# KAIST-AILab/SyncVSR

Measured on AMD Instinct MI355X. Metric: lip-clips/sec training (29x88x88), higher is better.
Workload: dtype bf16; 1 GPU; LRW training step (fwd+bwd+allreduce+clip+AdamW), ResNet18 + 6-layer 512-d encoder + vq audio-token CE head, random-init weights, N(0,1) clips 29x88x88, uniform tokens/labels; per_gpu_batch=32, global_batch=32, parallelism=dp1, hip_graph=False, enqueue=native step list

## Files before the change

### include/syncvsr_hip.h

```cpp
#ifndef SYNCVSR_HIP_H
#define SYNCVSR_HIP_H

#include <stdint.h>

#ifndef __HIP_PLATFORM_AMD__
typedef void* hipStream_t;
#else
#include <hip/hip_runtime_api.h>
#endif

#define SVSR_OK 0
#define SVSR_ERR_ARG 1001
#define SVSR_GRAD_ADD_DW 1
#define SVSR_GRAD_ADD_DB 2
#define SVSR_ERR_GROUP_OPEN 1003
#define SVSR_ERR_NO_GROUP 1004
#define SVSR_ERR_MASK_SIZE 1005

typedef struct svsr_wgrad_problem {
    const void* x; const void* dy; float* dw; float* dbias; const int* plan_dev; const int* meta;
    int Nimg; int in_pix; int Ci; int in_pitch; int Co; int out_pix; int out_pitch; int wt_taps;
} svsr_wgrad_problem;

typedef struct svsr_enc_layer {
    const void* wqkv; const void* wo; const void* w1; const void* w2;
    const float* bqkv; const float* bo; const float* b1; const float* b2; const float* g1; const float* be1; const float* g2; const float* be2;
    void* qkv; void* probs; void* ctx; void* ao; void* x1; void* z; void* hg; void* f; void* xout;
    float* m1; float* r1; float* m2; float* r2;
    unsigned site_probs; unsigned site_ao; unsigned site_fo; unsigned pad_;
} svsr_enc_layer;

typedef struct svsr_enc_bwd_layer {
    const void* w2t; const void* w1t; const void* wot; const void* wqkvt;
    const float* g1; const float* g2;
    const void* f; const void* x1; const void* ao; const void* xin; const void* z; const void* qkv; const void* probs;
    const float* m1; const float* r1; const float* m2; const float* r2;
    void* ds2; void* df; void* dz; void* dx1; void* ds1; void* dao; void* dqkv; void* dx;
    float* part1; float* part2;
    unsigned site_probs; unsigned site_ao; unsigned site_fo; unsigned pad_;
} svsr_enc_bwd_layer;

#ifdef __cplusplus
extern "C" {
#endif

int svsr_tune(const char* key, int value);
int svsr_tune_value(const char* key, int* value);
int svsr_colsum_rows(const float* ws, int nrows, int64_t ld, float* out0, int64_t n0, float* out1, int64_t n1, int accumulate, float scale, hipStream_t stream);
int svsr_colsum_rows_multi(const void* entries, int n, hipStream_t stream);

int svsr_conv_plan(int mode, int Nimg, int H, int W, int Co_out, int k, int stride, int pad, int* words, int cap_words, int* meta);
int svsr_rows_plan(int Nimg, int P, int src0, int dst0, int Co_out, int* words, int cap_words, int* meta);
int svsr_igemm_fwd_kgroups(const int* meta, int Ci, int Co, int bn_epilogue);
int svsr_igemm_fwd(const void* in, const void* wt, void* out, void* out_pre, const float* bias, const void* addend, float* stats, const int* plan_dev, const int* meta, int Nimg, int in_pix, int Ci, int in_pitch, int Co, int out_pix, int out_pitch, int wt_taps, int act, int out_f32, float alpha, const unsigned* drop_seed, unsigned drop_site, float drop_p, hipStream_t stream);

int svsr_wgrad_plan(int Nimg, int H, int W, int Ci, int Co, int k, int stride, int pad, int* words, int cap_words, int* meta, int64_t* part_floats);
int svsr_wgrad_rows_plan(int Nimg, int P, int src0, int dst0, int Ci, int Co, int has_bias, int* words, int cap_words, int* meta, int64_t* part_floats);
int svsr_igemm_wgrad(const void* x, const void* dyp, float* dw, float* dbias, const int* plan_dev, const int* meta, int Nimg, int in_pix, int Ci, int in_pitch, int Co, int out_pix, int out_pitch, int wt_taps, float* part, int64_t part_floats, hipStream_t stream);
int64_t svsr_igemm_wgrad_group_bytes(int n);
int svsr_igemm_wgrad_group(const svsr_wgrad_problem* problems, int n, void* table_dev, int64_t table_bytes, hipStream_t stream);
int svsr_igemm_wgrad_v2(const void* x, const void* dyp, float* dw, float* dbias, const int* plan_dev, const int* meta, int Nimg, int in_pix, int Ci, int in_pitch, int Co, int out_pix, int out_pitch, int wt_taps, float* part, int64_t part_floats, int mode, hipStream_t stream);
int svsr_igemm_wgrad_group_v2(const svsr_wgrad_problem* problems, const int* modes, int n, void* table_dev, int64_t table_bytes, hipStream_t stream);

int svsr_conv3x3_c64_stat_rows(int Nimg, int H, int W);
int64_t svsr_conv3x3_c64_pixtab(int Nimg, int H, int W, int* out, int64_t cap);
int svsr_conv3x3_c64(const void* in, const void* wt, void* out, const void* addend, float* stats, int Nimg, int H, int W, const int* dy, const int* dx, const int* tw, const int* pixtab, hipStream_t stream);

int svsr_igemm_dgrad_bn(const void* in, const void* wt, void* out, const void* addend, float* stats, const int* plan_dev, const int* meta, int Nimg, int in_pix, int Ci, int in_pitch, int Co, int out_pix, int out_pitch, int wt_taps, const void* y, const void* x, const float* mean, const float* rstd, const float* gamma, const float* beta, int act, hipStream_t stream);
int svsr_igemm_dgrad_relu(const void* in, const void* wt, void* out, float* stats, const int* plan_dev, const int* meta, int Nimg, int in_pix, int Ci, int in_pitch, int Co, int out_pix, int out_pitch, int wt_taps, const void* y, const float* zeros, const float* ones, float gscale, hipStream_t stream);
int svsr_conv3x3_c64_dgrad_bn(const void* in, const void* wt, void* out, const void* addend, float* stats, int Nimg, int H, int W, const int* dy, const int* dx, const int* tw, const void* y, const void* x, const float* mean, const float* rstd, const float* gamma, const float* beta, int act, const int* pixtab, hipStream_t stream);
int svsr_bn_bwd_from_stats(const void* g, const void* x, const float* mean, const float* rstd, const float* gamma, const float* stats, int nrows, float* coef, float* dgamma, float* dbeta, void* dx, int64_t npix, int C, hipStream_t stream);


int svsr_conv3x3_wgrad_plan(int Nimg, int H, int W, int Ci, int Co, int* splits, int64_t* part_floats);
int svsr_conv3x3_wgrad(const void* x, const void* dy, float* dw, int Nimg, int H, int W, int Ci, int Co, float* part, int64_t part_floats, hipStream_t stream);
int svsr_conv3x3_wgrad_v2(const void* x, const void* dy, float* dw, int Nimg, int H, int W, int Ci, int Co, float* part, int64_t part_floats, int mode, hipStream_t stream);

int svsr_stem_conv_fwd_stat_rows(int B, int T, int H, int W);
int64_t svsr_stem_conv_fwd_ws_bytes(int B, int T, int H, int W);
int svsr_stem_conv_fwd(const float* vid, const float* w, void* out, float* stats, int B, int T, int H, int W, void* ws, int64_t ws_bytes, hipStream_t stream);

int svsr_stem_conv_wgrad_plan(int B, int T, int H, int W, int* splits, int64_t* part_floats);
int svsr_stem_conv_wgrad(const float* vid, const void* dy, float* dw, int B, int T, int H, int W, int use_tr, float* part, int64_t part_floats, hipStream_t stream);

int svsr_stem_bwd_wgrad_ok(int B, int T, int H, int W);
int svsr_stem_bwd_wgrad(const float* vid, const void* gpool, const void* amax, const void* x, const float* mean, const float* rstd, const float* coef, float* dw, int B, int T, int H, int W, float* part, int64_t part_floats, hipStream_t stream);

int svsr_bn_finalize(const float* part, int nrows, int C, float count, float eps, float momentum, float* mean, float* rstd, float* running_mean, float* running_var, int64_t* num_batches_tracked, hipStream_t stream);

int svsr_bn_eval_prepare(const float* running_mean, const float* running_var, int C, float eps, float* mean, float* rstd, hipStream_t stream);

int svsr_bn_act_fwd(const void* x, const void* res, void* y, const float* mean, const float* rstd, const float* gamma, const float* beta, int64_t npix, int C, int act, hipStream_t stream);

int svsr_bn_act_bwd_rows(int64_t npix, int C);
int svsr_bn_act_bwd(const void* dy, const void* y, const void* x, const float* mean, const float* rstd, const float* gamma, float* slots, float* coef, float* dgamma, float* dbeta, void* dx, void* dres, int64_t npix, int C, int act, const float* beta, const void* res, hipStream_t stream);

int svsr_stem_bn_act_pool_fwd(const void* x, void* y, void* amax, const float* mean, const float* rstd, const float* gamma, const float* beta, int N, int Hc, int Wc, int Hp, int Wp, int C, int act, void* xwin, hipStream_t stream);

int svsr_stem_bn_act_pool_bwd_rows(int N, int Hc, int Wc, int C);
int svsr_stem_bn_act_pool_bwd(const void* dpool, const void* amax, const void* x, const float* mean, const float* rstd, const float* gamma, const float* beta, float* slots, float* coef, float* dgamma, float* dbeta, void* dx, int N, int Hc, int Wc, int Hp, int Wp, int C, int act, const void* xwin, void* gpool, hipStream_t stream);

int svsr_avgpool_fwd(const void* x, void* y, int64_t N, int HW, int C, hipStream_t stream);
int svsr_avgpool_bwd(const void* dy, void* dx, int64_t N, int HW, int C, hipStream_t stream);

int svsr_add_ln_fwd(const void* a, const void* r, const float* gamma, const float* beta, void* y, float* mean, float* rstd, int R, int D, float eps, hipStream_t stream);
int svsr_add_ln_bwd_rows(int R);
int svsr_add_ln_bwd(const void* dy, const void* a, const void* r, const float* gamma, const float* mean, const float* rstd, void* ds, float* dgamma, float* dbeta, int R, int D, const void* addend, float* part, hipStream_t stream);
int svsr_add_ln_bwd_partials(const void* dy, const void* a, const void* r, const float* gamma, const float* mean, const float* rstd, void* ds, int R, int D, const void* addend, float* part, hipStream_t stream);
int svsr_add_ln_bwd_branch(const void* dy, const void* a, const void* r, const float* gamma, const float* mean, const float* rstd, void* ds, int R, int D, const void* addend, float* part, void* ds2, float alpha2, const unsigned* drop_seed, unsigned drop_site, float drop_p, hipStream_t stream);
int svsr_bias_act_bwd_partials(const void* dy, const void* z, void* dz, float* db, int R, int N, int n_valid, int ld, int act, float gscale, float* part, hipStream_t stream);

int svsr_embed_ln_fwd(const void* feats, const float* cls, const float* pos, const float* type0, const float* gamma, const float* beta, void* sum_out, void* y, float* mean, float* rstd, int B, int S, int D, float eps, const unsigned* drop_seed, unsigned site_in, float p_in, unsigned site_out, float p_out, hipStream_t stream);
int svsr_embed_bwd_scatter(const void* ds, void* dfeats, float* dcls, float* dpos, float* dtype0, int B, int S, int D, float* part, const unsigned* drop_seed, unsigned site_in, float p_in, hipStream_t stream);

int svsr_rmsnorm_fwd(const void* x, const float* g, void* y, float* inv, int R, int D, int ld, float eps, hipStream_t stream);
int svsr_rmsnorm_bwd_rows(int R);
int svsr_rmsnorm_bwd(const void* dy, const void* x, const float* g, const float* inv, const void* addend, void* dx, float* dg, float* part, int R, int D, int ld, hipStream_t stream);

int svsr_rotary(void* qkv, const float* tab, int R, int S, int heads_total, int ld, int sign, hipStream_t stream);

int svsr_geglu_fwd(const void* u, void* y, int R, int I, int ldu, int ldy, const unsigned* drop_seed, unsigned drop_site, float drop_p, hipStream_t stream);
int svsr_geglu_bwd(const void* dy, const void* u, void* du, int R, int I, int ldu, int ldy, const unsigned* drop_seed, unsigned drop_site, float drop_p, hipStream_t stream);

int svsr_xt_embed_fwd(const void* feats, const float* wmask, const float* cls, void* x0, int B, int S, int F, int D, int ld, const unsigned* drop_seed, unsigned drop_site, float drop_p, hipStream_t stream);
int svsr_xt_embed_bwd(const void* dx0, void* dfeats, float* dcls, int B, int S, int F, int D, int ld, const unsigned* drop_seed, unsigned drop_site, float drop_p, hipStream_t stream);

int svsr_bias_act_bwd_rows(int R, int N);
int svsr_bias_act_bwd(const void* dy, const void* z, void* dz, float* db, int R, int N, int n_valid, int ld, int act, float gscale, float* part, hipStream_t stream);

int svsr_ce_fwd(const void* logits, int logits_f32, int ld, const int64_t* target_idx, const float* target_prob, int ldt, int R, int V, float smoothing, float* loss, float* lse, float* row_loss, hipStream_t stream);
int svsr_ce_bwd(const void* logits, int logits_f32, int ld, const int64_t* target_idx, const float* target_prob, int ldt, int R, int V, float smoothing, const float* lse, const float* gout, void* dlogits, int ldo, hipStream_t stream);

int svsr_linear_ce_ok(int R, int K, int G, int V);
int svsr_linear_ce_fwd(const void* h, const void* w, const float* bias, const int64_t* tok, int R, int K, int G, int V, int seq_S, int seq_s0, int seq_T, float* loss, float* lse, float* row_loss, hipStream_t stream);
int svsr_linear_ce_bwd(const void* h, const void* w, const float* bias, const int64_t* tok, int R, int K, int G, int V, int seq_S, int seq_s0, int seq_T, const float* lse, const float* gout, void* dlogits, hipStream_t stream);

int64_t svsr_w2v_stats_floats(int B, int F0);
int svsr_w2v_conv0(const float* wave, int B, int L_in, int pad, const float* w, const float* bias, const float* gamma, const float* beta, float eps, void* out, int out_rows, float* stats, int mode, hipStream_t stream);
int svsr_w2v_norm_gelu(void* x, int B, int F, int rows, const float* gamma, const float* beta, float eps, float* stats, int F0, int mode, hipStream_t stream);
int svsr_w2v_quantize(const void* feat, int R, int F, int keep, const float* gamma, const float* beta, float eps, const void* w, const float* bias, const unsigned* seed, unsigned site, int64_t* tok, float* logits_out, hipStream_t stream);

int svsr_topk_acc(const float* logits, const int64_t* labels, const float* soft_labels, int B, int C, float* out2, float* rows2, hipStream_t stream);

int svsr_grad_sumsq(const float* g, int64_t n, void* opt_state, hipStream_t stream);
int svsr_grad_sumsq_parts(const float* g, int64_t n, void* opt_state, int part0, int nparts, hipStream_t stream);
int svsr_adamw_step(float* p, const float* g, float* m, float* v, void* shadow, int64_t n, int64_t decay_end, float lr, float beta1, float beta2, float eps, float weight_decay, float max_norm, int warmup, int total_steps, void* opt_state, hipStream_t stream);
int svsr_adamw_range(float* p, const float* g, float* m, float* v, void* shadow, int64_t n, int64_t decay_end, float lr, float beta1, float beta2, float eps, float weight_decay, float max_norm, int warmup, int total_steps, void* opt_state, int advance, hipStream_t stream);

int svsr_cast_bf16(const float* src, void* dst, int64_t n, hipStream_t stream);
int svsr_transpose_cast_multi(const float* src, void* dst, const void* table, int n_entries, hipStream_t stream);
int svsr_transpose_bf16_multi(const void* src16, void* dst, const void* table, int n_entries, hipStream_t stream);
int svsr_fill_f32(float* p, int64_t n, float v, hipStream_t stream);
int svsr_fill_ranges(float* base, int64_t limit, const int64_t* ranges, int n, unsigned bits, hipStream_t stream);
int svsr_enc_gave_up(int reset);
int svsr_enc_gave_up_peek(void);
int svsr_debug_enc_spin_limit(unsigned limit);
int64_t svsr_enc_fwd_ws_bytes(int B);
int svsr_debug_enc_trace(int64_t* out, int n);
int svsr_enc_fwd(const void* x0, const svsr_enc_layer* layers, int n_layers, int B, int S, float ln_eps, const unsigned* drop_seed, float p_hidden, float p_attn, void* ws, int64_t ws_bytes, hipStream_t stream);

int64_t svsr_enc_bwd_ws_bytes(int B);
int svsr_enc_bwd(const void* dy, const svsr_enc_bwd_layer* layers, int n_layers, int B, int S, const unsigned* drop_seed, float p_hidden, float p_attn, void* ws, int64_t ws_bytes, hipStream_t stream);

int svsr_word_add(int* word, int delta, hipStream_t stream);
int svsr_lincomb2(const float* a, const float* b, float wb, float* out, hipStream_t stream);
int svsr_lincomb3_ratio(const float* a, float wa, const float* b, float wb, const float* c, float wc, float* out0, const float* num, const float* den, float* out1, hipStream_t stream);

int svsr_clip_prep(const void* src_u8, const int* params, float* dst, int B, int T, int Hs, int Ws, int H, int W, float mean, float std, hipStream_t stream);

int svsr_mha_fwd(const void* q, int q_pitch, const void* k, const void* v, int kv_pitch, const void* pe, int pe_pitch, const float* bias_u, const float* bias_v, const int* klen, int causal, int B, int H, int dh, int Lq, int Lk, int ldp, float scale, void* ctx, int ctx_pitch, void* probs, const unsigned* drop_seed, unsigned drop_site, float drop_p, hipStream_t stream);

int svsr_mha_bwd(const void* dctx, int dctx_pitch, const void* q, int q_pitch, const void* k, const void* v, int kv_pitch, const void* pe, int pe_pitch, const float* bias_u, const float* bias_v, const void* probs, void* ds, int B, int H, int dh, int Lq, int Lk, int ldp, float scale, void* dq, int dq_pitch, void* dq_ac, void* dq_bd, int aux_pitch, void* dk, void* dv, int dkv_pitch, void* dpe, int dpe_pitch, float* pe_part, const unsigned* drop_seed, unsigned drop_site, float drop_p, hipStream_t stream);

int64_t svsr_mha_flash_ws_bytes(int H, int Lq);
int svsr_mha_flash_fwd(const void* q, int q_pitch, const void* k, const void* v, int kv_pitch, const void* pe, int pe_pitch, const float* bias_u, const float* bias_v, const int* klen, int causal, int B, int H, int dh, int Lq, int Lk, int ldp, float scale, void* ctx, int ctx_pitch, float* lse, const unsigned* drop_seed, unsigned drop_site, float drop_p, hipStream_t stream);
int svsr_mha_flash_bwd(const void* dctx, int dctx_pitch, const void* ctx, int ctx_pitch, const float* lse, const void* q, int q_pitch, const void* k, const void* v, int kv_pitch, const void* pe, int pe_pitch, const float* bias_u, const float* bias_v, const int* klen, int causal, void* probs, void* ds, int B, int H, int dh, int Lq, int Lk, int ldp, float scale, void* dq, int dq_pitch, void* dq_ac, void* dq_bd, int aux_pitch, void* dk, void* dv, int dkv_pitch, void* dpe, int dpe_pitch, float* pe_part, void* ws, int64_t ws_bytes, const unsigned* drop_seed, unsigned drop_site, float drop_p, hipStream_t stream);
int svsr_mha_pe_transpose(const void* pe, int pe_pitch, int H, int Lq, void* ws, int64_t ws_bytes, hipStream_t stream);
int svsr_mha_flash_bwd_parts(const void* dctx, int dctx_pitch, const void* ctx, int ctx_pitch, const float* lse, const void* q, int q_pitch, const void* k, const void* v, int kv_pitch, const void* pe, int pe_pitch, const float* bias_u, const float* bias_v, const int* klen, int causal, void* probs, void* ds, int B, int H, int dh, int Lq, int Lk, int ldp, float scale, void* dq, int dq_pitch, void* dq_ac, void* dq_bd, int aux_pitch, void* dk, void* dv, int dkv_pitch, void* dpe, int dpe_pitch, float* pe_part, void* ws, int64_t ws_bytes, const unsigned* drop_seed, unsigned drop_site, float drop_p, int parts, hipStream_t stream);

int svsr_glu_dwconv_fwd_stat_rows(int B, int T);
int svsr_glu_dwconv_fwd(const void* u, const float* w, const float* bias, void* c, float* stats, int B, int T, int D, int K, hipStream_t stream);

int svsr_glu_dwconv_bwd(const void* dc, const void* u, const float* w, void* du, float* dw, float* dbias, float* part, int nsplit, int B, int T, int D, int K, hipStream_t stream);
int svsr_glu_dwconv_bwd_parts(const void* dc, const void* u, const float* w, void* du, float* dw, float* dbias, float* part, int nsplit, int B, int T, int D, int K, int parts, hipStream_t stream);

int svsr_ctc_fwd(const float* logits, int ld, const int64_t* labels, int Lmax, const int* ilen, int B, int T, int V, float* lse, float* ab, float* nll, float* loss, hipStream_t stream);

int svsr_ctc_grad(const float* logits, int ld, const int64_t* labels, int Lmax, const int* ilen, int B, int T, int V, const float* lse, const float* ab, const float* nll, const float* gout, void* dlogits, int ldo, hipStream_t stream);

int svsr_ctc_prefix_score(const float* logp, int ldp, const float* r_prev, const int64_t* last, const int64_t* ids, float* r_new, float* psi, int T, int V, int n, int S, int out_len, int blank, int eos, hipStream_t stream);

int svsr_lrs_targets(const int64_t* label, int B, int L, int odim, int64_t ignore_id, int64_t eos, int64_t* labels, int64_t* ys_in, int64_t* ys_out, hipStream_t stream);
int svsr_lrs_target_errors(int reset);
int svsr_embed_pos_fwd(const int64_t* tok, const float* emb, const float* pe, void* x, int R, int L, int D, float scale, hipStream_t stream);
int svsr_embed_pos_bwd(const int64_t* tok, const void* dx, float* demb, int R, int D, float scale, hipStream_t stream);

int svsr_ls_loss_fwd(const float* logits, int ld, const int64_t* target, int R, int V, float smoothing, float inv_denom, float* loss, float* lse, float* counts, float* rows3, hipStream_t stream);
int svsr_ls_loss_bwd(const float* logits, int ld, const int64_t* target, int R, int V, float smoothing, float inv_denom, const float* lse, const float* gout, void* dlogits, int ldo, hipStream_t stream);

int svsr_scale_bf16(const void* x, void* y, int64_t n, float alpha, const unsigned* drop_seed, unsigned drop_site, float drop_p, hipStream_t stream);

int svsr_mha_table_fwd(const void* pool, int pool_rows, int64_t pitch, const int* table, int table_pitch, int n, int Lq, int L, int H, float scale, void* ctx, int64_t ctx_pitch, hipStream_t stream);
int svsr_lm_embed_fwd(const void* x, int64_t x_pitch, const float* gamma, const float* beta, const float* pe, int pe_rows, const int* pos, int R, int D, float eps, float scale, void* out, hipStream_t stream);

int svsr_tconv_fwd(const void* x, int64_t x_pitch, int B, int T, int n_in, int d, int nb, const int64_t* branches, int co, int act, void* out, int64_t out_pitch, const void* res, int64_t res_pitch, int res_act, hipStream_t stream);
int svsr_tcn_se_fwd(const void* x, int64_t x_pitch, int B, int T, int n_in, int R, int nb, const void* w1, const void* w2, float* gate, hipStream_t stream);
int svsr_tcn_norm_pool_fwd(const void* x, int64_t x_pitch, int B, int T, int C, const float* scale, const float* shift, const float* mask, void* h, void* pooled, hipStream_t stream);

int svsr_beam_select_slices(int V, int beam, int max_rows);
int svsr_beam_select(const float* s0, const float* s1, const float* s2, const float* s3, float w0, float w1, float w2, float w3, int nplanes, int64_t ldv, const float* run, const int* clip_of, const int* row_lo, const int* out_off, int n, int C, int V, int beam, int max_rows, int out_rows, void* cand, int64_t* prev, int64_t* tok, float* total, float* vals, int* clip_out, int* count, hipStream_t stream);
int svsr_ctc_prefix_score_clips(const float* logp, int ldp, const float* r_prev, const int64_t* last, const int64_t* ids, const int* clip_of, const int* tlen, float* r_new, float* psi, int C, int Tmax, int V, int n, int S, int out_len, int blank, int eos, hipStream_t stream);
int svsr_mha_src_step_fwd(const void* q, int64_t q_pitch, const void* kv, int64_t kv_pitch, const int* clip_of, const int* tlen, int C, int Tmax, int n, int H, float scale, void* ctx, int64_t ctx_pitch, hipStream_t stream);

void* svsr_steplist_create(void);
int svsr_steplist_destroy(void* list);
int svsr_steplist_knows(const char* name);
int svsr_steplist_push_call(void* list, const char* name, const int64_t* slots, int nslots);
int svsr_steplist_push_wait(void* list, hipStream_t waiter, hipStream_t signaller);
int svsr_steplist_push_memset(void* list, void* ptr, int value, int64_t bytes, hipStream_t stream);
int svsr_steplist_push_break(void* list);
int svsr_steplist_segments(void* list);
int64_t svsr_steplist_size(void* list);
int svsr_steplist_run(void* list, int segment, int* failed);
int svsr_steplist_dry_run(void* list, int segment, int64_t* counts);
int svsr_steplist_push_group(void* list, int group);
int svsr_steplist_push_copy(void* list, void* dst, const void* src, int64_t bytes, hipStream_t stream, int when_skipped);
int svsr_steplist_set_skips(void* list, const uint8_t* mask, int ngroups);
int svsr_steplist_groups(void* list);
int64_t svsr_steplist_calls(void* list, int group);
int64_t svsr_steplist_last_issued(void* list);
int svsr_stream_wait(hipStream_t waiter, hipStream_t signaller);
int svsr_memset_async(void* ptr, int value, int64_t bytes, hipStream_t stream);
int svsr_memcpy_async(void* dst, const void* src, int64_t bytes, hipStream_t stream);

int svsr_device_cus(void);

int svsr_clock_probe(int64_t* out, int blocks, int iters, hipStream_t stream);

int svsr_debug_occupy_start(int workgroups, int lds_bytes, hipStream_t stream);
int svsr_debug_occupy_stop(void);

#ifdef __cplusplus
}
#endif
#endif
```

### syncvsr_amd/csrc/igemm_fwd.h

```cpp
#pragma once
#include "common.h"

struct IgemmFwdArgs {
    const bf16_t* in;
    const bf16_t* wt;
    void* out;
    bf16_t* out_pre;
    const float* bias;
    const bf16_t* addend;
    float* stats;
    const int* plan;
    int Nimg, in_pix, Ci, in_pitch;
    int Co, out_pix, out_pitch, wt_taps;
    int act, out_f32;
    float alpha;
    DropArgs drop;
    const bf16_t* bnb_y;
    const bf16_t* bnb_x;
    const float* bnb_mean;
    const float* bnb_rstd;
    const float* bnb_gamma;
    const float* bnb_beta;
    int bnb_act;
};


#define LDS_SWZ(row, chunk) ((row) * 64 + ((((chunk) ^ (((row) >> 1) & 7))) << 3))

#define P8_MAGIC 0x50380001
#define P8_HDR_WORDS 8
#define P8_DESC_WORDS 64
#define P8_BM 256
#define P8_BN 128
int igemm_p8_launch(const IgemmFwdArgs& a, const int* meta, hipStream_t stream);
```

### syncvsr_amd/csrc/igemm_fwd.hip

```cpp

#include <algorithm>
#include <map>
#include <vector>

#include "common.h"
#include "igemm_fwd.h"

#define PLAN_CLS_WORDS 24
#define PLAN_HDR_WORDS 2

__device__ unsigned g_zero_page[64];


template <int BM, int BN, int TM, int TN>
__device__ __forceinline__ void igemm_epilogue(const IgemmFwdArgs& p, f32x16 (&acc)[TM][TN], unsigned char* smem_raw, const long* sRow,
                                               int wm0, int wn0, int n0, int tid, bool active, int m_tile) {
    constexpr int WN = BN / 2;
    const int lane = tid & 63, wave = tid >> 6;
    float st_s[TN], st_q[TN];
    const bool bnb = p.bnb_x != nullptr;
    if (p.stats != nullptr && !bnb) {
#pragma unroll
        for (int j = 0; j < TN; ++j) {
            float s = 0.f, q = 0.f;
#pragma unroll
            for (int i = 0; i < TM; ++i)
#pragma unroll
                for (int r = 0; r < 16; ++r) { const float v = acc[i][j][r]; s += v; q += v * v; }
            st_s[j] = s + __shfl_xor(s, 32, 64);
            st_q[j] = q + __shfl_xor(q, 32, 64);
        }
    }
    float* sOut = reinterpret_cast<float*>(smem_raw);
    if (active) {
#pragma unroll
        for (int i = 0; i < TM; ++i)
#pragma unroll
            for (int j = 0; j < TN; ++j)
#pragma unroll
                for (int r = 0; r < 16; ++r) {
                    const int row = wm0 + i * 32 + (r & 3) + 8 * (r >> 2) + 4 * (lane >> 5);
                    sOut[row * BN + wn0 + j * 32 + (lane & 31)] = acc[i][j][r];
                }
    }
    __syncthreads();
    const bool vec_pitch = (p.out_pitch & 7) == 0;
    constexpr int CV = BN / 8;
    static_assert(256 % CV == 0, "a thread keeps its column group across the store loop");
    float bias8[8];
    {
        const int nb = n0 + (tid % CV) * 8;
#pragma unroll
        for (int k = 0; k < 8; ++k) bias8[k] = (p.bias != nullptr && nb + k < p.Co) ? p.bias[nb + k] : 0.f;
    }
    constexpr int ITERS = BM * CV / 256, RSTEP = 256 / CV;
    static_assert(BM * CV % 256 == 0, "whole rows per pass");
    const int c8 = tid % CV, rbase = tid / CV, n = n0 + c8 * 8;
    float bs1[8], bs2[8];
#pragma unroll
    for (int k = 0; k < 8; ++k) { bs1[k] = 0.f; bs2[k] = 0.f; }
    if (bnb) {
        float mu[8], rs[8];
        if (active) {
#pragma unroll
            for (int k = 0; k < 8; ++k) { mu[k] = p.bnb_mean[n + k]; rs[k] = p.bnb_rstd[n + k]; }
            const bool from_x = p.bnb_y == nullptr, swish_act = p.bnb_act == 2;
            float sc[8], sh[8];
            if (from_x || swish_act) {
#pragma unroll
                for (int k = 0; k < 8; ++k) { sc[k] = p.bnb_gamma[n + k] * rs[k]; sh[k] = __builtin_fmaf(-mu[k], sc[k], p.bnb_beta[n + k]); }
            }
            long offs[ITERS];
            u32x4 add8[ITERS], y8[ITERS], x8[ITERS];
#pragma unroll
            for (int i = 0; i < ITERS; ++i) offs[i] = sRow[rbase + RSTEP * i];
#pragma unroll
            for (int i = 0; i < ITERS; ++i) {
                const long o = (offs[i] >= 0 ? offs[i] : 0) + n;
                x8[i] = *reinterpret_cast<const u32x4*>(p.bnb_x + o);
                if (!from_x) y8[i] = *reinterpret_cast<const u32x4*>(p.bnb_y + o);
                if (p.addend != nullptr) add8[i] = *reinterpret_cast<const u32x4*>(p.addend + o);
            }
#pragma unroll
            for (int i = 0; i < ITERS; ++i) {
                if (offs[i] < 0) continue;
                const int r = rbase + RSTEP * i;
                const f32x4 lo = *reinterpret_cast<const f32x4*>(sOut + r * BN + c8 * 8);
                const f32x4 hi = *reinterpret_cast<const f32x4*>(sOut + r * BN + c8 * 8 + 4);
                float v[8] = {lo[0], lo[1], lo[2], lo[3], hi[0], hi[1], hi[2], hi[3]};
                float yv[8], xv[8];
                unpack8(x8[i], xv);
                if (from_x) {
#pragma unroll
                    for (int k = 0; k < 8; ++k) yv[k] = __builtin_fmaf(xv[k], sc[k], sh[k]);
                } else {
                    unpack8(y8[i], yv);
                }
                if (p.addend != nullptr) {
                    float a8[8];
                    unpack8(add8[i], a8);
#pragma unroll
                    for (int k = 0; k < 8; ++k) v[k] += a8[k];
                }
                if (swish_act) {
#pragma unroll
                    for (int k = 0; k < 8; ++k) {
                        const float z = __builtin_fmaf(xv[k], sc[k], sh[k]) + (from_x ? 0.f : yv[k]);
                        v[k] = bf2f(f2bf(bf2f(f2bf(v[k])) * swish_grad(z)));
                        bs1[k] += v[k];
                        bs2[k] += v[k] * (xv[k] - mu[k]) * rs[k];
                    }
                } else {
#pragma unroll
                    for (int k = 0; k < 8; ++k) {
                        v[k] = yv[k] > 0.f ? bf2f(f2bf(v[k])) : 0.f;
                        if (p.alpha != 1.f) v[k] = bf2f(f2bf(v[k] * p.alpha));
                        bs1[k] += v[k];
                        bs2[k] += v[k] * (xv[k] - mu[k]) * rs[k];
                    }
                }
                *reinterpret_cast<u32x4*>(reinterpret_cast<bf16_t*>(p.out) + offs[i] + n) = pack8(v);
            }
        }
    } else if (__builtin_expect(active && vec_pitch && n + 8 <= p.Co, 1)) {
        long offs[ITERS];
        f32x4 lo[ITERS], hi[ITERS];
        u32x4 add8[ITERS];
#pragma unroll
        for (int i = 0; i < ITERS; ++i) {
            const int r = rbase + RSTEP * i;
            offs[i] = sRow[r];
            lo[i] = *reinterpret_cast<const f32x4*>(sOut + r * BN + c8 * 8);
            hi[i] = *reinterpret_cast<const f32x4*>(sOut + r * BN + c8 * 8 + 4);
        }
        if (p.addend != nullptr) {
#pragma unroll
            for (int i = 0; i < ITERS; ++i)
                add8[i] = *reinterpret_cast<const u32x4*>(p.addend + (offs[i] >= 0 ? offs[i] : 0) + n);
        }
        const unsigned key = p.drop.seed != nullptr ? drop_key(p.drop) : 0u;
#pragma unroll
        for (int i = 0; i < ITERS; ++i) {
            const long off = offs[i];
            if (off < 0) continue;
            float v[8] = {lo[i][0], lo[i][1], lo[i][2], lo[i][3], hi[i][0], hi[i][1], hi[i][2], hi[i][3]};
#pragma unroll
            for (int k = 0; k < 8; ++k) v[k] += bias8[k];
            if (p.act == 1) {
                if (p.out_pre != nullptr) *reinterpret_cast<u32x4*>(p.out_pre + off + n) = pack8(v);
#pragma unroll
                for (int k = 0; k < 8; ++k) v[k] = gelu_erf(v[k]);
            } else if (p.act == 2) {
#pragma unroll
                for (int k = 0; k < 8; ++k) v[k] = fmaxf(v[k], 0.f);
            }
            if (p.drop.seed != nullptr) {
#pragma unroll
                for (int k = 0; k < 8; ++k) v[k] = drop_keep(key, p.drop.thresh, (unsigned)(off + n + k)) ? v[k] * p.drop.scale : 0.f;
            }
            if (p.alpha != 1.f) {
#pragma unroll
                for (int k = 0; k < 8; ++k) v[k] *= p.alpha;
            }
            if (p.addend != nullptr) {
                float a8[8];
                unpack8(add8[i], a8);
#pragma unroll
                for (int k = 0; k < 8; ++k) v[k] += a8[k];
            }
            if (p.out_f32) {
                float* o = reinterpret_cast<float*>(p.out) + off + n;
                *reinterpret_cast<f32x4*>(o) = f32x4{v[0], v[1], v[2], v[3]};
                *reinterpret_cast<f32x4*>(o + 4) = f32x4{v[4], v[5], v[6], v[7]};
            } else {
                *reinterpret_cast<u32x4*>(reinterpret_cast<bf16_t*>(p.out) + off + n) = pack8(v);
            }
        }
    } else
    for (int task = active ? tid : BM * CV; task < BM * CV; task += 256) {
        const int r = task / CV, c8 = task - r * CV;
        const long off = sRow[r];
        const int n = n0 + c8 * 8;
        if (off < 0 || n >= p.Co) continue;
        float v[8];
        const f32x4 lo = *reinterpret_cast<const f32x4*>(sOut + r * BN + c8 * 8);
        const f32x4 hi = *reinterpret_cast<const f32x4*>(sOut + r * BN + c8 * 8 + 4);
        v[0] = lo[0]; v[1] = lo[1]; v[2] = lo[2]; v[3] = lo[3]; v[4] = hi[0]; v[5] = hi[1]; v[6] = hi[2]; v[7] = hi[3];
        if (vec_pitch && n + 8 <= p.Co) {
#pragma unroll
            for (int k = 0; k < 8; ++k) v[k] += bias8[k];
            if (p.act == 1) {
                if (p.out_pre != nullptr) *reinterpret_cast<u32x4*>(p.out_pre + off + n) = pack8(v);
#pragma unroll
                for (int k = 0; k < 8; ++k) v[k] = gelu_erf(v[k]);
            } else if (p.act == 2) {
#pragma unroll
                for (int k = 0; k < 8; ++k) v[k] = fmaxf(v[k], 0.f);
            }
            if (p.drop.seed != nullptr) {
                const unsigned key = drop_key(p.drop);
#pragma unroll
                for (int k = 0; k < 8; ++k) v[k] = drop_keep(key, p.drop.thresh, (unsigned)(off + n + k)) ? v[k] * p.drop.scale : 0.f;
            }
            if (p.alpha != 1.f) {
#pragma unroll
                for (int k = 0; k < 8; ++k) v[k] *= p.alpha;
            }
            if (p.addend != nullptr) {
                float a8[8];
                unpack8(*reinterpret_cast<const u32x4*>(p.addend + off + n), a8);
#pragma unroll
                for (int k = 0; k < 8; ++k) v[k] += a8[k];
            }
            if (p.out_f32) {
                float* o = reinterpret_cast<float*>(p.out) + off + n;
                *reinterpret_cast<f32x4*>(o) = f32x4{v[0], v[1], v[2], v[3]};
                *reinterpret_cast<f32x4*>(o + 4) = f32x4{v[4], v[5], v[6], v[7]};
            } else {
                *reinterpret_cast<u32x4*>(reinterpret_cast<bf16_t*>(p.out) + off + n) = pack8(v);
            }
        } else {
#pragma unroll
            for (int k = 0; k < 8; ++k) {
                if (n + k >= p.Co) break;
                float x = v[k] + bias8[k];
                if (p.act == 1) {
                    if (p.out_pre != nullptr) p.out_pre[off + n + k] = f2bf(x);
                    x = gelu_erf(x);
                } else if (p.act == 2) {
                    x = fmaxf(x, 0.f);
                }
                if (p.drop.seed != nullptr) x = drop_keep(drop_key(p.drop), p.drop.thresh, (unsigned)(off + n + k)) ? x * p.drop.scale : 0.f;
                x *= p.alpha;
                if (p.addend != nullptr) x += bf2f(p.addend[off + n + k]);
                if (p.out_f32) reinterpret_cast<float*>(p.out)[off + n + k] = x;
                else reinterpret_cast<bf16_t*>(p.out)[off + n + k] = f2bf(x);
            }
        }
    }
    if (bnb) {
        __syncthreads();
        float* red = reinterpret_cast<float*>(smem_raw);
        if (active) {
#pragma unroll
            for (int k = 0; k < 8; ++k) { red[tid * 16 + k] = bs1[k]; red[tid * 16 + 8 + k] = bs2[k]; }
        }
        __syncthreads();
        for (int c = active ? tid : 2 * BN; c < 2 * BN; c += 256) {
            const int which = c / BN, cc = c - which * BN;
            float s = 0.f;
            for (int rb = 0; rb < RSTEP; ++rb) s += red[(rb * CV + (cc >> 3)) * 16 + which * 8 + (cc & 7)];
            if (n0 + cc < p.Co) p.stats[((long)m_tile * 2 + which) * p.Co + n0 + cc] = s;
        }
    } else if (p.stats != nullptr) {
        __syncthreads();
        float* red = reinterpret_cast<float*>(smem_raw);
#pragma unroll
        for (int j = 0; j < TN; ++j)
            if (active && lane < 32) {
                red[(wave * WN + j * 32 + lane) * 2 + 0] = st_s[j];
                red[(wave * WN + j * 32 + lane) * 2 + 1] = st_q[j];
            }
        __syncthreads();
        for (int c = active ? tid : BN; c < BN; c += 256) {
            const int wcol = c / WN, cc = c - wcol * WN;
            const float s = red[((0 * 2 + wcol) * WN + cc) * 2 + 0] + red[((1 * 2 + wcol) * WN + cc) * 2 + 0];
            const float q = red[((0 * 2 + wcol) * WN + cc) * 2 + 1] + red[((1 * 2 + wcol) * WN + cc) * 2 + 1];
            if (n0 + c < p.Co) {
                p.stats[((long)m_tile * 2 + 0) * p.Co + n0 + c] = s;
                p.stats[((long)m_tile * 2 + 1) * p.Co + n0 + c] = q;
            }
        }
    }
}

template <int BM, int BN, int TM, int TN>
__device__ __forceinline__ void igemm_mma_tile(const bf16_t* cA, const bf16_t* cB, f32x16 (&acc)[TM][TN], int wm0, int wn0, int lane) {
#pragma unroll
    for (int ks = 0; ks < 4; ++ks) {
        const int ch = ks * 2 + (lane >> 5);
        bf16x8 fa[TM], fb[TN];
#pragma unroll
        for (int i = 0; i < TM; ++i) {
            const int row = wm0 + i * 32 + (lane & 31);
            fa[i] = *reinterpret_cast<const bf16x8*>(cA + LDS_SWZ(row, ch));
        }
#pragma unroll
        for (int j = 0; j < TN; ++j) {
            const int row = wn0 + j * 32 + (lane & 31);
            fb[j] = *reinterpret_cast<const bf16x8*>(cB + LDS_SWZ(row, ch));
        }
#pragma unroll
        for (int i = 0; i < TM; ++i)
#pragma unroll
            for (int j = 0; j < TN; ++j)
                acc[i][j] = __builtin_amdgcn_mfma_f32_32x32x16_bf16(fa[i], fb[j], acc[i][j], 0, 0, 0);
    }
}

template <int LPT, int MAXL>
__device__ __forceinline__ void wait_tiles_barrier(int later) {
    if constexpr (MAXL > 0) {
        if (later == MAXL) { SVSR_WAIT_VM_BARRIER(LPT * MAXL); return; }
        wait_tiles_barrier<LPT, MAXL - 1>(later);
    } else {
        asm volatile("s_waitcnt vmcnt(0)\n\ts_barrier" ::: "memory");
    }
}

__device__ __forceinline__ void split_row(int m, int P, float inv_p, int& n, int& j) {
    n = (int)((float)m * inv_p);
    j = m - n * P;
    if (j < 0) { n--; j += P; } else if (j >= P) { n++; j -= P; }
}

template <int BM, int BN, int NS, int KG = 1>
__global__ __launch_bounds__(256 * KG) void k_igemm_fwd_glds(const IgemmFwdArgs p) {
    constexpr int BK = 64;
    static_assert(NS >= 2 && (BM / 32 + BN / 32) * (NS - 2) <= 63, "vmcnt immediate is 6 bits");
    constexpr int WM = BM / 2, WN = BN / 2, TM = WM / 32, TN = WN / 32;
    constexpr int A_ELEMS = BM * BK, B_ELEMS = BN * BK, S_ELEMS = A_ELEMS + B_ELEMS;
    constexpr int AR = BM / 32, BR = BN / 32, LPT = AR + BR;
    extern __shared__ __attribute__((aligned(16))) unsigned char smem_raw[];
    const int grp = KG == 1 ? 0 : __builtin_amdgcn_readfirstlane((int)threadIdx.x >> 8);
    bf16_t* sStage = reinterpret_cast<bf16_t*>(smem_raw) + grp * NS * S_ELEMS;
    long* sRow = reinterpret_cast<long*>(reinterpret_cast<bf16_t*>(smem_raw) + KG * NS * S_ELEMS);
    int* sTap = reinterpret_cast<int*>(sRow + BM);

    const int tid = threadIdx.x & 255, lane = tid & 63, wave = tid >> 6;
    const int wm0 = (wave >> 1) * WM, wn0 = (wave & 1) * WN;
    const int bx = blockIdx.x, by = blockIdx.y;
    const int n0 = by * BN;
    const int slot = tid & 7, r0 = tid >> 3;
    const int csw = slot ^ ((r0 >> 1) & 7);
    const int wrow = __builtin_amdgcn_readfirstlane(wave) * 8;

    const int hdr0 = p.plan[0];
    const int ncls = hdr0 & 0xffff;
    const bool identity = (hdr0 >> 16) != 0;
    int cls = 0;
    for (int c = 1; c < ncls; ++c)
        if (bx >= p.plan[PLAN_HDR_WORDS + c * PLAN_CLS_WORDS + 3]) cls = c;
    const int* cw = p.plan + PLAN_HDR_WORDS + cls * PLAN_CLS_WORDS;
    const int ntaps = cw[0], P = cw[1];
    const int* pos = p.plan + p.plan[1] + 2 * cw[2];
    const int m0 = (bx - cw[3]) * BM;
    const int Mc = p.Nimg * P;
    const float inv_p = 1.0f / (float)P;
    if (tid < 18) sTap[tid] = cw[4 + tid];

    const bf16_t* zero_src = reinterpret_cast<const bf16_t*>(g_zero_page) + slot * 8;
    const bf16_t* a_ptr[AR];
    unsigned a_ok = 0;
#pragma unroll
    for (int i = 0; i < AR; ++i) {
        const int m = m0 + r0 + 32 * i;
        const bool ok = m < Mc;
        if (identity) {
            a_ptr[i] = p.in + (long)(ok ? m : 0) * p.in_pix * p.in_pitch + csw * 8;
        } else {
            int n, j;
            split_row(ok ? m : 0, P, inv_p, n, j);
            a_ptr[i] = p.in + ((long)n * p.in_pix + pos[2 * j]) * p.in_pitch + csw * 8;
        }
        a_ok |= (ok ? 1u : 0u) << i;
    }
    const bf16_t* b_ptr[BR];
#pragma unroll
    for (int i = 0; i < BR; ++i) {
        const int n = n0 + r0 + 32 * i;
        b_ptr[i] = n < p.Co ? p.wt + (long)n * p.wt_taps * p.Ci + csw * 8 : nullptr;
    }
    for (int r = tid; r < BM; r += 256) {
        const int m = m0 + r;
        long off = -1;
        if (m < Mc) {
            if (identity) {
                off = (long)m * p.out_pix * p.out_pitch;
            } else {
                int n, j;
                split_row(m, P, inv_p, n, j);
                off = ((long)n * p.out_pix + pos[2 * j + 1]) * p.out_pitch;
            }
        }
        sRow[r] = off;
    }
    __syncthreads();

    const int KT_all = ntaps * (p.Ci / BK);
    const int KT_loop = (KT_all + KG - 1) / KG;
    const int k_begin = grp * KT_loop;
    const int KT = KT_all - k_begin < KT_loop ? (KT_all - k_begin > 0 ? KT_all - k_begin : 0) : KT_loop;
    const int spt = p.Ci / BK;
    int t_next = k_begin / spt, c_next = (k_begin - (k_begin / spt) * spt) * BK;
    auto stage = [&](int buf) {
        const int tw = sTap[9 + t_next];
        const int c0 = c_next;
        const long a_off = (long)sTap[t_next] * p.in_pitch + c0;
        bf16_t* dstA = sStage + buf * S_ELEMS + wrow * 64;
#pragma unroll
        for (int i = 0; i < AR; ++i) {
            const bf16_t* src = ((a_ok >> i) & 1u) ? a_ptr[i] + a_off : zero_src;
            __builtin_amdgcn_global_load_lds((const __attribute__((address_space(1))) void*)src,
                                             (__attribute__((address_space(3))) void*)(dstA + i * 32 * 64), 16, 0, 0);
        }
        bf16_t* dstB = sStage + buf * S_ELEMS + A_ELEMS + wrow * 64;
#pragma unroll
        for (int i = 0; i < BR; ++i) {
            const bf16_t* src = b_ptr[i] != nullptr ? b_ptr[i] + (long)tw * p.Ci + c0 : zero_src;
            __builtin_amdgcn_global_load_lds((const __attribute__((address_space(1))) void*)src,
                                             (__attribute__((address_space(3))) void*)(dstB + i * 32 * 64), 16, 0, 0);
        }
        c_next += BK;
        if (c_next >= p.Ci) { c_next = 0; ++t_next; }
    };

    f32x16 acc[TM][TN];
#pragma unroll
    for (int i = 0; i < TM; ++i)
#pragma unroll
        for (int j = 0; j < TN; ++j)
#pragma unroll
            for (int r = 0; r < 16; ++r) acc[i][j][r] = 0.f;

#pragma unroll
    for (int s = 0; s < NS - 1; ++s)
        if (s < KT) stage(s);
    int buf = 0;
    for (int it = 0; it < KT_loop; ++it) {
        int later = KT - 1 - it < NS - 2 ? KT - 1 - it : NS - 2;
        if (later < 0) later = 0;
        wait_tiles_barrier<LPT, NS - 2>(later);
        if (it + NS - 1 < KT) stage(buf >= 1 ? buf - 1 : NS - 1);
        if (KG == 1 || it < KT) {
            const bf16_t* cA = sStage + buf * S_ELEMS;
            igemm_mma_tile<BM, BN, TM, TN>(cA, cA + A_ELEMS, acc, wm0, wn0, lane);
        }
        buf = buf + 1 == NS ? 0 : buf + 1;
    }
    __syncthreads();
    if constexpr (KG == 2) {
        float* sX = reinterpret_cast<float*>(reinterpret_cast<bf16_t*>(smem_raw) + NS * S_ELEMS);
        static_assert((size_t)TM * TN * 16 * 256 * sizeof(float) <= (size_t)NS * S_ELEMS * sizeof(bf16_t), "exchange buffer fits the ring");
        if (grp == 1) {
#pragma unroll
            for (int i = 0; i < TM; ++i)
#pragma unroll
                for (int j = 0; j < TN; ++j)
#pragma unroll
                    for (int r = 0; r < 16; ++r) sX[((i * TN + j) * 16 + r) * 256 + tid] = acc[i][j][r];
        }
        __syncthreads();
        if (grp == 0) {
#pragma unroll
            for (int i = 0; i < TM; ++i)
#pragma unroll
                for (int j = 0; j < TN; ++j)
#pragma unroll
                    for (int r = 0; r < 16; ++r) acc[i][j][r] += sX[((i * TN + j) * 16 + r) * 256 + tid];
        }
        __syncthreads();
    }
    igemm_epilogue<BM, BN, TM, TN>(p, acc, smem_raw, sRow, wm0, wn0, n0, tid, grp == 0, bx);
}

template <int BM, int BN, int NS, int KG = 1>
static int launch_glds(const IgemmFwdArgs& a, int gx, int gy, hipStream_t stream) {
    const size_t lds = (size_t)KG * NS * (BM + BN) * 64 * sizeof(bf16_t) + (size_t)BM * sizeof(long) + 128;
    static size_t attr_set = 0;
    if (attr_set < lds) {
        (void)hipFuncSetAttribute(reinterpret_cast<const void*>(k_igemm_fwd_glds<BM, BN, NS, KG>), hipFuncAttributeMaxDynamicSharedMemorySize, (int)lds);
        attr_set = lds;
    }
    IgemmFwdArgs b = a;
    hipLaunchKernelGGL((k_igemm_fwd_glds<BM, BN, NS, KG>), dim3(gx, gy), dim3(256 * KG), lds, stream, b);
    return svsr_check_launch();
}

struct IgemmFwdPlan { int bm, bn, ns, gy; };

static IgemmFwdPlan igemm_fwd_plan(long M, int Co, int max_taps) {
    const int cus = svsr_stream_cus(nullptr);
    IgemmFwdPlan pl;
    const int forced = svsr_tune_get(SVSR_TUNE_IGEMM_TILE);
    const int thr = svsr_tune_get(SVSR_TUNE_IGEMM_M128);
    int bm;
    if (forced == 64 || forced == 128) bm = forced;
    else if (Co <= 64) bm = M >= 16384 ? 128 : 64;
    else {
        const long blocks128 = ((M + 127) / 128) * ((Co + 127) / 128);
        bm = (M >= thr || blocks128 >= 224) ? 128 : 64;
    }
    const int lin_rows = svsr_tune_get(SVSR_TUNE_IGEMM_LIN_BN64);
    if (bm == 64 && forced == 0 && Co > 64 && max_taps == 1 && lin_rows > 0 && M >= lin_rows) { pl.bm = 128; pl.bn = 64; pl.ns = 3; }
    else if (bm == 128 && Co > 64 && max_taps > 1 && ((M + 127) / 128) * ((Co + 127) / 128) < svsr_tune_get(SVSR_TUNE_IGEMM_BN64_BELOW)) { pl.bm = 128; pl.bn = 64; pl.ns = 2; }
    else if (bm == 128 && Co <= 64) { pl.bm = 128; pl.bn = 64; pl.ns = max_taps <= 4 ? 2 : 3; }
    else if (bm == 128) { pl.bm = 128; pl.bn = 128; pl.ns = 2; }
    else { pl.bm = 64; pl.bn = 64; pl.ns = 0; }
    pl.gy = (Co + pl.bn - 1) / pl.bn;
    if (pl.ns == 0) pl.ns = ((M + pl.bm - 1) / pl.bm) * pl.gy <= (long)cus * 5 / 2 ? 4 : 3;
    return pl;
}

struct PlanClass { int ntaps; int delta[9], tw[9]; std::vector<int> pos; };

static int plan_emit_p8(const std::vector<PlanClass>& cls, int Nimg, int Co, int in_pix, int out_pix, int* words, int cap_words, int* meta, long M, int max_taps, int bn) {
    long tiles_m = 0;
    for (const PlanClass& c : cls) tiles_m += ((long)Nimg * (long)(c.pos.size() / 2) + P8_BM - 1) / P8_BM;
    const int gy = Co / bn;
    const long nwords = P8_HDR_WORDS + tiles_m * (P8_DESC_WORDS + 2 * P8_BM);
    if (nwords > 0x7fffffffL || (long)Nimg * in_pix >= (1L << 31) || (long)Nimg * out_pix >= (1L << 31)) return -SVSR_ERR_ARG;
    if (words != nullptr) {
        if (cap_words < nwords) return -SVSR_ERR_ARG;
        const int off_desc = P8_HDR_WORDS, off_rows = P8_HDR_WORDS + (int)tiles_m * P8_DESC_WORDS;
        words[0] = P8_MAGIC; words[1] = (int)tiles_m; words[2] = gy; words[3] = off_desc; words[4] = off_rows;
        words[5] = (int)((tiles_m + 7) / 8 * 8 * gy); words[6] = 0; words[7] = 0;
        long t = 0;
        for (const PlanClass& c : cls) {
            const long P = (long)(c.pos.size() / 2), Mc = (long)Nimg * P;
            for (long m0 = 0; m0 < Mc; m0 += P8_BM, ++t) {
                int* d = words + off_desc + t * P8_DESC_WORDS;
                for (int k = 0; k < P8_DESC_WORDS; ++k) d[k] = 0;
                d[0] = c.ntaps; d[1] = (int)(Mc - m0 < P8_BM ? Mc - m0 : P8_BM);
                for (int k = 0; k < c.ntaps; ++k) { d[2 + k] = c.delta[k]; d[11 + k] = c.tw[k]; }
                int* rt = words + off_rows + t * 2 * P8_BM;
                for (int rr = 0; rr < P8_BM; ++rr) {
                    const long m = m0 + rr;
                    if (m < Mc) {
                        const long n = m / P, j = m - n * P;
                        rt[2 * rr] = (int)(n * in_pix + c.pos[2 * j]);
                        rt[2 * rr + 1] = (int)(n * out_pix + c.pos[2 * j + 1]);
                    } else { rt[2 * rr] = rt[0]; rt[2 * rr + 1] = -1; }
                }
            }
        }
    }
    if (meta != nullptr) {
        meta[0] = P8_BM; meta[1] = bn; meta[2] = 3; meta[3] = (int)tiles_m; meta[4] = gy; meta[5] = (int)cls.size(); meta[6] = max_taps;
        meta[7] = (int)(M & 0x7fffffff);
    }
    return (int)nwords;
}

static int plan_emit(std::vector<PlanClass>& cls, int Nimg, int Co, int* words, int cap_words, int* meta, const int* p8_pix = nullptr) {
    std::stable_sort(cls.begin(), cls.end(), [](const PlanClass& a, const PlanClass& b) { return a.ntaps > b.ntaps; });
    long M = 0;
    int max_taps = 0;
    for (const PlanClass& c : cls) { M += (long)Nimg * (long)(c.pos.size() / 2); if (c.ntaps > max_taps) max_taps = c.ntaps; }
    if (M >= (1L << 24) * 64 || cls.empty()) return -SVSR_ERR_ARG;
    if (p8_pix != nullptr && svsr_tune_get(SVSR_TUNE_P8) && Co % 64 == 0) {
        long tiles_m = 0;
        int min_taps = 9;
        for (const PlanClass& c : cls) { tiles_m += ((long)Nimg * (long)(c.pos.size() / 2) + P8_BM - 1) / P8_BM; if (c.ntaps < min_taps) min_taps = c.ntaps; }
        const int min_items = svsr_tune_get(SVSR_TUNE_P8_MIN_ITEMS);
        if (min_taps >= 4 && Co % P8_BN == 0 && tiles_m * (Co / P8_BN) >= min_items)
            return plan_emit_p8(cls, Nimg, Co, p8_pix[0], p8_pix[1], words, cap_words, meta, M, max_taps, P8_BN);
        if (min_taps >= 4 && Co >= 128 && tiles_m * (Co / 64) >= min_items)
            return plan_emit_p8(cls, Nimg, Co, p8_pix[0], p8_pix[1], words, cap_words, meta, M, max_taps, 64);
    }
    const IgemmFwdPlan pl = igemm_fwd_plan(M, Co, max_taps);
    const int ncls = (int)cls.size();
    int nwords = PLAN_HDR_WORDS + ncls * PLAN_CLS_WORDS;
    const int pos_word0 = nwords;
    for (const PlanClass& c : cls) nwords += (int)c.pos.size();
    long tiles = 0;
    if (words != nullptr) {
        if (cap_words < nwords) return -SVSR_ERR_ARG;
        words[0] = ncls; words[1] = pos_word0;
        int pos_off = 0;
        for (int i = 0; i < ncls; ++i) {
            const PlanClass& c = cls[i];
            int* w = words + PLAN_HDR_WORDS + i * PLAN_CLS_WORDS;
            const int P = (int)(c.pos.size() / 2);
            if ((long)Nimg * P >= (1L << 24)) return -SVSR_ERR_ARG;
            w[0] = c.ntaps; w[1] = P; w[2] = pos_off; w[3] = (int)tiles;
            for (int t = 0; t < 9; ++t) { w[4 + t] = t < c.ntaps ? c.delta[t] : 0; w[13 + t] = t < c.ntaps ? c.tw[t] : 0; }
            w[22] = 0; w[23] = 0;
            std::copy(c.pos.begin(), c.pos.end(), words + pos_word0 + 2 * pos_off);
            pos_off += P;
            tiles += ((long)Nimg * P + pl.bm - 1) / pl.bm;
        }
    } else {
        for (const PlanClass& c : cls) tiles += ((long)Nimg * (long)(c.pos.size() / 2) + pl.bm - 1) / pl.bm;
    }
    if (tiles > 0x7fffffffL) return -SVSR_ERR_ARG;
    if (meta != nullptr) {
        meta[0] = pl.bm; meta[1] = pl.bn; meta[2] = pl.ns; meta[3] = (int)tiles; meta[4] = pl.gy; meta[5] = ncls; meta[6] = max_taps;
        meta[7] = (int)(M & 0x7fffffff);
    }
    return nwords;
}

extern "C" int svsr_conv_plan(int mode, int Nimg, int H, int W, int Co_out, int k, int stride, int pad, int* words, int cap_words, int* meta) {
    if (Nimg < 1 || H < 1 || W < 1 || k < 1 || k > 3 || stride < 1 || pad < 0 || Co_out < 1 || mode < 0 || mode > 2) return -SVSR_ERR_ARG;
    const int Ho = (H + 2 * pad - k) / stride + 1, Wo = (W + 2 * pad - k) / stride + 1;
    if (Ho < 1 || Wo < 1) return -SVSR_ERR_ARG;
    std::vector<PlanClass> cls;
    std::map<std::vector<int>, int> index;
    auto add = [&](const std::vector<int>& key, int src, int dst) {
        auto it = index.find(key);
        if (it == index.end()) {
            PlanClass c;
            c.ntaps = (int)(key.size() / 2);
            for (int t = 0; t < c.ntaps; ++t) { c.delta[t] = key[2 * t]; c.tw[t] = key[2 * t + 1]; }
            cls.push_back(c);
            it = index.emplace(key, (int)cls.size() - 1).first;
        }
        cls[it->second].pos.push_back(src);
        cls[it->second].pos.push_back(dst);
    };
    std::vector<int> key;
    if (mode == 0) {
        for (int a = 0; a < Ho; ++a)
            for (int b = 0; b < Wo; ++b) {
                key.clear();
                for (int kh = 0; kh < k; ++kh)
                    for (int kw = 0; kw < k; ++kw) {
                        const int iy = a * stride + kh - pad, ix = b * stride + kw - pad;
                        if (iy < 0 || iy >= H || ix < 0 || ix >= W) continue;
                        key.push_back((kh - pad) * W + (kw - pad));
                        key.push_back(kh * k + kw);
                    }
                add(key, (a * stride) * W + b * stride, a * Wo + b);
            }
    } else {
        for (int y = 0; y < H; ++y)
            for (int x = 0; x < W; ++x) {
                key.clear();
                const int a = y / stride, b = x / stride, py = y % stride, px = x % stride;
                for (int kh = 0; kh < k; ++kh) {
                    if ((py + pad - kh) % stride) continue;
                    for (int kw = 0; kw < k; ++kw) {
                        if ((px + pad - kw) % stride) continue;
                        const int dq = (py + pad - kh) / stride, dp = (px + pad - kw) / stride;
                        const int oy = a + dq, ox = b + dp;
                        if (oy < 0 || oy >= Ho || ox < 0 || ox >= Wo) continue;
                        key.push_back(dq * Wo + dp);
                        key.push_back(kh * k + kw);
                    }
                }
                int ca = a < Ho ? a : Ho - 1, cb = b < Wo ? b : Wo - 1;
                if (ca != a || cb != b) {
                    const int shift = (a - ca) * Wo + (b - cb);
                    for (size_t t = 0; t < key.size(); t += 2) key[t] += shift;
                }
                if (mode == 2 && key.empty()) continue;
                add(key, ca * Wo + cb, y * W + x);
            }
    }
    const int p8_pix[2] = {mode == 0 ? H * W : Ho * Wo, mode == 0 ? Ho * Wo : H * W};
    const bool p8_ok = k == 3 && pad == 1 && H >= 2 && W >= 2 && (stride == 1 || (stride == 2 && mode == 0 && svsr_tune_get(SVSR_TUNE_P8) >= 1 && svsr_tune_get(SVSR_TUNE_P8) != 3));
    return plan_emit(cls, Nimg, Co_out, words, cap_words, meta, p8_ok ? p8_pix : nullptr);
}

extern "C" int svsr_rows_plan(int Nimg, int P, int src0, int dst0, int Co_out, int* words, int cap_words, int* meta) {
    if (Nimg < 1 || P < 1 || Co_out < 1) return -SVSR_ERR_ARG;
    std::vector<PlanClass> cls(1);
    cls[0].ntaps = 1; cls[0].delta[0] = 0; cls[0].tw[0] = 0;
    cls[0].pos.reserve(2 * (size_t)P);
    for (int j = 0; j < P; ++j) { cls[0].pos.push_back(src0 + j); cls[0].pos.push_back(dst0 + j); }
    const int n = plan_emit(cls, Nimg, Co_out, words, cap_words, meta);
    if (n > 0 && words != nullptr && P == 1 && src0 == 0 && dst0 == 0) words[0] |= 1 << 16;
    return n;
}

extern "C" int svsr_igemm_fwd_kgroups(const int* meta, int Ci, int Co, int bn_epilogue) {
    if (meta == nullptr || Ci < 64) return 1;
    const int bm = meta[0], bn = meta[1], gx = meta[3], gy = (Co + bn - 1) / bn;
    const int ks = svsr_tune_get(SVSR_TUNE_IGEMM_KSPLIT);
    if (!bn_epilogue && bm == 64 && bn == 64 && ks && (long)gx * gy <= ks && (long)meta[6] * (Ci / 64) >= 12) return 2;
    const int ks128 = svsr_tune_get(SVSR_TUNE_IGEMM_KSPLIT128);
    if (!bn_epilogue && bm == 128 && bn == 64 && meta[2] == 3 && meta[6] == 1 && ks128 > 0 && Ci / 64 >= ks128 && (long)gx * gy <= 288) return 2;
    return 1;
}

static int igemm_fwd_run(const void* in, const void* wt, void* out, void* out_pre, const float* bias, const void* addend,
                         float* stats, const int* plan_dev, const int* meta, int Nimg, int in_pix, int Ci, int in_pitch, int Co,
                         int out_pix, int out_pitch, int wt_taps, int act, int out_f32, float alpha, const unsigned* drop_seed,
                         unsigned drop_site, float drop_p, const void* bnb_y, const void* bnb_x, const float* bnb_mean,
                         const float* bnb_rstd, const float* bnb_gamma, const float* bnb_beta, int bnb_act, hipStream_t stream) {
    if (plan_dev == nullptr || meta == nullptr || Ci % 64 != 0 || Ci <= 0 || Co <= 0 || in_pitch % 8 != 0 || Nimg <= 0 || wt_taps < 1)
        return SVSR_ERR_ARG;
    if (act != 0 && (addend != nullptr || alpha != 1.f)) return SVSR_ERR_ARG;
    IgemmFwdArgs a;
    a.in = (const bf16_t*)in; a.wt = (const bf16_t*)wt; a.out = out; a.out_pre = (bf16_t*)out_pre;
    a.bias = bias; a.addend = (const bf16_t*)addend; a.stats = stats; a.plan = plan_dev;
    a.Nimg = Nimg; a.in_pix = in_pix; a.Ci = Ci; a.in_pitch = in_pitch; a.Co = Co; a.out_pix = out_pix; a.out_pitch = out_pitch;
    a.wt_taps = wt_taps; a.act = act; a.out_f32 = out_f32; a.alpha = alpha;
    a.drop = svsr_make_drop(drop_seed, drop_site, drop_p);
    a.bnb_y = (const bf16_t*)bnb_y; a.bnb_x = (const bf16_t*)bnb_x; a.bnb_mean = bnb_mean; a.bnb_rstd = bnb_rstd;
    a.bnb_gamma = bnb_gamma; a.bnb_beta = bnb_beta; a.bnb_act = bnb_act;
    const int bm = meta[0], bn = meta[1], ns = meta[2], gx = meta[3], gy = (Co + bn - 1) / bn;
    if (gx < 1) return SVSR_ERR_ARG;
    if (bm == P8_BM) return (bnb_x != nullptr && alpha != 1.f) ? SVSR_ERR_ARG : igemm_p8_launch(a, meta, stream);
    if (svsr_igemm_fwd_kgroups(meta, Ci, Co, bnb_x != nullptr) == 2) {
        if (bm == 128) return launch_glds<128, 64, 3, 2>(a, gx, gy, stream);
        return launch_glds<64, 64, 4, 2>(a, gx, gy, stream);
    }
#define SVSR_IGEMM_CASE(BM_, BN_, NS_) if (bm == BM_ && bn == BN_ && ns == NS_) return launch_glds<BM_, BN_, NS_>(a, gx, gy, stream)
    SVSR_IGEMM_CASE(128, 128, 2);
    SVSR_IGEMM_CASE(128, 64, 2);
    SVSR_IGEMM_CASE(128, 64, 3);
    SVSR_IGEMM_CASE(64, 64, 4);
    SVSR_IGEMM_CASE(64, 64, 3);
#undef SVSR_IGEMM_CASE
    return SVSR_ERR_ARG;
}

extern "C" int svsr_igemm_fwd(const void* in, const void* wt, void* out, void* out_pre, const float* bias, const void* addend,
                              float* stats, const int* plan_dev, const int* meta, int Nimg, int in_pix, int Ci, int in_pitch, int Co,
                              int out_pix, int out_pitch, int wt_taps, int act, int out_f32, float alpha, const unsigned* drop_seed,
                              unsigned drop_site, float drop_p, hipStream_t stream) {
    return igemm_fwd_run(in, wt, out, out_pre, bias, addend, stats, plan_dev, meta, Nimg, in_pix, Ci, in_pitch, Co, out_pix, out_pitch,
                         wt_taps, act, out_f32, alpha, drop_seed, drop_site, drop_p, nullptr, nullptr, nullptr, nullptr, nullptr, nullptr, 0, stream);
}

extern "C" int svsr_igemm_dgrad_relu(const void* in, const void* wt, void* out, float* stats, const int* plan_dev, const int* meta, int Nimg,
                                     int in_pix, int Ci, int in_pitch, int Co, int out_pix, int out_pitch, int wt_taps, const void* y,
                                     const float* zeros, const float* ones, float gscale, hipStream_t stream) {
    if (y == nullptr || zeros == nullptr || ones == nullptr || stats == nullptr || Co % 8 != 0 || out_pitch % 8 != 0 || !(gscale > 0.f)) return SVSR_ERR_ARG;
    return igemm_fwd_run(in, wt, out, nullptr, nullptr, nullptr, stats, plan_dev, meta, Nimg, in_pix, Ci, in_pitch, Co, out_pix, out_pitch,
                         wt_taps, 0, 0, gscale, nullptr, 0, 0.f, nullptr, y, zeros, ones, ones, zeros, 1, stream);
}

extern "C" int svsr_igemm_dgrad_bn(const void* in, const void* wt, void* out, const void* addend, float* stats, const int* plan_dev,
                                   const int* meta, int Nimg, int in_pix, int Ci, int in_pitch, int Co, int out_pix, int out_pitch,
                                   int wt_taps, const void* y, const void* x, const float* mean, const float* rstd, const float* gamma,
                                   const float* beta, int act, hipStream_t stream) {
    if (x == nullptr || mean == nullptr || rstd == nullptr || stats == nullptr || Co % 8 != 0 || out_pitch % 8 != 0) return SVSR_ERR_ARG;
    if (act != 1 && act != 2) return SVSR_ERR_ARG;
    if ((y == nullptr || act == 2) && (gamma == nullptr || beta == nullptr)) return SVSR_ERR_ARG;
    return igemm_fwd_run(in, wt, out, nullptr, nullptr, addend, stats, plan_dev, meta, Nimg, in_pix, Ci, in_pitch, Co, out_pix, out_pitch,
                         wt_taps, 0, 0, 1.0f, nullptr, 0, 0.f, y, x, mean, rstd, gamma, beta, act, stream);
}
```

### syncvsr_amd/csrc/steplist.hip

```cpp
#include <stdlib.h>
#include <string.h>

#include <string>
#include <unordered_map>
#include <utility>
#include <vector>

#include "common.h"
#include "../../include/syncvsr_hip.h"

namespace {

typedef int64_t Slot;

template <typename T> struct FromSlot;
template <> struct FromSlot<int> { static int get(Slot s) { return (int)s; } };
template <> struct FromSlot<unsigned> { static unsigned get(Slot s) { return (unsigned)s; } };
template <> struct FromSlot<int64_t> { static int64_t get(Slot s) { return s; } };
template <> struct FromSlot<float> { static float get(Slot s) { double d; memcpy(&d, &s, sizeof d); return (float)d; } };
template <typename P> struct FromSlot<P*> { static P* get(Slot s) { return reinterpret_cast<P*>((uintptr_t)s); } };

template <typename... A, size_t... I>
int invoke(int (*fn)(A...), const Slot* s, std::index_sequence<I...>) { return fn(FromSlot<A>::get(s[I])...); }

template <typename... A>
int thunk_n(int (*)(A...)) { return (int)sizeof...(A); }

typedef int (*Thunk)(const Slot*);
struct Entry { Thunk call; int nargs; };

template <typename F, F fn> struct Bind;
template <typename... A, int (*fn)(A...)>
struct Bind<int (*)(A...), fn> {
    static int call(const Slot* s) { return invoke(fn, s, std::index_sequence_for<A...>{}); }
    static constexpr int nargs = (int)sizeof...(A);
};

#define SVSR_REG(f) {#f, Entry{&Bind<decltype(&f), &f>::call, Bind<decltype(&f), &f>::nargs}}

const std::unordered_map<std::string, Entry>& registry() {
    static const std::unordered_map<std::string, Entry> r = {
        SVSR_REG(svsr_colsum_rows), SVSR_REG(svsr_colsum_rows_multi), SVSR_REG(svsr_igemm_fwd), SVSR_REG(svsr_igemm_wgrad), SVSR_REG(svsr_conv3x3_c64),
        SVSR_REG(svsr_igemm_dgrad_bn), SVSR_REG(svsr_igemm_dgrad_relu), SVSR_REG(svsr_conv3x3_c64_dgrad_bn), SVSR_REG(svsr_bn_bwd_from_stats),
        SVSR_REG(svsr_conv3x3_wgrad), SVSR_REG(svsr_stem_conv_fwd), SVSR_REG(svsr_stem_conv_wgrad), SVSR_REG(svsr_stem_bwd_wgrad), SVSR_REG(svsr_bn_finalize),
        SVSR_REG(svsr_bn_eval_prepare), SVSR_REG(svsr_bn_act_fwd), SVSR_REG(svsr_bn_act_bwd), SVSR_REG(svsr_stem_bn_act_pool_fwd),
        SVSR_REG(svsr_stem_bn_act_pool_bwd), SVSR_REG(svsr_avgpool_fwd), SVSR_REG(svsr_avgpool_bwd), SVSR_REG(svsr_add_ln_fwd),
        SVSR_REG(svsr_add_ln_bwd), SVSR_REG(svsr_embed_ln_fwd), SVSR_REG(svsr_embed_bwd_scatter), SVSR_REG(svsr_rmsnorm_fwd),
        SVSR_REG(svsr_rmsnorm_bwd), SVSR_REG(svsr_rotary), SVSR_REG(svsr_geglu_fwd), SVSR_REG(svsr_geglu_bwd), SVSR_REG(svsr_xt_embed_fwd),
        SVSR_REG(svsr_xt_embed_bwd), SVSR_REG(svsr_bias_act_bwd), SVSR_REG(svsr_ce_fwd), SVSR_REG(svsr_ce_bwd), SVSR_REG(svsr_linear_ce_fwd), SVSR_REG(svsr_linear_ce_bwd), SVSR_REG(svsr_topk_acc),
        SVSR_REG(svsr_grad_sumsq), SVSR_REG(svsr_grad_sumsq_parts), SVSR_REG(svsr_adamw_step), SVSR_REG(svsr_adamw_range), SVSR_REG(svsr_cast_bf16), SVSR_REG(svsr_transpose_cast_multi),
        SVSR_REG(svsr_transpose_bf16_multi), SVSR_REG(svsr_fill_f32), SVSR_REG(svsr_clip_prep), SVSR_REG(svsr_mha_fwd), SVSR_REG(svsr_mha_bwd), SVSR_REG(svsr_mha_flash_fwd), SVSR_REG(svsr_mha_flash_bwd), SVSR_REG(svsr_mha_flash_bwd_parts), SVSR_REG(svsr_mha_pe_transpose),
        SVSR_REG(svsr_glu_dwconv_fwd), SVSR_REG(svsr_glu_dwconv_bwd), SVSR_REG(svsr_glu_dwconv_bwd_parts), SVSR_REG(svsr_ctc_fwd), SVSR_REG(svsr_ctc_grad),
        SVSR_REG(svsr_ctc_prefix_score), SVSR_REG(svsr_lrs_targets), SVSR_REG(svsr_embed_pos_fwd), SVSR_REG(svsr_embed_pos_bwd), SVSR_REG(svsr_ls_loss_fwd),
        SVSR_REG(svsr_ls_loss_bwd), SVSR_REG(svsr_scale_bf16), SVSR_REG(svsr_word_add), SVSR_REG(svsr_lincomb2), SVSR_REG(svsr_igemm_wgrad_group), SVSR_REG(svsr_enc_fwd), SVSR_REG(svsr_enc_bwd), SVSR_REG(svsr_lincomb3_ratio), SVSR_REG(svsr_add_ln_bwd_partials), SVSR_REG(svsr_add_ln_bwd_branch), SVSR_REG(svsr_bias_act_bwd_partials),
        SVSR_REG(svsr_memcpy_async), SVSR_REG(svsr_w2v_conv0), SVSR_REG(svsr_w2v_norm_gelu), SVSR_REG(svsr_w2v_quantize),
        SVSR_REG(svsr_igemm_wgrad_v2), SVSR_REG(svsr_igemm_wgrad_group_v2), SVSR_REG(svsr_conv3x3_wgrad_v2), SVSR_REG(svsr_fill_ranges),
        SVSR_REG(svsr_mha_table_fwd), SVSR_REG(svsr_lm_embed_fwd),
        SVSR_REG(svsr_beam_select), SVSR_REG(svsr_ctc_prefix_score_clips), SVSR_REG(svsr_mha_src_step_fwd),
        SVSR_REG(svsr_tconv_fwd), SVSR_REG(svsr_tcn_se_fwd), SVSR_REG(svsr_tcn_norm_pool_fwd),
    };
    return r;
}

enum { OP_CALL = 0, OP_WAIT, OP_MEMSET, OP_BREAK, OP_COPY };
constexpr int MAX_ARGS = 48;

struct Op {
    int kind;
    Thunk call;
    int nargs;
    Slot args[MAX_ARGS];
    hipEvent_t ev;
    hipStream_t a, b;
    void* ptr; int value; size_t bytes;
    const void* src;
    int group;
};

struct StepList {
    std::vector<Op> ops;
    std::vector<size_t> seg_begin{0};
    std::vector<hipEvent_t> events;
    std::string last_error;
    int open_group = -1;
    std::vector<int64_t> group_calls;
    std::vector<uint8_t> skips;
    int64_t issued = 0;
};

bool skipped(const StepList* l, int group) { return group >= 0 && (size_t)group < l->skips.size() && l->skips[group] != 0; }

}

extern "C" {

int svsr_steplist_knows(const char* name) { return name != nullptr && registry().count(name) ? 1 : 0; }

void* svsr_steplist_create(void) { return new StepList(); }

int svsr_steplist_destroy(void* list) {
    StepList* l = static_cast<StepList*>(list);
    if (l == nullptr) return SVSR_ERR_ARG;
    for (hipEvent_t e : l->events) (void)hipEventDestroy(e);
    delete l;
    return SVSR_OK;
}

int svsr_steplist_push_call(void* list, const char* name, const int64_t* slots, int nslots) {
    StepList* l = static_cast<StepList*>(list);
    if (l == nullptr || name == nullptr || (slots == nullptr && nslots > 0)) return SVSR_ERR_ARG;
    auto it = registry().find(name);
    if (it == registry().end() || it->second.nargs != nslots || nslots > MAX_ARGS) return SVSR_ERR_ARG;
    Op op{};
    op.kind = OP_CALL; op.call = it->second.call; op.nargs = nslots; op.group = l->open_group;
    for (int i = 0; i < nslots; ++i) op.args[i] = slots[i];
    l->ops.push_back(op);
    if (l->open_group >= 0) ++l->group_calls[l->open_group];
    return SVSR_OK;
}

static unsigned wait_event_flags() {
    static const unsigned flags = [] {
        const char* v = getenv("SVSR_EVENT_SYSTEM_FENCE");
        return (unsigned)hipEventDisableTiming | ((v != nullptr && v[0] == '1') ? 0u : (unsigned)hipEventDisableSystemFence);
    }();
    return flags;
}

int svsr_steplist_push_wait(void* list, hipStream_t waiter, hipStream_t signaller) {
    StepList* l = static_cast<StepList*>(list);
    if (l == nullptr) return SVSR_ERR_ARG;
    Op op{};
    op.kind = OP_WAIT; op.a = waiter; op.b = signaller; op.group = -1;
    if (hipEventCreateWithFlags(&op.ev, wait_event_flags()) == hipSuccess) {
        l->events.push_back(op.ev);
    } else {
        op.ev = nullptr;
        (void)hipGetLastError();
    }
    l->ops.push_back(op);
    return SVSR_OK;
}

int svsr_steplist_push_memset(void* list, void* ptr, int value, int64_t bytes, hipStream_t stream) {
    StepList* l = static_cast<StepList*>(list);
    if (l == nullptr || ptr == nullptr || bytes < 0) return SVSR_ERR_ARG;
    Op op{};
    op.kind = OP_MEMSET; op.ptr = ptr; op.value = value; op.bytes = (size_t)bytes; op.a = stream; op.group = l->open_group;
    l->ops.push_back(op);
    return SVSR_OK;
}

int svsr_steplist_push_break(void* list) {
    StepList* l = static_cast<StepList*>(list);
    if (l == nullptr) return -SVSR_ERR_ARG;
    if (l->open_group >= 0) return -SVSR_ERR_GROUP_OPEN;
    l->seg_begin.push_back(l->ops.size());
    return (int)l->seg_begin.size() - 1;
}

int svsr_steplist_push_group(void* list, int group) {
    StepList* l = static_cast<StepList*>(list);
    if (l == nullptr || group < -1) return SVSR_ERR_ARG;
    if (group == -1) {
        if (l->open_group < 0) return SVSR_ERR_NO_GROUP;
        l->open_group = -1;
        return SVSR_OK;
    }
    if (l->open_group >= 0) return SVSR_ERR_GROUP_OPEN;
    if ((size_t)group >= l->group_calls.size()) l->group_calls.resize((size_t)group + 1, 0);
    l->open_group = group;
    return SVSR_OK;
}

int svsr_steplist_push_copy(void* list, void* dst, const void* src, int64_t bytes, hipStream_t stream, int when_skipped) {
    StepList* l = static_cast<StepList*>(list);
    if (l == nullptr || dst == nullptr || src == nullptr || bytes < 0) return SVSR_ERR_ARG;
    if (l->open_group >= 0) return SVSR_ERR_GROUP_OPEN;
    if (when_skipped < 0 || (size_t)when_skipped >= l->group_calls.size()) return SVSR_ERR_NO_GROUP;
    Op op{};
    op.kind = OP_COPY; op.ptr = dst; op.src = src; op.bytes = (size_t)bytes; op.a = stream; op.group = when_skipped;
    l->ops.push_back(op);
    return SVSR_OK;
}

int svsr_steplist_set_skips(void* list, const uint8_t* mask, int ngroups) {
    StepList* l = static_cast<StepList*>(list);
    if (l == nullptr || ngroups < 0 || (mask == nullptr && ngroups > 0)) return SVSR_ERR_ARG;
    if ((size_t)ngroups != l->group_calls.size()) return SVSR_ERR_MASK_SIZE;
    l->skips.assign(mask, mask + ngroups);
    return SVSR_OK;
}

int svsr_steplist_groups(void* list) {
    StepList* l = static_cast<StepList*>(list);
    return l == nullptr ? 0 : (int)l->group_calls.size();
}

int64_t svsr_steplist_calls(void* list, int group) {
    StepList* l = static_cast<StepList*>(list);
    if (l == nullptr) return -SVSR_ERR_ARG;
    if (group >= 0) return (size_t)group < l->group_calls.size() ? l->group_calls[group] : -SVSR_ERR_NO_GROUP;
    int64_t n = 0;
    for (const Op& op : l->ops) n += op.kind == OP_CALL;
    return n;
}

int64_t svsr_steplist_last_issued(void* list) {
    StepList* l = static_cast<StepList*>(list);
    return l == nullptr ? 0 : l->issued;
}

int svsr_steplist_segments(void* list) {
    StepList* l = static_cast<StepList*>(list);
    return l == nullptr ? 0 : (int)l->seg_begin.size();
}

int64_t svsr_steplist_size(void* list) {
    StepList* l = static_cast<StepList*>(list);
    return l == nullptr ? 0 : (int64_t)l->ops.size();
}

}

namespace {

template <bool ISSUE>
int walk(StepList* l, int segment, int* failed, int64_t* counts) {
    if (l == nullptr || segment >= (int)l->seg_begin.size()) return SVSR_ERR_ARG;
    const size_t lo = segment < 0 ? 0 : l->seg_begin[segment];
    const size_t hi = (segment < 0 || segment + 1 == (int)l->seg_begin.size()) ? l->ops.size() : l->seg_begin[segment + 1];
    if (ISSUE && segment <= 0) l->issued = 0;
    for (size_t i = lo; i < hi; ++i) {
        Op& op = l->ops[i];
        int rc = 0, kind = 0;
        switch (op.kind) {
            case OP_CALL:
                if (skipped(l, op.group)) continue;
                if (ISSUE) { rc = op.call(op.args); ++l->issued; }
                kind = 0;
                break;
            case OP_WAIT: {
                kind = 1;
                if (!ISSUE) break;
                hipError_t e = hipSuccess;
                if (op.ev == nullptr) {
                    e = hipEventCreateWithFlags(&op.ev, wait_event_flags());
                    if (e == hipSuccess) l->events.push_back(op.ev); else op.ev = nullptr;
                }
                if (e == hipSuccess) e = hipEventRecord(op.ev, op.b);
                if (e == hipSuccess) e = hipStreamWaitEvent(op.a, op.ev, 0);
                rc = (int)e;
                break;
            }
            case OP_MEMSET:
                if (skipped(l, op.group)) continue;
                if (ISSUE) rc = (int)hipMemsetAsync(op.ptr, op.value, op.bytes, op.a);
                kind = 2;
                break;
            case OP_COPY:
                if (!skipped(l, op.group)) continue;
                if (ISSUE) rc = (int)hipMemcpyAsync(op.ptr, op.src, op.bytes, hipMemcpyDeviceToDevice, op.a);
                kind = 3;
                break;
            default: continue;
        }
        if (rc != 0) {
            if (failed != nullptr) *failed = (int)i;
            return rc;
        }
        if (counts != nullptr) ++counts[kind];
    }
    return SVSR_OK;
}

}

extern "C" {

int svsr_steplist_run(void* list, int segment, int* failed) { return walk<true>(static_cast<StepList*>(list), segment, failed, nullptr); }

int svsr_steplist_dry_run(void* list, int segment, int64_t* counts) {
    if (counts == nullptr) return SVSR_ERR_ARG;
    counts[0] = counts[1] = counts[2] = counts[3] = 0;
    return walk<false>(static_cast<StepList*>(list), segment, nullptr, counts);
}

int svsr_stream_wait(hipStream_t waiter, hipStream_t signaller) {
    static hipEvent_t ring[64];
    static unsigned next = 0;
    static bool made = false;
    if (!made) {
        for (hipEvent_t& e : ring) {
            hipError_t rc = hipEventCreateWithFlags(&e, wait_event_flags());
            if (rc != hipSuccess) return (int)rc;
        }
        made = true;
    }
    hipEvent_t ev = ring[next++ & 63u];
    hipError_t e = hipEventRecord(ev, signaller);
    if (e == hipSuccess) e = hipStreamWaitEvent(waiter, ev, 0);
    return (int)e;
}

int svsr_memset_async(void* ptr, int value, int64_t bytes, hipStream_t stream) {
    if (ptr == nullptr || bytes < 0) return SVSR_ERR_ARG;
    return (int)hipMemsetAsync(ptr, value, (size_t)bytes, stream);
}

int svsr_memcpy_async(void* dst, const void* src, int64_t bytes, hipStream_t stream) {
    if (dst == nullptr || src == nullptr || bytes < 0) return SVSR_ERR_ARG;
    return (int)hipMemcpyAsync(dst, src, (size_t)bytes, hipMemcpyDeviceToDevice, stream);
}

}
```

### syncvsr_amd/model.py

```python
from __future__ import annotations

import math
from typing import Any, Optional

import torch
import torch.nn as nn

from . import ops
from .config import Config, audio_codec_dims
from .init import buffer_specs, hidden_dim, init_state_dict, pad64, param_specs, phys_shape, resnet_block_specs, xt_dims

BF16 = torch.bfloat16


class _SideStream:

    def __init__(self) -> None:
        self.stream: Optional[torch.cuda.Stream] = None
        self.keep: list = []
        self._issuing = False
        self.enabled = False
        self.enabled_small = False

    def run(self, fn, *keep, small: bool = False) -> None:
# ... 321 lines not shown
        return feats.float().view(videos.size(0), -1, 512)

    def forward(self, videos: torch.Tensor, audio_tokens: torch.Tensor, labels: torch.Tensor, word_mask: torch.Tensor) -> dict[str, torch.Tensor]:
        _require_device(videos)
        st = self.store()
        T = videos.size(2)
        A = self.audio_alignment
        audio_tokens = audio_tokens[:, : T * A].contiguous()
        if audio_tokens.size(1) != T * A:
            raise ValueError(f"audio_tokens has {audio_tokens.size(1)} steps, need >= {T * A}")
        wm = None
        if self.use_wb:
            if word_mask.shape != (videos.size(0), T):
                raise ValueError(f"word_mask must be [batch, frames] = {(videos.size(0), T)}, got {tuple(word_mask.shape)}")
            wm = word_mask.to(device=videos.device, dtype=torch.float32).contiguous()
        outs = _LrwFunction.apply(self.cls_token, self, st, videos.float().contiguous(), audio_tokens, labels.contiguous(),
                                   torch.is_grad_enabled(), wm)
        loss_category, loss_audio, acc = outs
        loss_total = loss_category + loss_audio * self.lambda_audio
        return {
            "loss_total": loss_total,
            "loss_category": loss_category,
            "loss_audio": loss_audio,
            "accuracy_top1": acc[0],
            "accuracy_top5": acc[1],
        }


    def prepare_batch(self, videos, audio_tokens, labels, word_mask):
        T = videos.size(2)
        A = self.audio_alignment
        if audio_tokens.size(1) < T * A:
            raise ValueError(f"audio_tokens has {audio_tokens.size(1)} steps, need >= {T * A}")
        hard = labels.dtype in (torch.int64, torch.int32)
        wm = word_mask
        if self.use_wb:
            if word_mask.shape != (videos.size(0), T):
                raise ValueError(f"word_mask must be [batch, frames] = {(videos.size(0), T)}, got {tuple(word_mask.shape)}")
            wm = word_mask.to(device=videos.device, dtype=torch.float32).contiguous()
        return (videos.float().contiguous(), audio_tokens[:, : T * A].contiguous(), (labels.long() if hard else labels.float()).contiguous(), wm)

    def _loss_weights(self) -> tuple[float, ...]:
        return (1.0, self.lambda_audio)

    def grad_store_spans(self, offsets: dict, phys: dict) -> list:
        if self.encoder_type != "huggingface":
            return []
        names = [(n, 1) for n, s, k in self._specs if k == "conv" and len(s) == 4]
        for i in range(self.layers):
            p = f"encoder.encoder.layer.{i}"
            names += [(f"{p}.attention.self.query.weight", 3), (f"{p}.attention.output.dense.weight", 1), (f"{p}.intermediate.dense.weight", 1),
                      (f"{p}.output.dense.weight", 1)]
        names += [("audio_projection.weight", 1), ("category_classifier.weight", 1)]
        spans = []
        for n, mult in names:
            o, numel, shape = offsets[n]
            if tuple(phys[n]) != tuple(shape):
                continue
            if mult == 3:
                kv = [offsets[n.replace("query", w)] for w in ("key", "value")]
                if [e[0] for e in kv] != [o + numel, o + 2 * numel] or any(tuple(phys[n.replace("query", w)]) != tuple(e[2]) for w, e in zip(("key", "value"), kv)):
                    continue
            spans.append((o, o + mult * numel))
        return spans

    def train_step_direct(self, videos, audio_tokens, labels, word_mask) -> dict[str, torch.Tensor]:
        _require_device(videos)
        st = self.store()
        self.direct_constants(videos.device)
        ctx = _NoAutogradCtx()
        self._metrics_on_side = True
        try:
            loss_category, loss_audio, acc = _LrwFunction.forward(ctx, self.cls_token, self, st, videos, audio_tokens, labels, True,
                                                                  word_mask if self.use_wb else None)
        finally:
            self._metrics_on_side = False
        if self._side.enabled:
            box: dict = {}
            self._side.run(lambda: box.__setitem__("t", ops.lincomb2(loss_category, loss_audio, self.lambda_audio)), loss_category, loss_audio)
            loss_total = box["t"]
        else:
            loss_total = ops.lincomb2(loss_category, loss_audio, self.lambda_audio)
        _LrwFunction.backward(ctx, *self._g_consts, None)
        return {"loss_total": loss_total, "loss_category": loss_category, "loss_audio": loss_audio, "accuracy_top1": acc[0],
                "accuracy_top5": acc[1]}


Model = TransformerLightningModule


class _ParamStore:

    def __init__(self, model, device: torch.device):
        self.device = device
        specs = model._specs
        fwd_rank = model._fwd_rank
        decay = sorted([(n, s) for n, s, k in specs if len(s) >= 2], key=lambda e: fwd_rank(e[0]))
        nodecay = [(n, s) for n, s, k in specs if len(s) < 2]
        self.offsets: dict[str, tuple[int, int, tuple[int, ...]]] = {}
        self._side = getattr(model, "_side", None)
        self._vc: dict = {}
        off = 0
        phys = getattr(model, "_phys", {})
        self.phys: dict[str, tuple[int, ...]] = {n: tuple(phys.get(n, s)) for n, s, _ in specs}
        for n, s in decay + nodecay:
            numel = math.prod(self.phys[n])
            off = (off + 3) // 4 * 4
            self.offsets[n] = (off, numel, tuple(s))
            off += numel
            if (n, s) == decay[-1]:
                off = (off + 3) // 4 * 4
                self.decay_end = off
        self.numel = (off + 3) // 4 * 4
        first = (decay + nodecay)[0][0]
        self.sumsq_head = self.offsets[first][1] if first == getattr(model, "stem_name", "?") + ".0.weight" and self.offsets[first][1] % 4 == 0 else 0
        later = [self.offsets[n][0] for n, s in decay if fwd_rank(n) >= 2]
        self.front_end = min(later) if later else self.decay_end
        self.flat = torch.zeros(self.numel, dtype=torch.float32, device=device)
        self.grad = torch.zeros(self.numel, dtype=torch.float32, device=device)
        self.w16 = torch.zeros(self.numel, dtype=BF16, device=device)
        self._params: dict[str, nn.Parameter] = {}
        for n, s, kind in specs:
            p = _get(model, n)
            o, numel, shape = self.offsets[n]
            view = self._view(self.flat, n)
            view.copy_(p.data.to(device))
            p.data = view
            p.grad = self._view(self.grad, n)
            self._params[n] = p
        self.buffers = {n: _get(model, n) for n, _, _ in model._bspecs}
        for n, b in self.buffers.items():
            if b.device != device:
                raise RuntimeError("move the module to the GPU before the first forward (model.to('cuda'))")
        fbufs = [(n, b) for n, b in self.buffers.items() if b.is_floating_point()]
        self.bufflat = torch.empty(sum(b.numel() for _, b in fbufs), dtype=torch.float32, device=device)
        o = 0
        for n, b in fbufs:
            view = self.bufflat[o : o + b.numel()].view(b.shape)
            view.copy_(b)
            b.data = view
            o += b.numel()
        entries = []
        toff = 0
        self.t_offsets: dict[str, tuple[int, tuple[int, int, int]]] = {}

        def add_t(key: str, src_off: int, A: int, T: int, Bd: int):
            nonlocal toff
            Apad = (A + 63) // 64 * 64
            self.t_offsets[key] = (toff, (Bd, T, Apad))
            entries.append((src_off, toff, A, T, Bd, Apad))
            toff += Bd * T * Apad

        for n, s, kind in specs:
            if kind == "conv" and len(s) == 4:
                add_t(n, self.offsets[n][0], s[0], s[2] * s[3], s[1])
        self.n_entries_front = sum(1 for e in entries if e[0] < self.front_end)
        assert all(e[0] < self.front_end for e in entries[: self.n_entries_front]) and all(e[0] >= self.front_end for e in entries[self.n_entries_front:])
        for key, src_off, A, Bd in model._transposed_entries(self.offsets):
            add_t(key, src_off, A, 1, Bd)
        self.w16t = torch.zeros(max(toff, 1), dtype=BF16, device=device)
        import numpy as np

        tab = np.zeros(len(entries), dtype=np.dtype([("src", "<i8"), ("dst", "<i8"), ("A", "<i4"), ("T", "<i4"), ("Bd", "<i4"), ("Apad", "<i4")]))
        for i, e in enumerate(entries):
            tab[i] = e
        self.table = torch.from_numpy(tab.view(np.uint8).copy()).to(device)
        self.n_entries = len(entries)
        self.bn: dict[str, dict[str, torch.Tensor]] = {}
        for n, s, kind in specs:
            if kind == "norm_w" and (n + "").replace(".weight", ".running_mean") in self.buffers:
                C = s[0]
                base = n[: -len(".weight")]
                self.bn[base] = dict(
                    coef=torch.empty(3 * C, dtype=torch.float32, device=device),
                    mean=torch.empty(C, dtype=torch.float32, device=device),
                    rstd=torch.empty(C, dtype=torch.float32, device=device),
                )
        self.shadow_fresh = False
        self.generation = 0

    def owns(self, model) -> bool:
        lo, hi = self.flat.data_ptr(), self.flat.data_ptr() + self.flat.numel() * 4
        anchor = model._specs[0][0]
        blo, bhi = self.bufflat.data_ptr(), self.bufflat.data_ptr() + self.bufflat.numel() * 4
        bufs_ok = all(blo <= b.data_ptr() < bhi for b in self.buffers.values() if b.is_floating_point() and b.numel())
        return bufs_ok and all(lo <= p.data_ptr() < hi for p in self._params.values()) and _get(model, anchor) is self._params[anchor]

    def _view(self, flat: torch.Tensor, name: str) -> torch.Tensor:
        o, numel, shape = self.offsets[name]
        seg = flat[o : o + numel]
        if len(shape) == 4:
            return seg.view(shape[0], shape[2], shape[3], shape[1]).permute(0, 3, 1, 2)
        ph = self.phys[name]
        if ph != shape:
            return seg.view(ph)[tuple(slice(0, d) for d in shape)]
        return seg.view(shape)

    def p32(self, name: str) -> torch.Tensor:
        v = self._vc.get(("p", name))
        if v is None:
            o, n, _ = self.offsets[name]
            v = self._vc[("p", name)] = self.flat[o : o + n]
        return v

    def g32(self, name: str) -> torch.Tensor:
        v = self._vc.get(("g", name))
        if v is None:
            o, n, _ = self.offsets[name]
            v = self._vc[("g", name)] = self.grad[o : o + n]
        return v

    def s16(self, name: str, numel: Optional[int] = None) -> torch.Tensor:
        v = self._vc.get(("s", name, numel))
        if v is None:
            o, n, _ = self.offsets[name]
            v = self._vc[("s", name, numel)] = self.w16[o : o + (numel or n)]
        return v

    def t16(self, key: str) -> torch.Tensor:
        v = self._vc.get(("t", key))
        if v is None:
            o, (Bd, T, Apad) = self.t_offsets[key]
            v = self._vc[("t", key)] = self.w16t[o : o + Bd * T * Apad].view(Bd, T, Apad)
        return v

    def span(self, name: str, numel: Optional[int] = None) -> tuple[int, int]:
        o, n, _ = self.offsets[name]
        return o, o + (numel or n)

    def refresh_shadows(self) -> None:
        if self._side is not None:
            self._side.join()
        self.generation += 1
        ops.cast_bf16(self.flat, self.w16)
        ops.transpose_shadows(self.flat, self.w16, self.w16t, self.table, self.n_entries)

    def zero_grad(self) -> None:
        if self.__dict__.get("grad_clean", False):
            self.grad_clean = False
            return
        ops.memset(self.grad, 0)

    def rebind_grads(self) -> None:
        for n, p in self._params.items():
            g = p.grad
            if g is None or g.data_ptr() != self.grad.data_ptr() + self.offsets[n][0] * 4:
                p.grad = self._view(self.grad, n)


def _bn_stats(st: _ParamStore, base: str, training: bool, count: int, stats):
    ws = st.bn[base]
    if training:
        ops.bn_finalize(stats, ws["mean"].numel(), count, ws["mean"], ws["rstd"], st.buffers[f"{base}.running_mean"],
                        st.buffers[f"{base}.running_var"], st.buffers[f"{base}.num_batches_tracked"])
    else:
        ops.bn_eval_prepare(st.buffers[f"{base}.running_mean"], st.buffers[f"{base}.running_var"], ws["mean"], ws["rstd"])
    return ws["mean"], ws["rstd"]


def _conv_bn(st: _ParamStore, tape: dict, x: torch.Tensor, conv: str, bn: str, k: int, stride: int, pad: int, training: bool,
             res: Optional[torch.Tensor], act: int) -> torch.Tensor:
    o, n, shape = st.offsets[f"{conv}.weight"]
    w16 = st.w16[o : o + n].view(shape[0], k, k, shape[1])
    c, stats = ops.conv2d_fwd(x, w16, k, stride, pad, want_stats=training)
    mean, rstd = _bn_stats(st, bn, training, c.numel() // c.shape[-1], stats)
    y = ops.bn_act_fwd(c, res, mean, rstd, st.p32(f"{bn}.weight"), st.p32(f"{bn}.bias"), act)
    tape[conv] = dict(x=x, c=c, y=y, mean=mean, rstd=rstd, k=k, stride=stride, pad=pad, act=act, bn=bn, res=res)
    return y


def _trunk_blocks(model):
    for prefix, inp, planes, stride, down in resnet_block_specs():
        yield model.trunk_name + prefix[len("resnet"):], inp, planes, stride, down


def _frontend_forward(model, st: "_ParamStore", tape: dict, videos: torch.Tensor, training: bool) -> torch.Tensor:
    B, _, T, H, W = videos.shape
    N = B * T
    sc, sb, act = model.stem_name + ".0", model.stem_name + ".1", model.trunk_act
    c, stats = ops.stem_conv_fwd(videos, st.p32(f"{sc}.weight"), want_stats=training)
    mean, rstd = _bn_stats(st, sb, training, c.numel() // 64, stats)
    if training:
        x, amax, xwin = ops.stem_bn_gelu_pool_fwd(c, mean, rstd, st.p32(f"{sb}.weight"), st.p32(f"{sb}.bias"), model.stem_act, want_win=True)
    else:
        (x, amax), xwin = ops.stem_bn_gelu_pool_fwd(c, mean, rstd, st.p32(f"{sb}.weight"), st.p32(f"{sb}.bias"), model.stem_act), None
    tape["stem"] = dict(videos=videos, c=c, amax=amax, xwin=xwin, mean=mean, rstd=rstd, pooled_shape=tuple(x.shape))
    for prefix, inp, planes, stride, down in _trunk_blocks(model):
        xin = x
        if down and training and model._side.enabled:
            box: dict = {}
            model._side.run(lambda xin=xin, prefix=prefix, stride=stride: box.__setitem__(
                "idt", _conv_bn(st, tape, xin, f"{prefix}.downsample.0", f"{prefix}.downsample.1", 1, stride, 0, training, None, 0)), xin)
            o1 = _conv_bn(st, tape, xin, f"{prefix}.conv1", f"{prefix}.bn1", 3, stride, 1, training, None, act)
            model._side.join()
            idt = box["idt"]
        else:
            o1 = _conv_bn(st, tape, xin, f"{prefix}.conv1", f"{prefix}.bn1", 3, stride, 1, training, None, act)
            idt = _conv_bn(st, tape, xin, f"{prefix}.downsample.0", f"{prefix}.downsample.1", 1, stride, 0, training, None, 0) if down else xin
        x = _conv_bn(st, tape, o1, f"{prefix}.conv2", f"{prefix}.bn2", 3, 1, 1, training, idt, act)
    tape["trunk_out_shape"] = tuple(x.shape)
    return ops.avgpool_fwd(x)


def _frontend_backward(model, st: "_ParamStore", tape: dict, dfeats: torch.Tensor) -> None:
    use_tr = model.use_tr
    act = model.trunk_act
    dx = ops.avgpool_bwd(dfeats, tape["trunk_out_shape"])
    fused = act in (1, 2) and ops.BN_BWD_FUSED
    dx_stats = None
    blocks = list(_trunk_blocks(model))
    rec = tape.get("_record_grads")
    for bi in range(len(blocks) - 1, -1, -1):
        prefix, inp, planes, stride, down = blocks[bi]
        if rec is not None:
            rec[prefix] = (dx.clone(), dx_stats is not None)
        t2 = tape[f"{prefix}.conv2"]
        ws2 = st.bn[t2["bn"]]
        if dx_stats is not None:
            dres = dx
            dc2 = ops.bn_bwd_from_stats(dx, t2["c"], t2["mean"], t2["rstd"], st.p32(f"{t2['bn']}.weight"), dx_stats, ws2["coef"],
                                        st.g32(f"{t2['bn']}.weight"), st.g32(f"{t2['bn']}.bias"))
        else:
            dc2, dres = ops.bn_act_bwd(dx, t2["y"], t2["c"], t2["mean"], t2["rstd"], st.p32(f"{t2['bn']}.weight"), ws2["coef"],
                                       st.g32(f"{t2['bn']}.weight"), st.g32(f"{t2['bn']}.bias"), act, True,
                                       beta=st.p32(f"{t2['bn']}.bias"), res=t2["res"])
        _conv_wgrad(model, st, f"{prefix}.conv2", t2, dc2, use_tr)
        t1 = tape[f"{prefix}.conv1"]
        ws1 = st.bn[t1["bn"]]
        w2t = st.t16(f"{prefix}.conv2.weight").view(planes, 3, 3, planes)
        if fused:
            g1, st1 = ops.conv2d_dgrad_bn(dc2, w2t, 3, 1, 1, t2["x"].shape[1:3], None, None, t1["c"], t1["mean"], t1["rstd"],
                                          st.p32(f"{t1['bn']}.weight"), st.p32(f"{t1['bn']}.bias"), act)
            dc1 = ops.bn_bwd_from_stats(g1, t1["c"], t1["mean"], t1["rstd"], st.p32(f"{t1['bn']}.weight"), st1, ws1["coef"],
                                        st.g32(f"{t1['bn']}.weight"), st.g32(f"{t1['bn']}.bias"))
        else:
            do1 = ops.conv2d_dgrad(dc2, w2t, 3, 1, 1, t2["x"].shape[1:3])
            dc1, _ = ops.bn_act_bwd(do1, t1["y"], t1["c"], t1["mean"], t1["rstd"], st.p32(f"{t1['bn']}.weight"), ws1["coef"],
                                    st.g32(f"{t1['bn']}.weight"), st.g32(f"{t1['bn']}.bias"), act, False, beta=st.p32(f"{t1['bn']}.bias"))
        _conv_wgrad(model, st, f"{prefix}.conv1", t1, dc1, use_tr)
        in_hw = t1["x"].shape[1:3]
        w1t = st.t16(f"{prefix}.conv1.weight").view(inp, 3, 3, planes)
        tp = tape[f"{blocks[bi - 1][0]}.conv2"] if fused and bi > 0 else None
        if tp is not None:
            tp_aux = tp["y"] if act == 1 else tp["res"]
            tp_gb = (st.p32(f"{tp['bn']}.weight"), st.p32(f"{tp['bn']}.bias"), act)
        if down:
            td = tape[f"{prefix}.downsample.0"]
            wsd = st.bn[td["bn"]]
            dcd, _ = ops.bn_act_bwd(dres, None, td["c"], td["mean"], td["rstd"], st.p32(f"{td['bn']}.weight"), wsd["coef"],
                                    st.g32(f"{td['bn']}.weight"), st.g32(f"{td['bn']}.bias"), 0, False)
            _conv_wgrad(model, st, f"{prefix}.downsample.0", td, dcd, use_tr)
            wdt = st.t16(f"{prefix}.downsample.0.weight").view(inp, 1, 1, planes)
            dxd = ops.conv2d_dgrad(dcd, wdt, 1, stride, 0, in_hw)
            if tp is not None:
                dx, dx_stats = ops.conv2d_dgrad_bn(dc1, w1t, 3, stride, 1, in_hw, dxd, tp_aux, tp["c"], tp["mean"], tp["rstd"], *tp_gb)
            else:
                dx, dx_stats = ops.conv2d_dgrad(dc1, w1t, 3, stride, 1, in_hw, addend=dxd), None
        elif tp is not None:
            dx, dx_stats = ops.conv2d_dgrad_bn(dc1, w1t, 3, stride, 1, in_hw, dres, tp_aux, tp["c"], tp["mean"], tp["rstd"], *tp_gb)
        else:
            dx, dx_stats = ops.conv2d_dgrad(dc1, w1t, 3, stride, 1, in_hw, addend=dres), None
        _ready(model, st, f"{prefix}.conv1.weight")
    ts = tape["stem"]
    if rec is not None:
        rec["stem"] = (dx.clone(), False)
    sc, sb = model.stem_name + ".0", model.stem_name + ".1"
    ws = st.bn[sb]
    fused = ts.get("xwin") is not None and use_tr and ops.stem_bwd_wgrad_ok(ts["videos"])
    dconv = ops.stem_bn_gelu_pool_bwd(dx, ts["amax"], ts["c"], ts["mean"], ts["rstd"], st.p32(f"{sb}.weight"), st.p32(f"{sb}.bias"),
                                      ws["coef"], st.g32(f"{sb}.weight"), st.g32(f"{sb}.bias"), model.stem_act, xwin=ts.get("xwin"),
                                      want_dx=not fused)
    if fused:
        _flush_deferred(model)
        model._side.join()
        early = getattr(model, "_early_sumsq", None)
        if early is not None and st.sumsq_head:
            with ops.window_group("tail"):
                model._side.run(lambda: ops.grad_sumsq_parts(st.grad, st.sumsq_head, st.numel - st.sumsq_head, early, 0, ops.SUMSQ_PARTS - 1))
            st.sumsq_tail_done = True
        ops.stem_bwd_wgrad(ts["videos"], dconv, ts["amax"], ts["c"], ts["mean"], ts["rstd"], ws["coef"], st.g32(f"{sc}.weight"))
    else:
        ops.stem_conv_wgrad(ts["videos"], dconv, st.g32(f"{sc}.weight"), use_tr)
    _flush_deferred(model)
    model._side.join()
    _ready(model, st, None)


_ABLATE: frozenset = frozenset()


def _conv_wgrad(model, st: "_ParamStore", conv: str, t: dict, dc: torch.Tensor, use_tr: bool) -> None:
    if "conv_wgrad" in _ABLATE:
        return
    model._side.run(lambda: ops.conv2d_wgrad(t["x"], dc, st.g32(f"{conv}.weight"), t["k"], t["stride"], t["pad"], use_tr), dc)


def _lin_wgrad(model, x, dy, gw, gb, rows: int, K: int, N: int, x_pitch: int, dy_pitch: int) -> None:
    if "lin_wgrad" in _ABLATE:
        return
    group = getattr(model, "_wg_group", None)
    if group is not None:
        group.append(dict(x=x, dy=dy, dw=gw, db=gb, rows=rows, K=K, N=N, x_pitch=x_pitch, dy_pitch=dy_pitch))
        return
    model._side.run(lambda: ops.linear_wgrad(x, dy, gw, rows=rows, K=K, N=N, x_pitch=x_pitch, dy_pitch=dy_pitch, db=gb), x, dy, small=True)


def _flush_lin_wgrads(model) -> None:
    group, model._wg_group = model._wg_group, None
    if not group:
        return
    keep = [t for q in group for t in (q["x"], q["dy"])]
    if model._side.enabled:
        model._side.run(lambda: ops.linear_wgrad_group(group), *keep)
    else:
        ops.linear_wgrad_group(group)


def _defer_list(model) -> Optional[list]:
    if not (model._side.enabled or model._side.enabled_small):
        return None
    d = model.__dict__.get("_deferred")
    if d is None:
        d = model.__dict__["_deferred"] = []
    return d


def _flush_deferred(model) -> None:
    d = model.__dict__.get("_deferred")
    if d:
        fns, keep = [f for f, _ in d], [k for _, k in d]
        d.clear()
        model._side.run(lambda: ops.run_deferred(fns), *keep, small=True)


def _ready(model, st: "_ParamStore", name: Optional[str]) -> None:
    _flush_deferred(model)
    if model.grad_ready_hook is not None:
        hook, lo = model.grad_ready_hook, (0 if name is None else st.offsets[name][0])
        ops.host_callback(lambda: hook(lo))


def _encoder_forward(model: TransformerLightningModule, st: _ParamStore, tape: dict, feats: torch.Tensor, B: int, T: int) -> torch.Tensor:
    D, S, H = model.dim, T + 1, model.heads
    R = B * S
    pos = st.p32("encoder.embeddings.position_embeddings.weight")
    type0 = st.p32("encoder.embeddings.token_type_embeddings.weight")
    d_in, d_out = model._d("emb.in", "emb"), model._d("emb.out")
    s0, x, mean0, rstd0 = ops.embed_ln_fwd(feats, st.p32("cls_token"), pos, type0, st.p32("encoder.embeddings.LayerNorm.weight"),
                                           st.p32("encoder.embeddings.LayerNorm.bias"), B, S, D, model.ln_eps, drop_in=d_in, drop_out=d_out)
    tape["emb"] = dict(sum=s0, mean=mean0, rstd=rstd0, d_in=d_in, d_out=d_out)
    if ops.enc_fused_ok(D, H, model.inter, S):
        return _encoder_forward_fused(model, st, tape, x, B, S)
    for i in range(model.layers):
        p = f"encoder.encoder.layer.{i}"
        wqkv = st.s16(f"{p}.attention.self.query.weight", 3 * D * D)
        bqkv = st.flat[st.offsets[f"{p}.attention.self.query.bias"][0] :][: 3 * D]
        qkv, _ = ops.linear_fwd(x, wqkv, bqkv, rows=R, K=D, N=3 * D, x_pitch=D)
        dpr, dao, dfo = model._d(f"enc.{i}.attn.probs", "attn"), model._d(f"enc.{i}.attn.out"), model._d(f"enc.{i}.ff.out")
        ctx, probs = ops.mha_fwd(qkv, 3 * D, qkv[:, D:], qkv[:, 2 * D:], 3 * D, B=B, H=H, Lq=S, Lk=S, drop=dpr)
        ao, _ = ops.linear_fwd(ctx, st.s16(f"{p}.attention.output.dense.weight"), st.p32(f"{p}.attention.output.dense.bias"),
                               rows=R, K=D, N=D, x_pitch=D, drop=dao)
        x1, m1, r1 = ops.add_ln_fwd(ao, x, st.p32(f"{p}.attention.output.LayerNorm.weight"), st.p32(f"{p}.attention.output.LayerNorm.bias"), model.ln_eps)
        hg, z = ops.linear_fwd(x1, st.s16(f"{p}.intermediate.dense.weight"), st.p32(f"{p}.intermediate.dense.bias"),
                               rows=R, K=D, N=model.inter, x_pitch=D, gelu=True)
        f, _ = ops.linear_fwd(hg, st.s16(f"{p}.output.dense.weight"), st.p32(f"{p}.output.dense.bias"), rows=R, K=model.inter, N=D,
                              x_pitch=model.inter, drop=dfo)
        x2, m2, r2 = ops.add_ln_fwd(f, x1, st.p32(f"{p}.output.LayerNorm.weight"), st.p32(f"{p}.output.LayerNorm.bias"), model.ln_eps)
        tape[p] = dict(x=x, qkv=qkv, ctx=ctx, probs=probs, ao=ao, x1=x1, m1=m1, r1=r1, z=z, hg=hg, f=f, m2=m2, r2=r2, dpr=dpr, dao=dao, dfo=dfo)
        x = x2
    return x


def _encoder_forward_fused(model: TransformerLightningModule, st: _ParamStore, tape: dict, x: torch.Tensor, B: int, S: int) -> torch.Tensor:
    D, H, I, Lc = model.dim, model.heads, model.inter, model.layers
    R = B * S
    dev = x.device
    ldp = ops.probs_pitch(S)
    qkv = torch.empty((Lc, R, 3 * D), dtype=BF16, device=dev)
    probs = torch.empty((Lc, B * H, S, ldp), dtype=BF16, device=dev)
    act = torch.empty((5, Lc, R, D), dtype=BF16, device=dev)
    zz = torch.empty((2, Lc, R, I), dtype=BF16, device=dev)
    stat = torch.empty((4, Lc, R), dtype=torch.float32, device=dev)
    training = model.training
    recs = []
    xin = x
    for i in range(Lc):
        p = f"encoder.encoder.layer.{i}"
        dpr, dao, dfo = model._d(f"enc.{i}.attn.probs", "attn"), model._d(f"enc.{i}.attn.out"), model._d(f"enc.{i}.ff.out")
        rec = dict(
            wqkv=st.s16(f"{p}.attention.self.query.weight", 3 * D * D), wo=st.s16(f"{p}.attention.output.dense.weight"),
            w1=st.s16(f"{p}.intermediate.dense.weight"), w2=st.s16(f"{p}.output.dense.weight"),
            bqkv=st.flat[st.offsets[f"{p}.attention.self.query.bias"][0]:][: 3 * D], bo=st.p32(f"{p}.attention.output.dense.bias"),
            b1=st.p32(f"{p}.intermediate.dense.bias"), b2=st.p32(f"{p}.output.dense.bias"),
            g1=st.p32(f"{p}.attention.output.LayerNorm.weight"), be1=st.p32(f"{p}.attention.output.LayerNorm.bias"),
            g2=st.p32(f"{p}.output.LayerNorm.weight"), be2=st.p32(f"{p}.output.LayerNorm.bias"),
            qkv=qkv[i], probs=probs[i], ctx=act[0, i], ao=act[1, i], x1=act[2, i], z=zz[0, i], hg=zz[1, i], f=act[3, i], xout=act[4, i],
            m1=stat[0, i], r1=stat[1, i], m2=stat[2, i], r2=stat[3, i],
            site_probs=model._sites[f"enc.{i}.attn.probs"], site_ao=model._sites[f"enc.{i}.attn.out"], site_fo=model._sites[f"enc.{i}.ff.out"])
        recs.append(rec)
        tape[p] = dict(x=xin, qkv=rec["qkv"], ctx=rec["ctx"], probs=rec["probs"], ao=rec["ao"], x1=rec["x1"], m1=rec["m1"], r1=rec["r1"], z=rec["z"],
                       hg=rec["hg"], f=rec["f"], m2=rec["m2"], r2=rec["r2"], dpr=dpr, dao=dao, dfo=dfo)
        xin = rec["xout"]
    on = training and (model.drop_p > 0.0 or model.attn_drop_p > 0.0)
    ops.enc_fwd(x, recs, B, S, model.ln_eps, model._drop_word if on else None, model.drop_p if training else 0.0,
                model.attn_drop_p if training else 0.0)
    return xin


def _encoder_layers_backward_fused(model: TransformerLightningModule, st: _ParamStore, tape: dict, dh: torch.Tensor, B: int, S: int,
                                   defer: Optional[list]) -> torch.Tensor:
    D, H, I, Lc = model.dim, model.heads, model.inter, model.layers
    R = B * S
    dev = dh.device
    t0 = tape["encoder.encoder.layer.0"]
    hidden_drop = t0["dfo"] is not None or t0["dao"] is not None
    act = torch.empty((6 if hidden_drop else 4, Lc, R, D), dtype=BF16, device=dev)
    dz = torch.empty((Lc, R, I), dtype=BF16, device=dev)
    dqkv = torch.empty((Lc, R, 3 * D), dtype=BF16, device=dev)
    part = torch.empty((Lc, 2, B, 2 * D), dtype=torch.float32, device=dev)
    recs = []
    for i in range(Lc):
        p = f"encoder.encoder.layer.{i}"
        t = tape[p]
        recs.append(dict(
            w2t=st.t16(f"{p}.output.dense.weight"), w1t=st.t16(f"{p}.intermediate.dense.weight"),
            wot=st.t16(f"{p}.attention.output.dense.weight"), wqkvt=st.t16(f"{p}.qkv"),
            g1=st.p32(f"{p}.attention.output.LayerNorm.weight"), g2=st.p32(f"{p}.output.LayerNorm.weight"),
            f=t["f"], x1=t["x1"], ao=t["ao"], xin=t["x"], z=t["z"], qkv=t["qkv"], probs=t["probs"], m1=t["m1"], r1=t["r1"], m2=t["m2"], r2=t["r2"],
            ds2=act[0, i], dx1=act[1, i], ds1=act[2, i], dx=act[3, i], df=act[4, i] if hidden_drop else act[0, i],
            dao=act[5, i] if hidden_drop else act[2, i], dz=dz[i], dqkv=dqkv[i], part1=part[i, 0], part2=part[i, 1],
            site_probs=model._sites[f"enc.{i}.attn.probs"], site_ao=model._sites[f"enc.{i}.attn.out"], site_fo=model._sites[f"enc.{i}.ff.out"]))
    on = hidden_drop or t0["dpr"] is not None
    ops.enc_bwd(dh, recs, B, S, model._drop_word if on else None, model.drop_p if hidden_drop else 0.0,
                model.attn_drop_p if t0["dpr"] is not None else 0.0)

    def ln_grads(rows, name):
        gw, gb = st.g32(f"{name}.weight"), st.g32(f"{name}.bias")
        if defer is None:
            ops.colsum_rows(rows, B, 2 * D, gw, D, gb, D)
        else:
            defer.append((lambda: ops.colsum_rows(rows, B, 2 * D, gw, D, gb, D), rows))

    for i in reversed(range(Lc)):
        p = f"encoder.encoder.layer.{i}"
        t, q = tape[p], recs[i]
        ln_grads(q["part2"], f"{p}.output.LayerNorm")
        _lin_wgrad(model, t["hg"], q["df"], st.g32(f"{p}.output.dense.weight"), st.g32(f"{p}.output.dense.bias"), R, I, D, I, D)
        _lin_wgrad(model, t["x1"], q["dz"], st.g32(f"{p}.intermediate.dense.weight"), st.g32(f"{p}.intermediate.dense.bias"), R, D, I, D, I)
        ln_grads(q["part1"], f"{p}.attention.output.LayerNorm")
        _lin_wgrad(model, t["ctx"], q["dao"], st.g32(f"{p}.attention.output.dense.weight"), st.g32(f"{p}.attention.output.dense.bias"), R, D, D, D, D)
        gq = st.grad[st.offsets[f"{p}.attention.self.query.weight"][0]:][: 3 * D * D]
        gqb = st.grad[st.offsets[f"{p}.attention.self.query.bias"][0]:][: 3 * D]
        _lin_wgrad(model, t["x"], q["dqkv"], gq, gqb, R, D, 3 * D, D, 3 * D)
        _flush_deferred(model)
        if getattr(model, "_wg_group", None) is None:
            _ready(model, st, f"{p}.attention.self.query.weight")
        elif i > 0:
            _flush_lin_wgrads(model)
            model._wg_group = []
            _ready(model, st, f"{p}.attention.self.query.weight")
    return recs[0]["dx"]


def _encoder_backward(model: TransformerLightningModule, st: _ParamStore, tape: dict, dh: torch.Tensor, B: int, T: int) -> torch.Tensor:
    D, S, H, I = model.dim, T + 1, model.heads, model.inter
    R = B * S
    use_tr = model.use_tr
    dx = dh
    defer = _defer_list(model)

    fused = ops.ENC_BWD_FUSED and ops.enc_fused_ok(D, H, I, S) and model.layers <= 8
    if fused:
        dx = _encoder_layers_backward_fused(model, st, tape, dh, B, S, defer)
    for i in reversed(range(0 if fused else model.layers)):
        p = f"encoder.encoder.layer.{i}"
        t = tape[p]
        ds2 = ops.add_ln_bwd(dx, t["f"], t["x1"], st.p32(f"{p}.output.LayerNorm.weight"), t["m2"], t["r2"],
                             st.g32(f"{p}.output.LayerNorm.weight"), st.g32(f"{p}.output.LayerNorm.bias"), defer=defer)
        df = ds2 if t["dfo"] is None else ops.scale_bf16(ds2, 1.0, drop=t["dfo"])
        _lin_wgrad(model, t["hg"], df, st.g32(f"{p}.output.dense.weight"), st.g32(f"{p}.output.dense.bias"), R, I, D, I, D)
        dhg = ops.linear_dgrad(df, st.t16(f"{p}.output.dense.weight"), rows=R, N=D, K=I, dy_pitch=D)
        dz = ops.bias_act_bwd(dhg, t["z"], st.g32(f"{p}.intermediate.dense.bias"), R=R, N=I, n_valid=I, ld=I, defer=defer)
        _lin_wgrad(model, t["x1"], dz, st.g32(f"{p}.intermediate.dense.weight"), None, R, D, I, D, I)
        dx1 = ops.linear_dgrad(dz, st.t16(f"{p}.intermediate.dense.weight"), rows=R, N=I, K=D, dy_pitch=I, addend=ds2)
        ds1 = ops.add_ln_bwd(dx1, t["ao"], t["x"], st.p32(f"{p}.attention.output.LayerNorm.weight"), t["m1"], t["r1"],
                             st.g32(f"{p}.attention.output.LayerNorm.weight"), st.g32(f"{p}.attention.output.LayerNorm.bias"), defer=defer)
        dao_ = ds1 if t["dao"] is None else ops.scale_bf16(ds1, 1.0, drop=t["dao"])
        _lin_wgrad(model, t["ctx"], dao_, st.g32(f"{p}.attention.output.dense.weight"), st.g32(f"{p}.attention.output.dense.bias"), R, D, D, D, D)
        dctx = ops.linear_dgrad(dao_, st.t16(f"{p}.attention.output.dense.weight"), rows=R, N=D, K=D, dy_pitch=D)
        qkv = t["qkv"]
        dqkv = torch.empty_like(qkv)
        ops.mha_bwd(dctx, qkv, 3 * D, qkv[:, D:], qkv[:, 2 * D:], 3 * D, t["probs"], B=B, H=H, Lq=S, Lk=S, dq=dqkv, dq_pitch=3 * D,
                    dk=dqkv[:, D:], dv=dqkv[:, 2 * D:], dkv_pitch=3 * D, drop=t["dpr"])
        gq = st.grad[st.offsets[f"{p}.attention.self.query.weight"][0] :][: 3 * D * D]
        gqb = st.grad[st.offsets[f"{p}.attention.self.query.bias"][0] :][: 3 * D]
        _lin_wgrad(model, t["x"], dqkv, gq, gqb, R, D, 3 * D, D, 3 * D)
        dx = ops.linear_dgrad(dqkv, st.t16(f"{p}.qkv"), rows=R, N=3 * D, K=D, dy_pitch=3 * D, addend=ds1)
        _flush_deferred(model)
        if getattr(model, "_wg_group", None) is None:
            _ready(model, st, f"{p}.attention.self.query.weight")
        elif i > 0:
            _flush_lin_wgrads(model)
            model._wg_group = []
            _ready(model, st, f"{p}.attention.self.query.weight")
    if getattr(model, "_wg_group", None) is not None:
        _flush_lin_wgrads(model)
        _ready(model, st, "encoder.encoder.layer.0.attention.self.query.weight")
    te = tape["emb"]
    if te["d_out"] is not None:
        dx = ops.scale_bf16(dx, 1.0, drop=te["d_out"])
    ds0 = ops.add_ln_bwd(dx, te["sum"], None, st.p32("encoder.embeddings.LayerNorm.weight"), te["mean"], te["rstd"],
                         st.g32("encoder.embeddings.LayerNorm.weight"), st.g32("encoder.embeddings.LayerNorm.bias"), defer=defer)
    dfeats = ops.embed_bwd_scatter(ds0, st.g32("cls_token"), st.g32("encoder.embeddings.position_embeddings.weight"),
                                   st.g32("encoder.embeddings.token_type_embeddings.weight"), B, S, D, drop_in=te["d_in"])
    _ready(model, st, "cls_token")
    return dfeats


def _xt_skips(model) -> set:
    if not model.training or model.layer_drop_p <= 0.0:
        return set()
    if model.layer_skip_override is not None:
        return set(model.layer_skip_override)
    return {n for n in range(2 * model.layers) if model._layer_rng.random() < model.layer_drop_p}


def _xt_block_fwd(model, st: _ParamStore, tape: dict, x: torch.Tensor, n: int, B: int, S: int, tab: torch.Tensor, nrot: int) -> torch.Tensor:
    D, Dp, H, E = model.dim, model.dim_p, model.heads, model.attn_inner
    I, Ip, Up = model.inter, model.inter_p, model.glu_p
    R, i, b = B * S, n // 2, f"encoder.layers.{n}"
    h, inv = ops.rmsnorm_fwd(x, st.p32(f"{b}.0.0.g"), D, model.rms_eps)
    if n % 2 == 0:
        qkv, _ = ops.linear_fwd(h, st.s16(f"{b}.1.to_q.weight", 3 * E * Dp), None, rows=R, K=Dp, N=3 * E, x_pitch=Dp)
        ops.rotary_(qkv, tab, S, nrot, 1)
        dpr = model._d(f"enc.{i}.attn.probs", "attn")
        ctx, probs = ops.mha_fwd(qkv, 3 * E, qkv[:, E:], qkv[:, 2 * E:], 3 * E, B=B, H=H, Lq=S, Lk=S, drop=dpr)
        x1, _ = ops.linear_fwd(ctx, st.s16(f"{b}.1.to_out.weight"), None, rows=R, K=E, N=Dp, x_pitch=E, addend=x)
        tape[b] = dict(x=x, h=h, inv=inv, qkv=qkv, ctx=ctx, probs=probs, dpr=dpr)
    else:
        u, _ = ops.linear_fwd(h, st.s16(f"{b}.1.ff.0.proj.weight"), st.p32(f"{b}.1.ff.0.proj.bias"), rows=R, K=Dp, N=Up, x_pitch=Dp)
        dff = model._d(f"enc.{i}.ff.hidden")
        y = ops.geglu_fwd(u, I, Ip, drop=dff)
        x1, _ = ops.linear_fwd(y, st.s16(f"{b}.1.ff.3.weight"), st.p32(f"{b}.1.ff.3.bias"), rows=R, K=Ip, N=Dp, x_pitch=Ip, addend=x)
        tape[b] = dict(x=x, h=h, inv=inv, u=u, y=y, dff=dff)
    return x1


def _xt_block_bwd(model, st: _ParamStore, tape: dict, dx: torch.Tensor, n: int, B: int, S: int) -> torch.Tensor:
    D, Dp, H, E = model.dim, model.dim_p, model.heads, model.attn_inner
    I, Ip, Up = model.inter, model.inter_p, model.glu_p
    R, b, t, tx = B * S, f"encoder.layers.{n}", tape[f"encoder.layers.{n}"], tape["xt"]
    if n % 2 == 1:
        _lin_wgrad(model, t["y"], dx, st.g32(f"{b}.1.ff.3.weight"), st.g32(f"{b}.1.ff.3.bias"), R, Ip, Dp, Ip, Dp)
        dy = ops.linear_dgrad(dx, st.t16(f"{b}.1.ff.3.weight"), rows=R, N=Dp, K=Ip, dy_pitch=Dp)
        du = ops.geglu_bwd(dy, t["u"], I, drop=t["dff"])
        _lin_wgrad(model, t["h"], du, st.g32(f"{b}.1.ff.0.proj.weight"), st.g32(f"{b}.1.ff.0.proj.bias"), R, Dp, Up, Dp, Up)
        dhn = ops.linear_dgrad(du, st.t16(f"{b}.1.ff.0.proj.weight"), rows=R, N=Up, K=Dp, dy_pitch=Up)
    else:
        _lin_wgrad(model, t["ctx"], dx, st.g32(f"{b}.1.to_out.weight"), None, R, E, Dp, E, Dp)
        dctx = ops.linear_dgrad(dx, st.t16(f"{b}.1.to_out.weight"), rows=R, N=Dp, K=E, dy_pitch=Dp)
# ... 192 lines not shown
```

### syncvsr_amd/ops.py

```python
from __future__ import annotations

import bisect
import ctypes
import os
import struct
from contextlib import contextmanager, nullcontext
from typing import Callable, Optional, Sequence

import torch

from . import _lib

BF16 = torch.bfloat16
BN_EPS = 1e-5
BN_MOMENTUM = 0.1
HALO_WGRAD = True


_DEV_INDEX: Optional[int] = None
STREAM_OVERRIDE: Optional[int] = None


def _stream() -> int:
    global _DEV_INDEX
# ... 209 lines not shown
        n = self.groups
        mask = (ctypes.c_uint8 * max(n, 1))()
        for g in skips:
            if not 0 <= g < n:
                raise ValueError(f"op group {g} is not in this step list ({n} groups)")
            mask[g] = 1
        _lib.check(self.lib.svsr_steplist_set_skips(self.handle, mask, n), "svsr_steplist_set_skips")

    def window_skips(self, zero: bool, tail: bool) -> set:
        if self.window is None:
            return set()
        return {g for g, run in zip(self.window, (zero, tail)) if not run}

    def would_issue(self, segment: int = -1) -> dict:
        counts = (ctypes.c_int64 * 4)()
        _lib.check(self.lib.svsr_steplist_dry_run(self.handle, int(segment), counts), "svsr_steplist_dry_run")
        return dict(zip(("calls", "waits", "memsets", "copies"), (int(c) for c in counts)))

    @property
    def last_issued(self) -> int:
        return int(self.lib.svsr_steplist_last_issued(self.handle))

    def add_callback(self, fn: Callable[[], None]) -> None:
        seg = self.lib.svsr_steplist_push_break(self.handle)
        if seg < 1:
            _lib.check(-seg if seg < 0 else 1001, "svsr_steplist_push_break")
        self.callbacks.setdefault(seg - 1, []).append(fn)

    @property
    def segments(self) -> int:
        return int(self.lib.svsr_steplist_segments(self.handle))

    @property
    def size(self) -> int:
        return int(self.lib.svsr_steplist_size(self.handle))

    def kept_bytes(self) -> int:
        seen: dict[int, int] = {}
        for t in self.keep:
            if torch.is_tensor(t) and t.is_cuda:
                s = t.untyped_storage()
                seen[s.data_ptr()] = s.nbytes()
        return sum(seen.values())

    def run(self) -> None:
        failed = ctypes.c_int(-1)
        run, h, cbs = self.lib.svsr_steplist_run, self.handle, self.callbacks
        if len(cbs) == 0:
            rc = run(h, -1, ctypes.byref(failed))
            if rc != 0:
                _lib.check(rc, f"svsr_steplist_run (op {failed.value})")
            return
        for k in range(self.segments):
            rc = run(h, k, ctypes.byref(failed))
            if rc != 0:
                _lib.check(rc, f"svsr_steplist_run (op {failed.value})")
            for fn in cbs.get(k, ()):
                fn()


_REC: Optional[StepRecorder] = None
_ALLOC_KEEP = ("empty", "empty_like")
_ALLOC_FORBID = ("zeros", "zeros_like", "ones", "ones_like", "full", "full_like")


@contextmanager
def recording(rec: StepRecorder):
    global _REC, PLAN_CACHE_PINNED
    if _REC is not None or _TIMING is not None:
        raise RuntimeError("nested recording / recording while per-launch event timing is on")
    saved = {n: getattr(torch, n) for n in _ALLOC_KEEP + _ALLOC_FORBID}

    def keeper(fn):
        def w(*a, **k):
            t = fn(*a, **k)
            rec.keep.append(t)
            return t
        return w

    def forbid(name):
        def w(*a, **k):
            raise RuntimeError(f"torch.{name} inside a recorded step launches a kernel the native step list does not hold (use ops.zeros)")
        return w

    for n in _ALLOC_KEEP:
        setattr(torch, n, keeper(saved[n]))
    for n in _ALLOC_FORBID:
        setattr(torch, n, forbid(n))
    _REC = rec
    rec.main_stream = _stream()
    PLAN_CACHE_PINNED = True
    try:
        yield rec
    finally:
        _REC = None
        for n, f in saved.items():
            setattr(torch, n, f)
        rec.closed = True


def active_recorder() -> Optional[StepRecorder]:
    return _REC


def layer_groups() -> Optional[StepRecorder]:
    return _REC if _REC is not None and _REC.layer_groups else None


def window_group(which: str):
    rec = _REC
    if rec is None or rec.window is None:
        return nullcontext()
    return rec.group(rec.window[("zero", "tail").index(which)])


def host_callback(fn: Callable[[], None]) -> None:
    fn()
    if _REC is not None:
        _REC.add_callback(fn)


def stream_wait(waiter: torch.cuda.Stream, signaller: torch.cuda.Stream) -> None:
    if _REC is None:
        waiter.wait_stream(signaller)
        return
    w, s = waiter.cuda_stream, signaller.cuda_stream
    _lib.check(_lib.load().svsr_stream_wait(w, s), "svsr_stream_wait")
    _REC.wait(w, s)


def device_cus() -> int:
    return int(_lib.load().svsr_device_cus())


def shader_clock_mhz(blocks: int = 256, iters: int = 20000) -> float:
    out = torch.zeros(blocks * 2 + 1, dtype=torch.int64, device="cuda")
    _lib.check(_lib.load().svsr_clock_probe(_p(out), blocks, iters, _stream()), "svsr_clock_probe")
    torch.cuda.current_stream().synchronize()
    h = out[: blocks * 2].view(blocks, 2).sum(0).tolist()
    return 100.0 * h[0] / max(1, h[1])


def memset(t: torch.Tensor, value: int = 0) -> None:
    nbytes, stream = t.numel() * t.element_size(), _stream()
    if _REC is not None and _REC.append_only:
        _REC.memset(t.data_ptr(), value, nbytes, stream)
        return
    _lib.check(_lib.load().svsr_memset_async(t.data_ptr(), value, nbytes, stream), "svsr_memset_async")
    if _REC is not None:
        _REC.memset(t.data_ptr(), value, nbytes, stream)


GRAD_STORE = True
GRAD_FILL_NAN = False


class GradCoverage:

    def __init__(self, grad: torch.Tensor, spans):
        self.grad, self.base, self.numel = grad, grad.data_ptr(), grad.numel()
        self.spans, self.holes = self.plan(spans, self.numel)
        self._planned = set(self.spans)
        self._los = [lo for lo, _ in self.spans]
        self._ranges = (ctypes.c_int64 * (2 * max(1, len(self.holes))))(*[v for h in self.holes for v in h])
        self._touched: set = set()

    @staticmethod
    def plan(spans, numel: int) -> tuple:
        spans = sorted({(int(lo), int(hi)) for lo, hi in spans})
        holes, at = [], 0
        for lo, hi in spans:
            if lo % 4 or lo < at or hi <= lo or hi > numel:
                raise ValueError(f"gradient span [{lo}, {hi}) is misaligned, empty, overlaps its neighbour or leaves the buffer")
            if lo > at:
                holes.append((at // 4 * 4, lo))
            at = hi
        if numel % 4:
            raise ValueError("the flat gradient buffer is a multiple of 4 elements")
        if at < numel:
            holes.append((at // 4 * 4, numel))
        return spans, holes

    def hole_elems(self) -> int:
        return sum(hi - lo for lo, hi in self.holes)

    def fill(self) -> None:
        if GRAD_FILL_NAN:
            _call("svsr_fill_f32", self.base, self.numel, float("nan"), _stream())
        if self.holes:
            _call("svsr_fill_ranges", self.base, self.numel, self._ranges, len(self.holes), 0, _stream())

    def begin(self) -> None:
        global _COVER
        self._touched = set()
        _COVER = self

    def touch(self, ptr: int, n: int) -> int:
        lo = (ptr - self.base) // 4
        key = (lo, lo + n)
        if key not in self._planned:
            i = bisect.bisect_left(self._los, lo)
            run, at = [], lo
            while i + len(run) < len(self.spans) and self.spans[i + len(run)][0] == at and self.spans[i + len(run)][1] <= lo + n:
                at = self.spans[i + len(run)][1]
                run.append(self.spans[i + len(run)])
            if len(run) > 1 and at == lo + n:
                done = [s in self._touched for s in run]
                if all(done):
                    return 1
                if any(done):
                    raise RuntimeError(f"a weight-gradient launch writes elements [{lo}, {lo + n}) of the gradient buffer: some of the first-touch spans "
                                       f"it covers were written earlier in this step, others not — it can neither add nor store")
                self._touched.update(run)
                return 0
            i = bisect.bisect_right(self._los, lo)
            for s in self.spans[max(0, i - 1) : i + 1]:
                if s[0] < lo + n and lo < s[1]:
                    raise RuntimeError(f"a weight-gradient launch writes elements [{lo}, {lo + n}) of the gradient buffer, part of the first-touch span "
                                       f"[{s[0]}, {s[1]}) but not all of it: the span is not zero-filled, so the launch can neither add nor store")
            return 1
        if key in self._touched:
            return 1
        self._touched.add(key)
        return 0

    def end(self) -> list:
        global _COVER
        if _COVER is self:
            _COVER = None
        return sorted(self._planned - self._touched)


_COVER: Optional[GradCoverage] = None


def _grad_add(dw: torch.Tensor, n: int) -> int:
    return 1 if _COVER is None else _COVER.touch(dw.data_ptr(), n)


def end_grad_coverage() -> list:
    return [] if _COVER is None else _COVER.end()


def zeros(shape, dtype, device) -> torch.Tensor:
    t = torch.empty(shape, dtype=dtype, device=device)
    memset(t, 0)
    return t


def word_add(word: torch.Tensor, delta: int) -> None:
    _call("svsr_word_add", _p(word), int(delta), _stream())


def lincomb2(a: torch.Tensor, b: torch.Tensor, wb: float) -> torch.Tensor:
    out = torch.empty((), dtype=torch.float32, device=a.device)
    _call("svsr_lincomb2", _p(a), _p(b), float(wb), _p(out), _stream())
    return out


def lincomb3_ratio(a, wa: float, b, wb: float, c, wc: float, num=None, den=None):
    out0 = torch.empty((), dtype=torch.float32, device=a.device)
    out1 = torch.empty((), dtype=torch.float32, device=a.device) if num is not None else None
    _call("svsr_lincomb3_ratio", _p(a), float(wa), _p(b), float(wb), _p(c), float(wc), _p(out0), _p(num), _p(den), _p(out1), _stream())
    return out0, out1


def _call(name: str, *args, label: Optional[str] = None, flops: float = 0.0, nbytes: float = 0.0) -> None:
    if _REC is not None and _REC.append_only:
        _REC.call(name, args)
        return
    timing = _TIMING
    if timing is not None:
        s, e = torch.cuda.Event(enable_timing=True), torch.cuda.Event(enable_timing=True)
        s.record()
    rc = getattr(_lib.load(), name)(*args)
    if timing is not None:
        e.record()
        timing.setdefault(label or name, []).append((s, e, flops, nbytes))
    if rc != 0:
        _lib.check(rc, name)
    if _REC is not None:
        _REC.call(name, args)


class Plan:
    __slots__ = ("words", "meta", "bm", "bn", "ns", "tiles", "label")

    def __init__(self, builder: str, *args):
        fn = getattr(_lib.load(), builder)
        meta = (ctypes.c_int * 8)()
        n = fn(*args, None, 0, meta)
        if n <= 0:
            _lib.check(-n if n < 0 else 1001, builder)
        host = torch.empty(n, dtype=torch.int32)
        n2 = fn(*args, host.data_ptr(), n, meta)
        if n2 != n:
            _lib.check(1001, builder)
        self.words = host.to("cuda")
        self.meta = meta
        self.bm, self.bn, self.ns, self.tiles = int(meta[0]), int(meta[1]), int(meta[2]), int(meta[3])
        self.label = f"k_igemm_p8<{self.bm},{self.bn},{self.ns}>" if self.bm == 256 else f"k_igemm_fwd_glds<{self.bm},{self.bn},{self.ns}>"


def conv_plan(mode: int, N: int, H: int, W: int, Co_out: int, k: int, stride: int, pad: int) -> Plan:
    key = ("conv", mode, N, H, W, Co_out, k, stride, pad)
    pl = _PLAN_CACHE.get(key)
    if pl is None:
        pl = _PLAN_CACHE[key] = Plan("svsr_conv_plan", mode, N, H, W, Co_out, k, stride, pad)
    return pl


def rows_plan(Nimg: int, P: int, src0: int, dst0: int, Co_out: int, Ci: Optional[int] = None) -> Plan:
    key = ("rows", Nimg, P, src0, dst0, Co_out)
    pl = _PLAN_CACHE.get(key)
    if pl is None:
        pl = _PLAN_CACHE[key] = Plan("svsr_rows_plan", Nimg, P, src0, dst0, Co_out)
    return pl


class WPlan:
    __slots__ = ("words", "meta", "bc", "splits", "part_floats", "label")

    def __init__(self, builder: str, *args):
        fn = getattr(_lib.load(), builder)
        meta = (ctypes.c_int * 8)()
        nfl = ctypes.c_int64(0)
        n = fn(*args, None, 0, meta, ctypes.byref(nfl))
        if n <= 0:
            _lib.check(-n if n < 0 else 1001, builder)
        host = torch.empty(n, dtype=torch.int32)
        if fn(*args, host.data_ptr(), n, meta, ctypes.byref(nfl)) != n:
            _lib.check(1001, builder)
        self.words = host.to("cuda")
        self.meta = meta
        self.bc, self.splits, self.part_floats = int(meta[0]), int(meta[2]), int(nfl.value)
        self.label = f"k_igemm_wgrad<{self.bc},{int(meta[1])}>"


def wgrad_conv_plan(N: int, H: int, W: int, Ci: int, Co: int, k: int, stride: int, pad: int) -> WPlan:
    key = ("wconv", N, H, W, Ci, Co, k, stride, pad)
    pl = _PLAN_CACHE.get(key)
    if pl is None:
        pl = _PLAN_CACHE[key] = WPlan("svsr_wgrad_plan", N, H, W, Ci, Co, k, stride, pad)
    return pl


def wgrad_rows_plan(Nimg: int, P: int, src0: int, dst0: int, Ci: int, Co: int, has_bias: bool) -> WPlan:
    key = ("wrows", Nimg, P, src0, dst0, Ci, Co, bool(has_bias))
    pl = _PLAN_CACHE.get(key)
    if pl is None:
        pl = _PLAN_CACHE[key] = WPlan("svsr_wgrad_rows_plan", Nimg, P, src0, dst0, Ci, Co, int(has_bias))
    return pl


def igemm_fwd(plan: Plan, inp: torch.Tensor, wt: torch.Tensor, out: torch.Tensor, *, Nimg: int, in_pix: int, Ci: int, in_pitch: int,
              Co: int, out_pix: int, out_pitch: int, wt_taps: int = 1, bias: Optional[torch.Tensor] = None,
              addend: Optional[torch.Tensor] = None, want_stats: bool = False, gelu: bool = False,
              out_pre: Optional[torch.Tensor] = None, out_f32: bool = False, relu: bool = False, alpha: float = 1.0, drop=None,
              flops: float = 0.0):
    stats = st = None
    if want_stats:
        stats = scratch(plan.tiles * 2 * Co)
        st = (stats, plan.tiles)
    label = plan.label
    if _TIMING is not None and plan.bm == 64 and int(_lib.load().svsr_igemm_fwd_kgroups(plan.meta, Ci, Co, 0)) == 2:
        label = label[:-1] + ",2>"
    _call("svsr_igemm_fwd", _p(inp), _p(wt), _p(out), _p(out_pre), _p(bias), _p(addend), _p(stats), plan.words.data_ptr(), plan.meta,
          Nimg, in_pix, Ci, in_pitch, Co, out_pix, out_pitch, wt_taps, 1 if gelu else (2 if relu else 0), int(out_f32), float(alpha),
          *_drop(drop), _stream(), label=label, flops=flops)
    return st


def igemm_wgrad(plan: WPlan, x: torch.Tensor, dyp: torch.Tensor, dw: torch.Tensor, *, Nimg: int, in_pix: int, Ci: int, in_pitch: int,
                Co: int, out_pix: int, out_pitch: int, wt_taps: int = 1, db: Optional[torch.Tensor] = None, flops: float = 0.0,
                mode: Optional[int] = None) -> None:
    part = scratch(plan.part_floats) if plan.part_floats else None
    if mode is None:
        mode = _grad_add(dw, Co * wt_taps * Ci) | 2
    _call("svsr_igemm_wgrad_v2", _p(x), _p(dyp), _p(dw), _p(db), plan.words.data_ptr(), plan.meta, Nimg, in_pix, Ci, in_pitch, Co, out_pix,
          out_pitch, wt_taps, _p(part), plan.part_floats, mode, _stream(), label=plan.label, flops=flops)


class _WgradProblem(ctypes.Structure):
    _fields_ = [("x", ctypes.c_void_p), ("dy", ctypes.c_void_p), ("dw", ctypes.c_void_p), ("dbias", ctypes.c_void_p), ("plan_dev", ctypes.c_void_p),
                ("meta", ctypes.c_void_p), ("Nimg", ctypes.c_int), ("in_pix", ctypes.c_int), ("Ci", ctypes.c_int), ("in_pitch", ctypes.c_int),
                ("Co", ctypes.c_int), ("out_pix", ctypes.c_int), ("out_pitch", ctypes.c_int), ("wt_taps", ctypes.c_int)]


_WG_TABLES: dict = {}


def _group_table(nbytes: int, device) -> torch.Tensor:
    key = (str(device), _stream())
    t = _WG_TABLES.get(key)
    if t is None or t.numel() < nbytes:
        if t is not None:
            _SCRATCH_KEEP.append(t)
        t = _WG_TABLES[key] = torch.empty(max(nbytes, 1 << 16), dtype=torch.uint8, device=device)
    return t


def linear_wgrad_group(problems: Sequence[dict]) -> None:
    grouped, keep, modes = [], [], []
    for q in problems:
        rows, K, N, seq, db = q["rows"], q["K"], q["N"], q.get("seq"), q.get("db")
        if seq is None:
            plan, geo = wgrad_rows_plan(rows, 1, 0, 0, K, N, db is not None), (rows, 1, 1)
        else:
            S, s0, n = seq
            plan, geo = wgrad_rows_plan(rows // n, n, s0, 0, K, N, db is not None), (rows // n, S, n)
        if not (plan.bc == 64 and int(plan.meta[1]) == 3 and plan.splits == 1):
            linear_wgrad(q["x"], q["dy"], q["dw"], rows=rows, K=K, N=N, x_pitch=q["x_pitch"], dy_pitch=q["dy_pitch"], seq=seq, db=db)
            continue
        grouped.append(_WgradProblem(_p(q["x"]), _p(q["dy"]), _p(q["dw"]), _p(db), plan.words.data_ptr(), ctypes.addressof(plan.meta),
                                     geo[0], geo[1], K, q["x_pitch"], N, geo[2], q["dy_pitch"], 1))
        keep.append(plan)
        modes.append(_grad_add(q["dw"], N * K) | 2)
    if not grouped:
        return
    arr = (_WgradProblem * len(grouped))(*grouped)
    nbytes = int(_lib.load().svsr_igemm_wgrad_group_bytes(len(grouped)))
    table = _group_table(nbytes, problems[0]["x"].device)
    flops = sum(2.0 * q["rows"] * q["K"] * q["N"] for q in problems)
    _call("svsr_igemm_wgrad_group_v2", arr, (ctypes.c_int * len(modes))(*modes), len(grouped), _p(table), nbytes, _stream(),
          label="k_igemm_wgrad_group<64,3>", flops=flops)


def conv_out_size(n: int, k: int, stride: int, pad: int) -> int:
    return (n + 2 * pad - k) // stride + 1


def conv2d_fwd(x: torch.Tensor, w16: torch.Tensor, k: int, stride: int, pad: int, want_stats: bool = False):
    N, H, W, Ci = x.shape
    Co = w16.shape[0]
    Ho, Wo = conv_out_size(H, k, stride, pad), conv_out_size(W, k, stride, pad)
    out = torch.empty((N, Ho, Wo, Co), dtype=BF16, device=x.device)
    if _c64_ok(Ci, Co, k, stride, pad, W):
        return out, conv3x3_c64(x, w16, out, None, want_stats, _conv_taps(k, pad))
    st = igemm_fwd(conv_plan(0, N, H, W, Co, k, stride, pad), x, w16, out, Nimg=N, in_pix=H * W, Ci=Ci, in_pitch=Ci, Co=Co,
                   out_pix=Ho * Wo, out_pitch=Co, wt_taps=k * k, want_stats=want_stats, flops=2.0 * N * Ho * Wo * Co * Ci * k * k)
    return out, st


_TAPS: dict = {}


def _conv_taps(k: int, pad: int) -> tuple:
    t = _TAPS.get((k, pad))
    if t is None:
        t = _TAPS[(k, pad)] = tuple((kh - pad, kw - pad, kh * k + kw) for kh in range(k) for kw in range(k))
    return t


C64_CONV = True


_C64_TABS: dict = {}


def c64_pixtab(N: int, H: int, W: int, device) -> torch.Tensor:
    key = (N, H, W, str(device))
    t = _C64_TABS.get(key)
    if t is None:
        lib = _lib.load()
        n = int(lib.svsr_conv3x3_c64_pixtab(N, H, W, None, 0))
        if n <= 0:
            raise _lib.SvsrError(f"svsr_conv3x3_c64_pixtab({N}, {H}, {W}) failed ({n})")
        host = torch.empty(n, dtype=torch.int32)
        got = int(lib.svsr_conv3x3_c64_pixtab(N, H, W, host.data_ptr(), n))
        if got != n:
            raise _lib.SvsrError(f"svsr_conv3x3_c64_pixtab wrote {got} of {n} entries")
        t = _C64_TABS[key] = host.to(device)
    return t


def _c64_ok(Ci: int, Co: int, k: int, stride: int, pad: int, W: int) -> bool:
    return C64_CONV and Ci == 64 and Co == 64 and k == 3 and stride == 1 and pad == 1 and W <= 29


def conv3x3_c64(x: torch.Tensor, wt: torch.Tensor, out: torch.Tensor, addend: Optional[torch.Tensor], want_stats: bool,
                taps: Sequence[tuple[int, int, int]]):
    N, H, W, _ = x.shape
    dy, dx, tw = zip(*taps)
    stats = st = None
    if want_stats:
        rows = _query("svsr_conv3x3_c64_stat_rows", N, H, W)[0]
        stats = scratch(rows * 2 * 64)
        st = (stats, rows)
    _call("svsr_conv3x3_c64", _p(x), _p(wt), _p(out), _p(addend), _p(stats), N, H, W, _ints(dy), _ints(dx), _ints(tw), _p(c64_pixtab(N, H, W, x.device)), _stream(),
          label="k_conv3x3_c64", flops=2.0 * N * H * W * 64 * 64 * 9)
    return st


def conv2d_dgrad(dy: torch.Tensor, w16t: torch.Tensor, k: int, stride: int, pad: int, in_hw: tuple[int, int],
                 addend: Optional[torch.Tensor] = None) -> torch.Tensor:
    N, Ho, Wo, Co = dy.shape
    Ci = w16t.shape[0]
    H, W = in_hw
    dx = torch.empty((N, H, W, Ci), dtype=BF16, device=dy.device) if addend is None else addend
    if stride == 1 and _c64_ok(Ci, Co, k, stride, pad, W):
        taps = tuple((pad - kh, pad - kw, kh * k + kw) for kh in range(k) for kw in range(k))
        conv3x3_c64(dy, w16t, dx, addend, False, taps)
        return dx
    igemm_fwd(conv_plan(1 if addend is None else 2, N, H, W, Ci, k, stride, pad), dy, w16t, dx, Nimg=N, in_pix=Ho * Wo, Ci=Co, in_pitch=Co, Co=Ci, out_pix=H * W,
              out_pitch=Ci, wt_taps=k * k, addend=addend, flops=2.0 * N * Ho * Wo * Co * Ci * k * k)
    return dx


BN_BWD_FUSED = True


def conv2d_dgrad_bn(dy: torch.Tensor, w16t: torch.Tensor, k: int, stride: int, pad: int, in_hw: tuple[int, int],
                    addend: Optional[torch.Tensor], y: Optional[torch.Tensor], x: torch.Tensor, mean: torch.Tensor, rstd: torch.Tensor,
                    gamma: Optional[torch.Tensor] = None, beta: Optional[torch.Tensor] = None, act: int = 1):
    N, Ho, Wo, Co = dy.shape
    Ci = w16t.shape[0]
    H, W = in_hw
    if x.shape != (N, H, W, Ci) or not x.is_contiguous() or (y is not None and (y.shape != x.shape or not y.is_contiguous())):
        raise ValueError("conv2d_dgrad_bn: y / x must be contiguous tensors with the geometry of the result")
    if (y is None or act == 2) and (gamma is None or beta is None):
        raise ValueError("conv2d_dgrad_bn: y=None / act=2 need gamma and beta")
    g = torch.empty((N, H, W, Ci), dtype=BF16, device=dy.device) if addend is None else addend
    if stride == 1 and _c64_ok(Ci, Co, k, stride, pad, W):
        taps = tuple((pad - kh, pad - kw, kh * k + kw) for kh in range(k) for kw in range(k))
        tdy, tdx, tw = zip(*taps)
        rows = _query("svsr_conv3x3_c64_stat_rows", N, H, W)[0]
        stats = scratch(rows * 2 * 64)
        _call("svsr_conv3x3_c64_dgrad_bn", _p(dy), _p(w16t), _p(g), _p(addend), _p(stats), N, H, W, _ints(tdy), _ints(tdx), _ints(tw),
              _p(y), _p(x), _p(mean), _p(rstd), _p(gamma), _p(beta), act, _p(c64_pixtab(N, H, W, dy.device)), _stream(), label="k_conv3x3_c64+bn", flops=2.0 * N * H * W * 64 * 64 * 9)
        return g, (stats, rows)
    plan = conv_plan(1, N, H, W, Ci, k, stride, pad)
    stats = scratch(plan.tiles * 2 * Ci)
    _call("svsr_igemm_dgrad_bn", _p(dy), _p(w16t), _p(g), _p(addend), _p(stats), plan.words.data_ptr(), plan.meta, N, Ho * Wo, Co, Co, Ci,
          H * W, Ci, k * k, _p(y), _p(x), _p(mean), _p(rstd), _p(gamma), _p(beta), act, _stream(), label=plan.label + "+bn", flops=2.0 * N * Ho * Wo * Co * Ci * k * k)
    return g, (stats, plan.tiles)


def bn_bwd_from_stats(g, x, mean, rstd, gamma, stats, coef, dgamma, dbeta) -> torch.Tensor:
    part, rows = stats
    C = x.shape[-1]
    dx = torch.empty_like(x)
    _call("svsr_bn_bwd_from_stats", _p(g), _p(x), _p(mean), _p(rstd), _p(gamma), _p(part), rows, _p(coef), _p(dgamma), _p(dbeta), _p(dx),
          x.numel() // C, C, _stream())
    return dx


def conv2d_wgrad(x: torch.Tensor, dy: torch.Tensor, dw: torch.Tensor, k: int, stride: int, pad: int, use_tr: bool = True, mode: Optional[int] = None) -> None:
    N, H, W, Ci = x.shape
    _, Ho, Wo, Co = dy.shape
    if HALO_WGRAD and use_tr and k == 3 and stride == 1 and pad == 1 and W <= 29 and H * W >= 100 and Ci % 64 == 0 and Co % 64 == 0:
        _, nfl = _query("svsr_conv3x3_wgrad_plan", N, H, W, Ci, Co)
        part = scratch(nfl) if nfl else None
        _call("svsr_conv3x3_wgrad_v2", _p(x), _p(dy), _p(dw), N, H, W, Ci, Co, _p(part), nfl, _grad_add(dw, Co * 9 * Ci) if mode is None else mode & 1, _stream(),
              label="k_wgrad3x3_halo", flops=2.0 * N * H * W * Co * Ci * 9)
        return
    igemm_wgrad(wgrad_conv_plan(N, H, W, Ci, Co, k, stride, pad), x, dy, dw, Nimg=N, in_pix=H * W, Ci=Ci, in_pitch=Ci, Co=Co,
                out_pix=Ho * Wo, out_pitch=Co, wt_taps=k * k, flops=2.0 * N * Ho * Wo * Co * Ci * k * k, mode=mode)


def halo_wgrad_ok(x: torch.Tensor, dy: torch.Tensor, k: int, stride: int, pad: int) -> bool:
    N, H, W, Ci = x.shape
    Co = dy.shape[-1]
    return HALO_WGRAD and k == 3 and stride == 1 and pad == 1 and W <= 29 and H * W >= 100 and Ci % 64 == 0 and Co % 64 == 0


def linear_fwd(x: torch.Tensor, w16: torch.Tensor, bias: Optional[torch.Tensor], *, rows: int, K: int, N: int, x_pitch: int,
               out: Optional[torch.Tensor] = None, out_pitch: Optional[int] = None, gelu: bool = False,
               out_f32: bool = False, addend: Optional[torch.Tensor] = None,
               seq: Optional[tuple[int, int, int]] = None, relu: bool = False, alpha: float = 1.0,
               drop=None) -> tuple[torch.Tensor, Optional[torch.Tensor]]:
    out_pitch = out_pitch or N
    if out is None:
        out = torch.empty((rows, out_pitch), dtype=torch.float32 if out_f32 else BF16, device=x.device)
    pre = torch.empty_like(out) if gelu else None
    if seq is None:
        plan, geo = rows_plan(rows, 1, 0, 0, N, None if (gelu or out_f32 or out_pitch % 8) else K), dict(Nimg=rows, in_pix=1, out_pix=1)
    else:
        S, s0, n = seq
        plan, geo = rows_plan(rows // n, n, s0, 0, N), dict(Nimg=rows // n, in_pix=S, out_pix=n)
    igemm_fwd(plan, x, w16, out, Ci=K, in_pitch=x_pitch, Co=N, out_pitch=out_pitch, bias=bias, addend=addend, gelu=gelu, out_pre=pre,
              out_f32=out_f32, relu=relu, alpha=alpha, drop=drop, flops=2.0 * rows * N * K, **geo)
    return out, pre


def linear_dgrad(dy: torch.Tensor, w16t: torch.Tensor, *, rows: int, N: int, K: int, dy_pitch: int, out: Optional[torch.Tensor] = None,
                 addend: Optional[torch.Tensor] = None, seq: Optional[tuple[int, int, int]] = None, alpha: float = 1.0,
                 drop=None) -> torch.Tensor:
    Np = w16t.shape[-1]
    if seq is None:
        if out is None:
            out = torch.empty((rows, K), dtype=BF16, device=dy.device)
        plan, geo = rows_plan(rows, 1, 0, 0, K, Np), dict(Nimg=rows, in_pix=1, out_pix=1)
    else:
        S, s0, n = seq
        assert out is not None
        plan, geo = rows_plan(rows // n, n, 0, s0, K), dict(Nimg=rows // n, in_pix=n, out_pix=S)
    igemm_fwd(plan, dy, w16t, out, Ci=Np, in_pitch=dy_pitch, Co=K, out_pitch=K, addend=addend, alpha=alpha, drop=drop,
              flops=2.0 * rows * N * K, **geo)
    return out


def linear_dgrad_bn(dy: torch.Tensor, w16t: torch.Tensor, *, rows: int, N: int, K: int, dy_pitch: int, x: torch.Tensor, mean: torch.Tensor,
                    rstd: torch.Tensor, gamma: torch.Tensor, beta: torch.Tensor, act: int):
    Np = w16t.shape[-1]
    if x.shape != (rows, K) or not x.is_contiguous():
        raise ValueError("linear_dgrad_bn: x must be a contiguous [rows, K] tensor")
    g = torch.empty((rows, K), dtype=BF16, device=dy.device)
    plan = rows_plan(rows, 1, 0, 0, K)
    stats = scratch(plan.tiles * 2 * K)
    _call("svsr_igemm_dgrad_bn", _p(dy), _p(w16t), _p(g), None, _p(stats), plan.words.data_ptr(), plan.meta, rows, 1, Np, dy_pitch, K,
          1, K, 1, None, _p(x), _p(mean), _p(rstd), _p(gamma), _p(beta), act, _stream(), label=plan.label + "+bn", flops=2.0 * rows * N * K)
    return g, (stats, plan.tiles)


_CONST_VECS: dict = {}


def linear_dgrad_relu(dy: torch.Tensor, w16t: torch.Tensor, *, rows: int, N: int, K: int, dy_pitch: int, y: torch.Tensor, gscale: float = 1.0):
    Np = w16t.shape[-1]
    if y.shape != (rows, K) or not y.is_contiguous():
        raise ValueError("linear_dgrad_relu: y must be a contiguous [rows, K] tensor")
    key = (str(dy.device), K)
    cv = _CONST_VECS.get(key)
    if cv is None:
        import numpy as np

        cv = _CONST_VECS[key] = tuple(torch.from_numpy(np.full(K, v, dtype=np.float32)).to(dy.device) for v in (0.0, 1.0))
    dz = torch.empty((rows, K), dtype=BF16, device=dy.device)
    plan = rows_plan(rows, 1, 0, 0, K)
    stats = torch.empty(plan.tiles * 2 * K, dtype=torch.float32, device=dy.device)
    _call("svsr_igemm_dgrad_relu", _p(dy), _p(w16t), _p(dz), _p(stats), plan.words.data_ptr(), plan.meta, rows, 1, Np, dy_pitch, K, 1, K, 1,
          _p(y), _p(cv[0]), _p(cv[1]), float(gscale), _stream(), label=plan.label + "+relu", flops=2.0 * rows * N * K)
    return dz, (stats, plan.tiles)


def linear_wgrad(x: torch.Tensor, dy: torch.Tensor, dw: torch.Tensor, *, rows: int, K: int, N: int, x_pitch: int, dy_pitch: int,
                 seq: Optional[tuple[int, int, int]] = None, use_tr: bool = True, db: Optional[torch.Tensor] = None, mode: Optional[int] = None) -> None:
    if seq is None:
        plan, geo = wgrad_rows_plan(rows, 1, 0, 0, K, N, db is not None), dict(Nimg=rows, in_pix=1, out_pix=1)
    else:
        S, s0, n = seq
        plan, geo = wgrad_rows_plan(rows // n, n, s0, 0, K, N, db is not None), dict(Nimg=rows // n, in_pix=S, out_pix=n)
    igemm_wgrad(plan, x, dy, dw, Ci=K, in_pitch=x_pitch, Co=N, out_pitch=dy_pitch, db=db, flops=2.0 * rows * N * K, mode=mode, **geo)


_STEM_WS: dict = {}


def stem_conv_fwd(videos: torch.Tensor, w: torch.Tensor, want_stats: bool = False):
    B, C, T, H, W = videos.shape
    assert C == 1 and videos.dtype == torch.float32 and videos.is_contiguous()
    out = torch.empty((B * T, H // 2, W // 2, 64), dtype=BF16, device=videos.device)
    stats = st = None
    if want_stats:
        rows = _query("svsr_stem_conv_fwd_stat_rows", B, T, H, W)[0]
        stats = scratch(rows * 2 * 64)
        st = (stats, rows)
    nws = _query("svsr_stem_conv_fwd_ws_bytes", B, T, H, W)[0]
    ws = None
    if nws:
        key = (videos.device, _stream())
        ws = _STEM_WS.get(key)
        if ws is None or ws.numel() < nws:
            if ws is not None:
                _SCRATCH_KEEP.append(ws)
            ws = _STEM_WS[key] = torch.empty(nws, dtype=torch.uint8, device=videos.device)
    _call("svsr_stem_conv_fwd", _p(videos), _p(w), _p(out), _p(stats), B, T, H, W, _p(ws), nws, _stream(),
          label="k_stem_conv_fwd", flops=2.0 * B * T * (H // 2) * (W // 2) * 64 * 245)
    return out, st


def stem_conv_wgrad(videos: torch.Tensor, dy: torch.Tensor, dw: torch.Tensor, use_tr: bool = True) -> None:
    B, _, T, H, W = videos.shape
    _, nfl = _query("svsr_stem_conv_wgrad_plan", B, T, H, W)
    _call("svsr_stem_conv_wgrad", _p(videos), _p(dy), _p(dw), B, T, H, W, int(use_tr), _p(scratch(nfl)), nfl, _stream(),
          label=f"k_stem_conv_wgrad<{'true' if use_tr else 'false'}>", flops=2.0 * B * T * (H // 2) * (W // 2) * 64 * 245)


ACT_NONE, ACT_RELU, ACT_GELU, ACT_SWISH = 0, 1, 1, 2


def stem_bn_gelu_pool_fwd(x: torch.Tensor, mean, rstd, gamma, beta, act: int = ACT_GELU, want_win: bool = False):
    N, Hc, Wc, C = x.shape
    Hp, Wp = (Hc - 1) // 2 + 1, (Wc - 1) // 2 + 1
    y = torch.empty((N, Hp, Wp, C), dtype=BF16, device=x.device)
    amax = torch.empty((N, Hp, Wp, C), dtype=torch.uint8, device=x.device)
    xwin = torch.empty((N, Hp, Wp, C), dtype=BF16, device=x.device) if want_win else None
    _call("svsr_stem_bn_act_pool_fwd", _p(x), _p(y), _p(amax), _p(mean), _p(rstd), _p(gamma), _p(beta), N, Hc, Wc, Hp, Wp, C, act, _p(xwin), _stream())
    return (y, amax, xwin) if want_win else (y, amax)


def stem_bn_gelu_pool_bwd(dpool, amax, x, mean, rstd, gamma, beta, coef, dgamma, dbeta, act: int = ACT_GELU, xwin=None, want_dx: bool = True):
    N, Hc, Wc, C = x.shape
    _, Hp, Wp, _ = dpool.shape
    assert want_dx or xwin is not None
    dx = torch.empty_like(x) if want_dx else None
    slots = scratch(_query("svsr_stem_bn_act_pool_bwd_rows", N, Hc, Wc, C)[0] * 2 * C)
    gpool = torch.empty_like(dpool) if xwin is not None else None
    _call("svsr_stem_bn_act_pool_bwd", _p(dpool), _p(amax), _p(x), _p(mean), _p(rstd), _p(gamma), _p(beta), _p(slots), _p(coef),
          _p(dgamma), _p(dbeta), _p(dx), N, Hc, Wc, Hp, Wp, C, act, _p(xwin), _p(gpool), _stream())
    return dx if want_dx else gpool


def stem_bwd_wgrad_ok(videos: torch.Tensor) -> bool:
    B, _, T, H, W = videos.shape
    return bool(_lib.load().svsr_stem_bwd_wgrad_ok(B, T, H, W))


def stem_bwd_wgrad(videos: torch.Tensor, gpool, amax, x, mean, rstd, coef, dw: torch.Tensor) -> None:
    B, _, T, H, W = videos.shape
    _, nfl = _query("svsr_stem_conv_wgrad_plan", B, T, H, W)
    _call("svsr_stem_bwd_wgrad", _p(videos), _p(gpool), _p(amax), _p(x), _p(mean), _p(rstd), _p(coef), _p(dw), B, T, H, W, _p(scratch(nfl)), nfl,
          _stream(), label="k_stem_bwd_wgrad", flops=2.0 * B * T * (H // 2) * (W // 2) * 64 * 245)


def bn_finalize(stats, C: int, count: int, mean, rstd, running_mean=None, running_var=None, nbt=None) -> None:
    part, rows = stats
    _call("svsr_bn_finalize", _p(part), rows, C, float(count), BN_EPS, BN_MOMENTUM, _p(mean), _p(rstd), _p(running_mean), _p(running_var),
          _p(nbt), _stream())


def bn_eval_prepare(running_mean, running_var, mean, rstd) -> None:
    _call("svsr_bn_eval_prepare", _p(running_mean), _p(running_var), running_mean.numel(), BN_EPS, _p(mean), _p(rstd), _stream())


def bn_act_fwd(x, res, mean, rstd, gamma, beta, act: int) -> torch.Tensor:
    C = x.shape[-1]
    y = torch.empty_like(x)
    _call("svsr_bn_act_fwd", _p(x), _p(res), _p(y), _p(mean), _p(rstd), _p(gamma), _p(beta), x.numel() // C, C, act, _stream())
    return y


def bn_act_bwd(dy, y, x, mean, rstd, gamma, coef, dgamma, dbeta, act: int, want_dres: bool, beta=None, res=None):
    C = x.shape[-1]
    dx = torch.empty_like(x)
    dres = torch.empty_like(x) if want_dres else None
    slots = scratch(_query("svsr_bn_act_bwd_rows", x.numel() // C, C)[0] * 2 * C)
    _call("svsr_bn_act_bwd", _p(dy), _p(y), _p(x), _p(mean), _p(rstd), _p(gamma), _p(slots), _p(coef), _p(dgamma), _p(dbeta), _p(dx),
          _p(dres), x.numel() // C, C, act, _p(beta), _p(res), _stream())
    return dx, dres


def avgpool_fwd(x: torch.Tensor) -> torch.Tensor:
    N, H, W, C = x.shape
    y = torch.empty((N, C), dtype=BF16, device=x.device)
    _call("svsr_avgpool_fwd", _p(x), _p(y), N, H * W, C, _stream())
    return y


def avgpool_bwd(dy: torch.Tensor, shape) -> torch.Tensor:
    N, H, W, C = shape
    dx = torch.empty(shape, dtype=BF16, device=dy.device)
    _call("svsr_avgpool_bwd", _p(dy), _p(dx), N, H * W, C, _stream())
    return dx


def add_ln_fwd(a, r, gamma, beta, eps: float):
    R, D = a.shape
    y = torch.empty_like(a)
    mean = torch.empty(R, dtype=torch.float32, device=a.device)
    rstd = torch.empty(R, dtype=torch.float32, device=a.device)
    _call("svsr_add_ln_fwd", _p(a), _p(r), _p(gamma), _p(beta), _p(y), _p(mean), _p(rstd), R, D, eps, _stream())
    return y, mean, rstd


def colsum_rows(part, rows: int, ld: int, out0, n0: int, out1=None, n1: int = 0) -> None:
    _call("svsr_colsum_rows", _p(part), rows, ld, _p(out0), n0, _p(out1), n1, 1, 1.0, _stream())


class _ColsumEntry(ctypes.Structure):
    _fields_ = [("ws", ctypes.c_void_p), ("out0", ctypes.c_void_p), ("out1", ctypes.c_void_p), ("ld", ctypes.c_int64), ("n0", ctypes.c_int64),
                ("n1", ctypes.c_int64), ("nrows", ctypes.c_int32), ("accumulate", ctypes.c_int32), ("scale", ctypes.c_float), ("reserved", ctypes.c_int32)]


COLSUM_MULTI = True


def _deferred_colsum(part, rows: int, ld: int, out0, n0: int, out1=None, n1: int = 0):
    f = lambda: colsum_rows(part, rows, ld, out0, n0, out1, n1)
    f.colsum = (part, rows, ld, out0, n0, out1, n1)
    return f


def run_deferred(fns) -> None:
    batch: list = []

    def flush():
        if len(batch) == 1:
            colsum_rows(*batch[0])
        elif batch:
            arr = (_ColsumEntry * len(batch))()
            for e, (part, rows, ld, out0, n0, out1, n1) in zip(arr, batch):
                e.ws, e.out0, e.out1, e.ld, e.n0, e.n1, e.nrows, e.accumulate, e.scale = _p(part), _p(out0), _p(out1), ld, n0, n1, rows, 1, 1.0
            _call("svsr_colsum_rows_multi", arr, len(batch), _stream())
        batch.clear()

    for f in fns:
        a = getattr(f, "colsum", None)
        if a is None or not COLSUM_MULTI:
            flush()
            f()
            continue
        outs = {_p(a[3]), _p(a[5])} - {None}
        if any(({_p(b[3]), _p(b[5])} - {None}) & outs for b in batch):
            flush()
        batch.append(a)
    flush()


def add_ln_bwd(dy, a, r, gamma, mean, rstd, dgamma, dbeta, addend=None, out=None, defer: Optional[list] = None, branch=None):
    R, D = a.shape
    ds = torch.empty_like(a) if out is None else out
    if defer is not None:
        rows = _query("svsr_add_ln_bwd_rows", R)[0]
        part = torch.empty(rows * 2 * D, dtype=torch.float32, device=a.device)
        if branch is not None:
            alpha, drop = branch
            ds2 = torch.empty_like(a)
            _call("svsr_add_ln_bwd_branch", _p(dy), _p(a), _p(r), _p(gamma), _p(mean), _p(rstd), _p(ds), R, D, _p(addend), _p(part), _p(ds2), float(alpha),
                  *_drop(drop), _stream())
            defer.append((_deferred_colsum(part, rows, 2 * D, dgamma, D, dbeta, D), part))
            return ds, ds2
        _call("svsr_add_ln_bwd_partials", _p(dy), _p(a), _p(r), _p(gamma), _p(mean), _p(rstd), _p(ds), R, D, _p(addend), _p(part), _stream())
        defer.append((_deferred_colsum(part, rows, 2 * D, dgamma, D, dbeta, D), part))
# ... 651 lines not shown
```

Measured before the change: 6543 clips/s.

## Fuse strided 1x1 downsample dgrad scatter into 3x3 dgrad epilogue via compact addend

Result: no change. 6584 clips/s, median of 6 (+0.6%).

```diff
diff --git a/include/syncvsr_hip.h b/include/syncvsr_hip.h
--- a/include/syncvsr_hip.h
+++ b/include/syncvsr_hip.h
@@ -51,6 +51,7 @@
 
 int svsr_conv_plan(int mode, int Nimg, int H, int W, int Co_out, int k, int stride, int pad, int* words, int cap_words, int* meta);
 int svsr_rows_plan(int Nimg, int P, int src0, int dst0, int Co_out, int* words, int cap_words, int* meta);
+int svsr_conv_plan_v2(int mode, int Nimg, int H, int W, int Co_out, int k, int stride, int pad, int addend_stride, int* words, int cap_words, int* meta);
 int svsr_igemm_fwd_kgroups(const int* meta, int Ci, int Co, int bn_epilogue);
 int svsr_igemm_fwd(const void* in, const void* wt, void* out, void* out_pre, const float* bias, const void* addend, float* stats, const int* plan_dev, const int* meta, int Nimg, int in_pix, int Ci, int in_pitch, int Co, int out_pix, int out_pitch, int wt_taps, int act, int out_f32, float alpha, const unsigned* drop_seed, unsigned drop_site, float drop_p, hipStream_t stream);
 
@@ -67,6 +68,8 @@
 int svsr_conv3x3_c64(const void* in, const void* wt, void* out, const void* addend, float* stats, int Nimg, int H, int W, const int* dy, const int* dx, const int* tw, const int* pixtab, hipStream_t stream);
 
 int svsr_igemm_dgrad_bn(const void* in, const void* wt, void* out, const void* addend, float* stats, const int* plan_dev, const int* meta, int Nimg, int in_pix, int Ci, int in_pitch, int Co, int out_pix, int out_pitch, int wt_taps, const void* y, const void* x, const float* mean, const float* rstd, const float* gamma, const float* beta, int act, hipStream_t stream);
+int svsr_igemm_dgrad_v2(const void* in, const void* wt, void* out, const void* addend, const int* plan_dev, const int* meta, int Nimg, int in_pix, int Ci, int in_pitch, int Co, int out_pix, int out_pitch, int wt_taps, int addend_stride, hipStream_t stream);
+int svsr_igemm_dgrad_bn_v2(const void* in, const void* wt, void* out, const void* addend, float* stats, const int* plan_dev, const int* meta, int Nimg, int in_pix, int Ci, int in_pitch, int Co, int out_pix, int out_pitch, int wt_taps, const void* y, const void* x, const float* mean, const float* rstd, const float* gamma, const float* beta, int act, int addend_stride, hipStream_t stream);
 int svsr_igemm_dgrad_relu(const void* in, const void* wt, void* out, float* stats, const int* plan_dev, const int* meta, int Nimg, int in_pix, int Ci, int in_pitch, int Co, int out_pix, int out_pitch, int wt_taps, const void* y, const float* zeros, const float* ones, float gscale, hipStream_t stream);
 int svsr_conv3x3_c64_dgrad_bn(const void* in, const void* wt, void* out, const void* addend, float* stats, int Nimg, int H, int W, const int* dy, const int* dx, const int* tw, const void* y, const void* x, const float* mean, const float* rstd, const float* gamma, const float* beta, int act, const int* pixtab, hipStream_t stream);
 int svsr_bn_bwd_from_stats(const void* g, const void* x, const float* mean, const float* rstd, const float* gamma, const float* stats, int nrows, float* coef, float* dgamma, float* dbeta, void* dx, int64_t npix, int C, hipStream_t stream);
diff --git a/syncvsr_amd/csrc/igemm_fwd.h b/syncvsr_amd/csrc/igemm_fwd.h
--- a/syncvsr_amd/csrc/igemm_fwd.h
+++ b/syncvsr_amd/csrc/igemm_fwd.h
@@ -22,6 +22,7 @@
     const float* bnb_gamma;
     const float* bnb_beta;
     int bnb_act;
+    int add_strided;
 };
 
 
diff --git a/syncvsr_amd/csrc/igemm_fwd.hip b/syncvsr_amd/csrc/igemm_fwd.hip
--- a/syncvsr_amd/csrc/igemm_fwd.hip
+++ b/syncvsr_amd/csrc/igemm_fwd.hip
@@ -12,9 +12,9 @@
 __device__ unsigned g_zero_page[64];
 
 
-template <int BM, int BN, int TM, int TN>
+template <int BM, int BN, int TM, int TN, bool SADD>
 __device__ __forceinline__ void igemm_epilogue(const IgemmFwdArgs& p, f32x16 (&acc)[TM][TN], unsigned char* smem_raw, const long* sRow,
-                                               int wm0, int wn0, int n0, int tid, bool active, int m_tile) {
+                                               const int* sAdd, int wm0, int wn0, int n0, int tid, bool active, int m_tile) {
     constexpr int WN = BN / 2;
     const int lane = tid & 63, wave = tid >> 6;
     float st_s[TN], st_q[TN];
@@ -79,7 +79,11 @@
                 const long o = (offs[i] >= 0 ? offs[i] : 0) + n;
                 x8[i] = *reinterpret_cast<const u32x4*>(p.bnb_x + o);
                 if (!from_x) y8[i] = *reinterpret_cast<const u32x4*>(p.bnb_y + o);
-                if (p.addend != nullptr) add8[i] = *reinterpret_cast<const u32x4*>(p.addend + o);
+                if (p.addend != nullptr) {
+                    if constexpr (!SADD) add8[i] = *reinterpret_cast<const u32x4*>(p.addend + o);
+                    else if (sAdd != nullptr) add8[i] = *reinterpret_cast<const u32x4*>(p.addend + (long)sAdd[rbase + RSTEP * i] * p.out_pitch + n);
+                    else add8[i] = u32x4{0u, 0u, 0u, 0u};
+                }
             }
 #pragma unroll
             for (int i = 0; i < ITERS; ++i) {
@@ -134,9 +138,18 @@
             hi[i] = *reinterpret_cast<const f32x4*>(sOut + r * BN + c8 * 8 + 4);
         }
         if (p.addend != nullptr) {
-#pragma unroll
-            for (int i = 0; i < ITERS; ++i)
-                add8[i] = *reinterpret_cast<const u32x4*>(p.addend + (offs[i] >= 0 ? offs[i] : 0) + n);
+            if constexpr (!SADD) {
+#pragma unroll
+                for (int i = 0; i < ITERS; ++i)
+                    add8[i] = *reinterpret_cast<const u32x4*>(p.addend + (offs[i] >= 0 ? offs[i] : 0) + n);
+            } else if (sAdd != nullptr) {
+#pragma unroll
+                for (int i = 0; i < ITERS; ++i)
+                    add8[i] = *reinterpret_cast<const u32x4*>(p.addend + (long)sAdd[rbase + RSTEP * i] * p.out_pitch + n);
+            } else {
+#pragma unroll
+                for (int i = 0; i < ITERS; ++i) add8[i] = u32x4{0u, 0u, 0u, 0u};
+            }
         }
         const unsigned key = p.drop.seed != nullptr ? drop_key(p.drop) : 0u;
 #pragma unroll
@@ -314,7 +327,7 @@
     if (j < 0) { n--; j += P; } else if (j >= P) { n++; j -= P; }
 }
 
-template <int BM, int BN, int NS, int KG = 1>
+template <int BM, int BN, int NS, int KG = 1, bool SADD = false>
 __global__ __launch_bounds__(256 * KG) void k_igemm_fwd_glds(const IgemmFwdArgs p) {
     constexpr int BK = 64;
     static_assert(NS >= 2 && (BM / 32 + BN / 32) * (NS - 2) <= 63, "vmcnt immediate is 6 bits");
@@ -326,6 +339,7 @@
     bf16_t* sStage = reinterpret_cast<bf16_t*>(smem_raw) + grp * NS * S_ELEMS;
     long* sRow = reinterpret_cast<long*>(reinterpret_cast<bf16_t*>(smem_raw) + KG * NS * S_ELEMS);
     int* sTap = reinterpret_cast<int*>(sRow + BM);
+    int* sAdd = sTap + 32;
 
     const int tid = threadIdx.x & 255, lane = tid & 63, wave = tid >> 6;
     const int wm0 = (wave >> 1) * WM, wn0 = (wave & 1) * WN;
@@ -347,7 +361,8 @@
     const int m0 = (bx - cw[3]) * BM;
     const int Mc = p.Nimg * P;
     const float inv_p = 1.0f / (float)P;
-    if (tid < 18) sTap[tid] = cw[4 + tid];
+    if (tid < (SADD ? 19 : 18)) sTap[tid] = cw[4 + tid];
+    const int add_tab = SADD ? cw[22] : 0, add_pix = SADD ? cw[23] : 0;
 
     const bf16_t* zero_src = reinterpret_cast<const bf16_t*>(g_zero_page) + slot * 8;
     const bf16_t* a_ptr[AR];
@@ -374,6 +389,7 @@
     for (int r = tid; r < BM; r += 256) {
         const int m = m0 + r;
         long off = -1;
+        int apix = 0;
         if (m < Mc) {
             if (identity) {
                 off = (long)m * p.out_pix * p.out_pitch;
@@ -381,9 +397,11 @@
                 int n, j;
                 split_row(m, P, inv_p, n, j);
                 off = ((long)n * p.out_pix + pos[2 * j + 1]) * p.out_pitch;
+                if (add_tab != 0) apix = n * add_pix + p.plan[add_tab + j];
             }
         }
         sRow[r] = off;
+        if (add_tab != 0) sAdd[r] = apix;
     }
     __syncthreads();
 
@@ -461,20 +479,29 @@
         }
         __syncthreads();
     }
-    igemm_epilogue<BM, BN, TM, TN>(p, acc, smem_raw, sRow, wm0, wn0, n0, tid, grp == 0, bx);
+    const int* sAddE = nullptr;
+    if constexpr (SADD) {
+        if (__builtin_amdgcn_readfirstlane(sTap[18]) != 0) sAddE = sAdd;
+    }
+    igemm_epilogue<BM, BN, TM, TN, SADD>(p, acc, smem_raw, sRow, sAddE, wm0, wn0, n0, tid, grp == 0, bx);
+}
+
+template <int BM, int BN, int NS, int KG, bool SADD>
+static int launch_glds_as(const IgemmFwdArgs& a, int gx, int gy, hipStream_t stream) {
+    const size_t lds = (size_t)KG * NS * (BM + BN) * 64 * sizeof(bf16_t) + (size_t)BM * sizeof(long) + 128 + (SADD ? (size_t)BM * sizeof(int) : 0);
+    static size_t attr_set = 0;
+    if (attr_set < lds) {
+        (void)hipFuncSetAttribute(reinterpret_cast<const void*>(k_igemm_fwd_glds<BM, BN, NS, KG, SADD>), hipFuncAttributeMaxDynamicSharedMemorySize, (int)lds);
+        attr_set = lds;
+    }
+    IgemmFwdArgs b = a;
+    hipLaunchKernelGGL((k_igemm_fwd_glds<BM, BN, NS, KG, SADD>), dim3(gx, gy), dim3(256 * KG), lds, stream, b);
+    return svsr_check_launch();
 }
 
 template <int BM, int BN, int NS, int KG = 1>
 static int launch_glds(const IgemmFwdArgs& a, int gx, int gy, hipStream_t stream) {
-    const size_t lds = (size_t)KG * NS * (BM + BN) * 64 * sizeof(bf16_t) + (size_t)BM * sizeof(long) + 128;
-    static size_t attr_set = 0;
-    if (attr_set < lds) {
-        (void)hipFuncSetAttribute(reinterpret_cast<const void*>(k_igemm_fwd_glds<BM, BN, NS, KG>), hipFuncAttributeMaxDynamicSharedMemorySize, (int)lds);
-        attr_set = lds;
-    }
-    IgemmFwdArgs b = a;
-    hipLaunchKernelGGL((k_igemm_fwd_glds<BM, BN, NS, KG>), dim3(gx, gy), dim3(256 * KG), lds, stream, b);
-    return svsr_check_launch();
+    return a.add_strided ? launch_glds_as<BM, BN, NS, KG, true>(a, gx, gy, stream) : launch_glds_as<BM, BN, NS, KG, false>(a, gx, gy, stream);
 }
 
 struct IgemmFwdPlan { int bm, bn, ns, gy; };
@@ -502,7 +529,7 @@
     return pl;
 }
 
-struct PlanClass { int ntaps; int delta[9], tw[9]; std::vector<int> pos; };
+struct PlanClass { int ntaps; int delta[9], tw[9]; std::vector<int> pos; std::vector<int> cidx; };
 
 static int plan_emit_p8(const std::vector<PlanClass>& cls, int Nimg, int Co, int in_pix, int out_pix, int* words, int cap_words, int* meta, long M, int max_taps, int bn) {
     long tiles_m = 0;
@@ -542,7 +569,8 @@
     return (int)nwords;
 }
 
-static int plan_emit(std::vector<PlanClass>& cls, int Nimg, int Co, int* words, int cap_words, int* meta, const int* p8_pix = nullptr) {
+static int plan_emit(std::vector<PlanClass>& cls, int Nimg, int Co, int* words, int cap_words, int* meta, const int* p8_pix = nullptr,
+                     int add_stride = 1, int add_pix = 0) {
     std::stable_sort(cls.begin(), cls.end(), [](const PlanClass& a, const PlanClass& b) { return a.ntaps > b.ntaps; });
     long M = 0;
     int max_taps = 0;
@@ -563,6 +591,9 @@
     int nwords = PLAN_HDR_WORDS + ncls * PLAN_CLS_WORDS;
     const int pos_word0 = nwords;
     for (const PlanClass& c : cls) nwords += (int)c.pos.size();
+    int add_word = nwords;
+    for (const PlanClass& c : cls) nwords += (int)c.cidx.size();
+    if (add_stride > 1 && (long)Nimg * add_pix >= (1L << 31)) return -SVSR_ERR_ARG;
     long tiles = 0;
     if (words != nullptr) {
         if (cap_words < nwords) return -SVSR_ERR_ARG;
@@ -575,7 +606,9 @@
             if ((long)Nimg * P >= (1L << 24)) return -SVSR_ERR_ARG;
             w[0] = c.ntaps; w[1] = P; w[2] = pos_off; w[3] = (int)tiles;
             for (int t = 0; t < 9; ++t) { w[4 + t] = t < c.ntaps ? c.delta[t] : 0; w[13 + t] = t < c.ntaps ? c.tw[t] : 0; }
-            w[22] = 0; w[23] = 0;
+            w[22] = c.cidx.empty() ? 0 : add_word; w[23] = c.cidx.empty() ? 0 : add_pix;
+            std::copy(c.cidx.begin(), c.cidx.end(), words + add_word);
+            add_word += (int)c.cidx.size();
             std::copy(c.pos.begin(), c.pos.end(), words + pos_word0 + 2 * pos_off);
             pos_off += P;
             tiles += ((long)Nimg * P + pl.bm - 1) / pl.bm;
@@ -585,29 +618,33 @@
     }
     if (tiles > 0x7fffffffL) return -SVSR_ERR_ARG;
     if (meta != nullptr) {
-        meta[0] = pl.bm; meta[1] = pl.bn; meta[2] = pl.ns; meta[3] = (int)tiles; meta[4] = pl.gy; meta[5] = ncls; meta[6] = max_taps;
+        meta[0] = pl.bm; meta[1] = pl.bn; meta[2] = pl.ns; meta[3] = (int)tiles; meta[4] = pl.gy; meta[5] = ncls | (add_stride > 1 ? add_stride << 16 : 0); meta[6] = max_taps;
         meta[7] = (int)(M & 0x7fffffff);
     }
     return nwords;
 }
 
-extern "C" int svsr_conv_plan(int mode, int Nimg, int H, int W, int Co_out, int k, int stride, int pad, int* words, int cap_words, int* meta) {
+static int conv_plan(int mode, int Nimg, int H, int W, int Co_out, int k, int stride, int pad, int add_stride, int* words, int cap_words, int* meta) {
     if (Nimg < 1 || H < 1 || W < 1 || k < 1 || k > 3 || stride < 1 || pad < 0 || Co_out < 1 || mode < 0 || mode > 2) return -SVSR_ERR_ARG;
+    if (add_stride < 1 || add_stride > 0x7fff || (add_stride > 1 && mode != 1)) return -SVSR_ERR_ARG;
+    const int Wc = (W + add_stride - 1) / add_stride, Hc = (H + add_stride - 1) / add_stride;
     const int Ho = (H + 2 * pad - k) / stride + 1, Wo = (W + 2 * pad - k) / stride + 1;
     if (Ho < 1 || Wo < 1) return -SVSR_ERR_ARG;
     std::vector<PlanClass> cls;
-    std::map<std::vector<int>, int> index;
-    auto add = [&](const std::vector<int>& key, int src, int dst) {
+    std::map<std::pair<std::vector<int>, bool>, int> index;
+    auto add = [&](const std::vector<int>& taps, int src, int dst, int cpix = -1) {
+        const std::pair<std::vector<int>, bool> key(taps, cpix >= 0);
         auto it = index.find(key);
         if (it == index.end()) {
             PlanClass c;
-            c.ntaps = (int)(key.size() / 2);
-            for (int t = 0; t < c.ntaps; ++t) { c.delta[t] = key[2 * t]; c.tw[t] = key[2 * t + 1]; }
+            c.ntaps = (int)(taps.size() / 2);
+            for (int t = 0; t < c.ntaps; ++t) { c.delta[t] = taps[2 * t]; c.tw[t] = taps[2 * t + 1]; }
             cls.push_back(c);
             it = index.emplace(key, (int)cls.size() - 1).first;
         }
         cls[it->second].pos.push_back(src);
         cls[it->second].pos.push_back(dst);
+        if (cpix >= 0) cls[it->second].cidx.push_back(cpix);
     };
     std::vector<int> key;
     if (mode == 0) {
@@ -645,12 +682,20 @@
                     for (size_t t = 0; t < key.size(); t += 2) key[t] += shift;
                 }
                 if (mode == 2 && key.empty()) continue;
-                add(key, ca * Wo + cb, y * W + x);
+                add(key, ca * Wo + cb, y * W + x, add_stride > 1 && y % add_stride == 0 && x % add_stride == 0 ? (y / add_stride) * Wc + x / add_stride : -1);
             }
     }
     const int p8_pix[2] = {mode == 0 ? H * W : Ho * Wo, mode == 0 ? Ho * Wo : H * W};
     const bool p8_ok = k == 3 && pad == 1 && H >= 2 && W >= 2 && (stride == 1 || (stride == 2 && mode == 0 && svsr_tune_get(SVSR_TUNE_P8) >= 1 && svsr_tune_get(SVSR_TUNE_P8) != 3));
-    return plan_emit(cls, Nimg, Co_out, words, cap_words, meta, p8_ok ? p8_pix : nullptr);
+    return plan_emit(cls, Nimg, Co_out, words, cap_words, meta, p8_ok && add_stride == 1 ? p8_pix : nullptr, add_stride, Hc * Wc);
+}
+
+extern "C" int svsr_conv_plan(int mode, int Nimg, int H, int W, int Co_out, int k, int stride, int pad, int* words, int cap_words, int* meta) {
+    return conv_plan(mode, Nimg, H, W, Co_out, k, stride, pad, 1, words, cap_words, meta);
+}
+
+extern "C" int svsr_conv_plan_v2(int mode, int Nimg, int H, int W, int Co_out, int k, int stride, int pad, int addend_stride, int* words, int cap_words, int* meta) {
+    return conv_plan(mode, Nimg, H, W, Co_out, k, stride, pad, addend_stride, words, cap_words, meta);
 }
 
 extern "C" int svsr_rows_plan(int Nimg, int P, int src0, int dst0, int Co_out, int* words, int cap_words, int* meta) {
@@ -678,7 +723,7 @@
                          float* stats, const int* plan_dev, const int* meta, int Nimg, int in_pix, int Ci, int in_pitch, int Co,
                          int out_pix, int out_pitch, int wt_taps, int act, int out_f32, float alpha, const unsigned* drop_seed,
                          unsigned drop_site, float drop_p, const void* bnb_y, const void* bnb_x, const float* bnb_mean,
-                         const float* bnb_rstd, const float* bnb_gamma, const float* bnb_beta, int bnb_act, hipStream_t stream) {
+                         const float* bnb_rstd, const float* bnb_gamma, const float* bnb_beta, int bnb_act, hipStream_t stream, int addend_stride = 1) {
     if (plan_dev == nullptr || meta == nullptr || Ci % 64 != 0 || Ci <= 0 || Co <= 0 || in_pitch % 8 != 0 || Nimg <= 0 || wt_taps < 1)
         return SVSR_ERR_ARG;
     if (act != 0 && (addend != nullptr || alpha != 1.f)) return SVSR_ERR_ARG;
@@ -690,6 +735,9 @@
     a.drop = svsr_make_drop(drop_seed, drop_site, drop_p);
     a.bnb_y = (const bf16_t*)bnb_y; a.bnb_x = (const bf16_t*)bnb_x; a.bnb_mean = bnb_mean; a.bnb_rstd = bnb_rstd;
     a.bnb_gamma = bnb_gamma; a.bnb_beta = bnb_beta; a.bnb_act = bnb_act;
+    if (addend_stride < 1 || (meta[5] >> 16) != (addend_stride > 1 ? addend_stride : 0)) return SVSR_ERR_ARG;
+    a.add_strided = addend_stride > 1;
+    if (a.add_strided && (addend == nullptr || addend == out || Co % 8 != 0 || out_pitch % 8 != 0 || out_f32 || meta[0] == P8_BM)) return SVSR_ERR_ARG;
     const int bm = meta[0], bn = meta[1], ns = meta[2], gx = meta[3], gy = (Co + bn - 1) / bn;
     if (gx < 1) return SVSR_ERR_ARG;
     if (bm == P8_BM) return (bnb_x != nullptr && alpha != 1.f) ? SVSR_ERR_ARG : igemm_p8_launch(a, meta, stream);
@@ -733,3 +781,21 @@
     return igemm_fwd_run(in, wt, out, nullptr, nullptr, addend, stats, plan_dev, meta, Nimg, in_pix, Ci, in_pitch, Co, out_pix, out_pitch,
                          wt_taps, 0, 0, 1.0f, nullptr, 0, 0.f, y, x, mean, rstd, gamma, beta, act, stream);
 }
+
+extern "C" int svsr_igemm_dgrad_bn_v2(const void* in, const void* wt, void* out, const void* addend, float* stats, const int* plan_dev,
+                                      const int* meta, int Nimg, int in_pix, int Ci, int in_pitch, int Co, int out_pix, int out_pitch,
+                                      int wt_taps, const void* y, const void* x, const float* mean, const float* rstd, const float* gamma,
+                                      const float* beta, int act, int addend_stride, hipStream_t stream) {
+    if (x == nullptr || mean == nullptr || rstd == nullptr || stats == nullptr || Co % 8 != 0 || out_pitch % 8 != 0) return SVSR_ERR_ARG;
+    if (act != 1 && act != 2) return SVSR_ERR_ARG;
+    if ((y == nullptr || act == 2) && (gamma == nullptr || beta == nullptr)) return SVSR_ERR_ARG;
+    return igemm_fwd_run(in, wt, out, nullptr, nullptr, addend, stats, plan_dev, meta, Nimg, in_pix, Ci, in_pitch, Co, out_pix, out_pitch,
+                         wt_taps, 0, 0, 1.0f, nullptr, 0, 0.f, y, x, mean, rstd, gamma, beta, act, stream, addend_stride);
+}
+
+extern "C" int svsr_igemm_dgrad_v2(const void* in, const void* wt, void* out, const void* addend, const int* plan_dev, const int* meta, int Nimg,
+                                   int in_pix, int Ci, int in_pitch, int Co, int out_pix, int out_pitch, int wt_taps, int addend_stride,
+                                   hipStream_t stream) {
+    return igemm_fwd_run(in, wt, out, nullptr, nullptr, addend, nullptr, plan_dev, meta, Nimg, in_pix, Ci, in_pitch, Co, out_pix, out_pitch,
+                         wt_taps, 0, 0, 1.0f, nullptr, 0, 0.f, nullptr, nullptr, nullptr, nullptr, nullptr, nullptr, 0, stream, addend_stride);
+}
diff --git a/syncvsr_amd/csrc/steplist.hip b/syncvsr_amd/csrc/steplist.hip
--- a/syncvsr_amd/csrc/steplist.hip
+++ b/syncvsr_amd/csrc/steplist.hip
@@ -58,6 +58,7 @@
         SVSR_REG(svsr_mha_table_fwd), SVSR_REG(svsr_lm_embed_fwd),
         SVSR_REG(svsr_beam_select), SVSR_REG(svsr_ctc_prefix_score_clips), SVSR_REG(svsr_mha_src_step_fwd),
         SVSR_REG(svsr_tconv_fwd), SVSR_REG(svsr_tcn_se_fwd), SVSR_REG(svsr_tcn_norm_pool_fwd),
+        SVSR_REG(svsr_igemm_dgrad_v2), SVSR_REG(svsr_igemm_dgrad_bn_v2),
     };
     return r;
 }
diff --git a/syncvsr_amd/model.py b/syncvsr_amd/model.py
--- a/syncvsr_amd/model.py
+++ b/syncvsr_amd/model.py
@@ -647,6 +647,15 @@
     return ops.avgpool_fwd(x)
 
 
+DENSE_DOWNSAMPLE_DGRAD = False
+
+
+def _downsample_dgrad(dcd: torch.Tensor, wdt: torch.Tensor, stride: int, in_hw) -> torch.Tensor:
+    if DENSE_DOWNSAMPLE_DGRAD:
+        return ops.conv2d_dgrad(dcd, wdt, 1, stride, 0, in_hw)
+    return ops.conv2d_dgrad(dcd, wdt, 1, 1, 0, dcd.shape[1:3])
+
+
 def _frontend_backward(model, st: "_ParamStore", tape: dict, dfeats: torch.Tensor) -> None:
     use_tr = model.use_tr
     act = model.trunk_act
@@ -696,11 +705,12 @@
                                     st.g32(f"{td['bn']}.weight"), st.g32(f"{td['bn']}.bias"), 0, False)
             _conv_wgrad(model, st, f"{prefix}.downsample.0", td, dcd, use_tr)
             wdt = st.t16(f"{prefix}.downsample.0.weight").view(inp, 1, 1, planes)
-            dxd = ops.conv2d_dgrad(dcd, wdt, 1, stride, 0, in_hw)
+            dxd = _downsample_dgrad(dcd, wdt, stride, in_hw)
             if tp is not None:
-                dx, dx_stats = ops.conv2d_dgrad_bn(dc1, w1t, 3, stride, 1, in_hw, dxd, tp_aux, tp["c"], tp["mean"], tp["rstd"], *tp_gb)
+                dx, dx_stats = ops.conv2d_dgrad_bn(dc1, w1t, 3, stride, 1, in_hw, dxd, tp_aux, tp["c"], tp["mean"], tp["rstd"], *tp_gb,
+                                                   addend_stride=1 if DENSE_DOWNSAMPLE_DGRAD else stride)
             else:
-                dx, dx_stats = ops.conv2d_dgrad(dc1, w1t, 3, stride, 1, in_hw, addend=dxd), None
+                dx, dx_stats = ops.conv2d_dgrad(dc1, w1t, 3, stride, 1, in_hw, addend=dxd, addend_stride=1 if DENSE_DOWNSAMPLE_DGRAD else stride), None
         elif tp is not None:
             dx, dx_stats = ops.conv2d_dgrad_bn(dc1, w1t, 3, stride, 1, in_hw, dres, tp_aux, tp["c"], tp["mean"], tp["rstd"], *tp_gb)
         else:
diff --git a/syncvsr_amd/ops.py b/syncvsr_amd/ops.py
--- a/syncvsr_amd/ops.py
+++ b/syncvsr_amd/ops.py
@@ -535,12 +535,22 @@
         self.label = f"k_igemm_p8<{self.bm},{self.bn},{self.ns}>" if self.bm == 256 else f"k_igemm_fwd_glds<{self.bm},{self.bn},{self.ns}>"
 
 
-def conv_plan(mode: int, N: int, H: int, W: int, Co_out: int, k: int, stride: int, pad: int) -> Plan:
-    key = ("conv", mode, N, H, W, Co_out, k, stride, pad)
+def conv_plan(mode: int, N: int, H: int, W: int, Co_out: int, k: int, stride: int, pad: int, addend_stride: int = 1) -> Plan:
+    key = ("conv", mode, N, H, W, Co_out, k, stride, pad) if addend_stride == 1 else ("conv", mode, N, H, W, Co_out, k, stride, pad, addend_stride)
     pl = _PLAN_CACHE.get(key)
     if pl is None:
-        pl = _PLAN_CACHE[key] = Plan("svsr_conv_plan", mode, N, H, W, Co_out, k, stride, pad)
+        if addend_stride == 1:
+            pl = _PLAN_CACHE[key] = Plan("svsr_conv_plan", mode, N, H, W, Co_out, k, stride, pad)
+        else:
+            pl = _PLAN_CACHE[key] = Plan("svsr_conv_plan_v2", mode, N, H, W, Co_out, k, stride, pad, addend_stride)
     return pl
+
+
+def _compact_addend_ok(addend: Optional[torch.Tensor], addend_stride: int, N: int, H: int, W: int, C: int) -> None:
+    if addend_stride < 2:
+        raise ValueError("addend_stride must be >= 1")
+    if addend is None or tuple(addend.shape) != (N, -(-H // addend_stride), -(-W // addend_stride), C) or addend.dtype != BF16 or not addend.is_contiguous():
+        raise ValueError(f"a compact addend of stride {addend_stride} is a contiguous bf16 tensor [N, ceil(H/s), ceil(W/s), C]")
 
 
 def rows_plan(Nimg: int, P: int, src0: int, dst0: int, Co_out: int, Ci: Optional[int] = None) -> Plan:
@@ -726,10 +736,17 @@
 
 
 def conv2d_dgrad(dy: torch.Tensor, w16t: torch.Tensor, k: int, stride: int, pad: int, in_hw: tuple[int, int],
-                 addend: Optional[torch.Tensor] = None) -> torch.Tensor:
+                 addend: Optional[torch.Tensor] = None, addend_stride: int = 1) -> torch.Tensor:
     N, Ho, Wo, Co = dy.shape
     Ci = w16t.shape[0]
     H, W = in_hw
+    if addend_stride != 1:
+        _compact_addend_ok(addend, addend_stride, N, H, W, Ci)
+        dx = torch.empty((N, H, W, Ci), dtype=BF16, device=dy.device)
+        plan = conv_plan(1, N, H, W, Ci, k, stride, pad, addend_stride)
+        _call("svsr_igemm_dgrad_v2", _p(dy), _p(w16t), _p(dx), _p(addend), plan.words.data_ptr(), plan.meta, N, Ho * Wo, Co, Co, Ci, H * W, Ci, k * k,
+              addend_stride, _stream(), label=plan.label, flops=2.0 * N * Ho * Wo * Co * Ci * k * k)
+        return dx
     dx = torch.empty((N, H, W, Ci), dtype=BF16, device=dy.device) if addend is None else addend
     if stride == 1 and _c64_ok(Ci, Co, k, stride, pad, W):
         taps = tuple((pad - kh, pad - kw, kh * k + kw) for kh in range(k) for kw in range(k))
@@ -745,7 +762,7 @@
 
 def conv2d_dgrad_bn(dy: torch.Tensor, w16t: torch.Tensor, k: int, stride: int, pad: int, in_hw: tuple[int, int],
                     addend: Optional[torch.Tensor], y: Optional[torch.Tensor], x: torch.Tensor, mean: torch.Tensor, rstd: torch.Tensor,
-                    gamma: Optional[torch.Tensor] = None, beta: Optional[torch.Tensor] = None, act: int = 1):
+                    gamma: Optional[torch.Tensor] = None, beta: Optional[torch.Tensor] = None, act: int = 1, addend_stride: int = 1):
     N, Ho, Wo, Co = dy.shape
     Ci = w16t.shape[0]
     H, W = in_hw
@@ -753,6 +770,15 @@
         raise ValueError("conv2d_dgrad_bn: y / x must be contiguous tensors with the geometry of the result")
     if (y is None or act == 2) and (gamma is None or beta is None):
         raise ValueError("conv2d_dgrad_bn: y=None / act=2 need gamma and beta")
+    if addend_stride != 1:
+        _compact_addend_ok(addend, addend_stride, N, H, W, Ci)
+        g = torch.empty((N, H, W, Ci), dtype=BF16, device=dy.device)
+        plan = conv_plan(1, N, H, W, Ci, k, stride, pad, addend_stride)
+        stats = scratch(plan.tiles * 2 * Ci)
+        _call("svsr_igemm_dgrad_bn_v2", _p(dy), _p(w16t), _p(g), _p(addend), _p(stats), plan.words.data_ptr(), plan.meta, N, Ho * Wo, Co, Co, Ci,
+              H * W, Ci, k * k, _p(y), _p(x), _p(mean), _p(rstd), _p(gamma), _p(beta), act, addend_stride, _stream(), label=plan.label + "+bn",
+              flops=2.0 * N * Ho * Wo * Co * Ci * k * k)
+        return g, (stats, plan.tiles)
     g = torch.empty((N, H, W, Ci), dtype=BF16, device=dy.device) if addend is None else addend
     if stride == 1 and _c64_ok(Ci, Co, k, stride, pad, W):
         taps = tuple((pad - kh, pad - kw, kh * k + kw) for kh in range(k) for kw in range(k))
```
